# microsoft/hyperspace

Hardware: NVIDIA H100
Metric: createIndex rows/sec (higher is better)
Workload: dtype int64

## Files before the change

hyperspace_b200/csrc/api.cu:

```cuda
#include <dirent.h>
#include <fcntl.h>
#include <sys/stat.h>
#include <unistd.h>

#include <algorithm>
#include <atomic>
#include <chrono>
#include <exception>
#include <map>
#include <mutex>
#include <thread>

#include "device_utils.cuh"
#include "engine.h"

using namespace hs;

#define HS_STR2(x) #x
#define HS_STR(x) HS_STR2(x)

namespace {

void set_err(char* err, size_t errlen, const char* msg) {
  if (err && errlen) {
// ... 262 lines not shown
    return HS_EINVAL;
  }
  hs_ctx* ctx = new hs_ctx();
  ctx->device = device_id;
  int rc = guarded(nullptr, err, errlen, [&] {
    HS_CUDA(cudaSetDevice(device_id));
    cudaDeviceProp prop;
    HS_CUDA(cudaGetDeviceProperties(&prop, device_id));
    ctx->sm_count = prop.multiProcessorCount;
    if (prop.major != 9 || prop.minor != 0)
      fail(HS_ENODEVICE, "device %d is sm_%d%d; this library is built for sm_90a only", device_id, prop.major, prop.minor);
    if (cuda_stream) {
      ctx->stream = (cudaStream_t)cuda_stream;
      ctx->own_stream = false;
    } else {
      HS_CUDA(cudaStreamCreateWithFlags(&ctx->stream, cudaStreamNonBlocking));
      ctx->own_stream = true;
    }
    HS_CUDA(cudaStreamCreateWithFlags(&ctx->h2d_stream, cudaStreamNonBlocking));
    HS_CUDA(cudaStreamCreateWithFlags(&ctx->d2h_stream, cudaStreamNonBlocking));
  });
  if (rc != HS_OK) {
    delete ctx;
    return rc == HS_ECUDA ? HS_ENODEVICE : rc;
  }
  *out = ctx;
  return HS_OK;
}

void hs_shutdown(hs_ctx* ctx) {
  if (!ctx) return;
  cudaSetDevice(ctx->device);
  xfer_release(ctx);
  if (ctx->decode_cache && ctx->decode_cache_free) ctx->decode_cache_free(ctx->decode_cache);
  ctx->decode_cache = nullptr;
  comm_destroy(ctx);
  if (ctx->own_stream) cudaStreamDestroy(ctx->stream);
  if (ctx->h2d_stream) {
    cudaStreamSynchronize(ctx->h2d_stream);
    cudaStreamDestroy(ctx->h2d_stream);
  }
  if (ctx->d2h_stream) {
    cudaStreamSynchronize(ctx->d2h_stream);
    cudaStreamDestroy(ctx->d2h_stream);
  }
  delete ctx;
}

void hs_trim(hs_ctx* ctx) {
  if (!ctx) return;
  cudaSetDevice(ctx->device);
  cudaStreamSynchronize(ctx->stream);
  ctx->pool.trim();
}

void hs_profile_enable(hs_ctx* ctx, int on) {
  if (!ctx) return;
  cudaSetDevice(ctx->device);
  cudaStreamSynchronize(ctx->stream);
  for (auto& k : ctx->kevents) {
    ctx->event_pool.push_back(k.a);
    ctx->event_pool.push_back(k.b);
  }
  ctx->kevents.clear();
  ctx->profile = on != 0;
}

int hs_profile_report(hs_ctx* ctx, char* out, size_t outlen) {
  if (!ctx || !out || !outlen) return HS_EINVAL;
  cudaSetDevice(ctx->device);
  cudaStreamSynchronize(ctx->stream);
  std::map<std::string, std::pair<int, double>> acc;
  for (auto& k : ctx->kevents) {
    float ms = 0;
    if (cudaEventElapsedTime(&ms, k.a, k.b) != cudaSuccess) {
      cudaGetLastError();
      continue;
    }
    auto& e = acc[k.name];
    e.first++;
    e.second += ms;
  }
  std::string s = "{";
  bool first = true;
  for (auto& kv : acc) {
    char buf[256];
    snprintf(buf, sizeof buf, "%s\"%s\": {\"launches\": %d, \"ms\": %.6f}", first ? "" : ", ", kv.first.c_str(), kv.second.first,
             kv.second.second);
    s += buf;
    first = false;
  }
  s += "}";
  if (s.size() + 1 > outlen) return HS_ENOMEM;
  memcpy(out, s.c_str(), s.size() + 1);
  for (auto& k : ctx->kevents) {
    ctx->event_pool.push_back(k.a);
    ctx->event_pool.push_back(k.b);
  }
  ctx->kevents.clear();
  return HS_OK;
}

void* hs_host_alloc(hs_ctx* ctx, size_t bytes) {
  if (!ctx) return nullptr;
  try {
    cudaSetDevice(ctx->device);
    return ctx->pool.get(bytes, true);
  } catch (...) {
    return nullptr;
  }
}

void hs_host_free(hs_ctx* ctx, void* p) {
  if (ctx && p) ctx->pool.put(p);
}


int hs_stage_sources(hs_ctx* ctx, const hs_source_file* files, int32_t n_files, hs_staged** out, char* err, size_t errlen) {
  if (!ctx || !out || n_files < 0 || (n_files > 0 && !files)) return HS_EINVAL;
  *out = nullptr;
  std::unique_ptr<hs_staged> sg(new hs_staged());
  sg->ctx = ctx;
  int rc = guarded(ctx, err, errlen, [&] {
    const int launches_before = ctx->launches;
    std::vector<uint64_t> sizes(n_files), off(n_files);
    uint64_t total = 0;
    for (int f = 0; f < n_files; f++) {
      const hs_source_file& sf = files[f];
      if (sf.data && sf.on_device) fail(HS_EINVAL, "source file %d is already on the device", f);
      if (sf.data) {
        sizes[f] = sf.size;
      } else {
        if (!sf.path) fail(HS_EINVAL, "source file %d has neither data nor path", f);
        struct stat st;
        if (stat(sf.path, &st) != 0) fail(HS_EIO, "cannot stat %s", sf.path);
        sizes[f] = (uint64_t)st.st_size;
      }
      if (sizes[f] < 12) fail(HS_EFORMAT, "source file %d: too small to be a Parquet file", f);
      off[f] = total;
      total += round_up(sizes[f], 16) + 16;
    }
    sg->d_images.alloc(ctx, std::max<uint64_t>(total, 16));
    HS_CUDA(cudaEventCreate(&sg->begin));
    HS_CUDA(cudaEventRecord(sg->begin, ctx->h2d_stream));
    sg->files.resize(n_files);
    sg->names.resize(n_files);
    sg->metas.resize(n_files);
    std::vector<uint8_t*> pinned(n_files, nullptr);
    std::vector<size_t> disk;
    for (int f = 0; f < n_files; f++)
      if (!files[f].data) {
        sg->staging.emplace_back(ctx, sizes[f], true);
        pinned[f] = sg->staging.back().get();
        disk.push_back((size_t)f);
      }
    std::vector<std::atomic<int>> read_done(n_files);
    for (auto& d : read_done) d.store(0);
    std::exception_ptr read_error;
    std::thread reader;
    if (!disk.empty())
      reader = std::thread([&] {
        try {
          parallel_files(disk.size(), [&](size_t j) {
            const size_t f = disk[j];
            read_file_into(files[f].path, pinned[f], sizes[f]);
            read_done[f].store(1, std::memory_order_release);
          });
        } catch (...) {
          read_error = std::current_exception();
        }
        for (size_t f : disk)
          if (!read_done[f].load()) read_done[f].store(-1, std::memory_order_release);
      });
    struct Joiner {
      std::thread& t;
      ~Joiner() {
        if (t.joinable()) t.join();
      }
    } joiner{reader};
    for (int f = 0; f < n_files; f++) {
      const hs_source_file& sf = files[f];
      sg->names[f] = sf.path ? sf.path : ("<memory file " + std::to_string(f) + ">");
      const uint8_t* host = (const uint8_t*)sf.data;
      if (!host) {
        int st;
        while ((st = read_done[f].load(std::memory_order_acquire)) == 0) std::this_thread::yield();
        if (st < 0) {
          if (reader.joinable()) reader.join();
          if (read_error) std::rethrow_exception(read_error);
          fail(HS_EIO, "cannot read %s", sf.path);
        }
        host = pinned[f];
      }
      sg->metas[f] = std::make_shared<hs::pq::FileMeta>(hs::pq::parse_footer(host, sizes[f], sg->names[f].c_str()));
      HS_CUDA(cudaMemcpyAsync(sg->d_images.get() + off[f], host, sizes[f], cudaMemcpyHostToDevice, ctx->h2d_stream));
      hs_source_file& o = sg->files[f];
      o.path = nullptr;
      o.data = sg->d_images.get() + off[f];
      o.size = sizes[f];
      o.file_id = sf.file_id;
      o.on_device = 1;
      o.reserved = 0;
      sg->bytes += sizes[f];
    }
    HS_CUDA(cudaEventCreate(&sg->ready));
    HS_CUDA(cudaEventRecord(sg->ready, ctx->h2d_stream));
    for (int f = 0; f < n_files; f++) ctx->staged[sg->files[f].data] = hs_ctx::StagedImage{sg->metas[f], sg->ready};
    ctx->launches = launches_before;
  });
  if (rc == HS_OK) *out = sg.release();
  return rc;
}

int32_t hs_staged_num_files(const hs_staged* s) { return s ? (int32_t)s->files.size() : 0; }

int hs_staged_file(const hs_staged* s, int32_t i, hs_source_file* out) {
  if (!s || !out || i < 0 || i >= (int32_t)s->files.size()) return HS_EINVAL;
  *out = s->files[i];
  out->path = s->names[i].c_str();
  return HS_OK;
}

static void timeline(hs_ctx* ctx, const char* what, cudaEvent_t a, cudaEvent_t b) {
  static const bool on = getenv("HS_TIMELINE") != nullptr;
  if (!on || !a || !b) return;
  static cudaEvent_t base = nullptr;
  if (!base) base = a;
  float t0 = 0, t1 = 0;
  if (cudaEventElapsedTime(&t0, base, a) != cudaSuccess || cudaEventElapsedTime(&t1, base, b) != cudaSuccess) {
    cudaGetLastError();
    return;
  }
  fprintf(stderr, "[hs timeline] %-8s %10.2f -> %10.2f  (%8.2f ms)\n", what, t0, t1, t1 - t0);
}

int hs_staged_wait(hs_staged* s, float* ms_copy) {
  if (!s) return HS_EINVAL;
  cudaSetDevice(s->ctx->device);
  if (cudaEventSynchronize(s->ready) != cudaSuccess) return HS_ECUDA;
  if (ms_copy && cudaEventElapsedTime(ms_copy, s->begin, s->ready) != cudaSuccess) *ms_copy = 0;
  timeline(s->ctx, "H2D", s->begin, s->ready);
  return HS_OK;
}

void hs_staged_free(hs_staged* s) {
  if (!s) return;
  hs_ctx* ctx = s->ctx;
  cudaSetDevice(ctx->device);
  if (s->ready) {
    cudaEventSynchronize(s->ready);
    cudaEventDestroy(s->ready);
  }
  if (s->begin && !getenv("HS_TIMELINE")) cudaEventDestroy(s->begin);
  for (const hs_source_file& f : s->files) ctx->staged.erase(f.data);
  cudaStreamSynchronize(ctx->stream);
  delete s;
}


int hs_create_index_async(hs_ctx* ctx, const hs_index_spec* spec, hs_pending** out, char* err, size_t errlen) {
  if (!ctx || !spec || !out) return HS_EINVAL;
  *out = nullptr;
  std::unique_ptr<hs_pending> pd(new hs_pending());
  pd->ctx = ctx;
  pd->res.reset(new hs_index_result());
  hs_stats& st = pd->st;
  memset(&st, 0, sizeof st);
  hs_index_result* res = pd->res.get();
  int rc = guarded(ctx, err, errlen, [&] {
    if (spec->n_indexed < 1) fail(HS_EINVAL, "at least one indexed column is required");
    if (spec->n_files < 0 || (spec->n_files > 0 && !spec->files)) fail(HS_EINVAL, "bad source file list");
    if (spec->output == HS_OUT_FILES && !spec->out_dir) fail(HS_EINVAL, "HS_OUT_FILES needs out_dir");
    HS_CUDA(cudaEventCreate(&pd->t_begin));
    HS_CUDA(cudaEventCreate(&pd->t_compute_end));
    HS_CUDA(cudaEventRecord(pd->t_begin, ctx->stream));
    std::vector<std::string> cols = names_of(spec->indexed_columns, spec->n_indexed, spec->included_columns, spec->n_included);
    for (size_t i = 0; i < cols.size(); i++)
      for (size_t j = i + 1; j < cols.size(); j++)
        if (cols[i] == cols[j]) fail(HS_EINVAL, "duplicate column '%s' in index config", cols[i].c_str());
    EncodedFiles enc;
    {
      Table table;
      const bool no_carry = getenv("HS_NO_CARRY") != nullptr;
      CarryOptions carry;
      if ((ctx->world == 1 || p2p_exchange_supported(ctx, spec->num_buckets)) && !spec->disable_dictionary &&
          spec->n_deleted_file_ids == 0 && !no_carry && fused_partition_supported(spec->num_buckets)) {
        carry.first_col = spec->n_indexed;
        carry.num_segments = spec->num_buckets;
      }
      if (fused_partition_supported(spec->num_buckets) && spec->n_deleted_file_ids == 0 && !getenv("HS_NO_ZEROCOPY")) {
        carry.zc_tile_rows = fused_tile_rows(p2p_exchange_supported(ctx, spec->num_buckets));
        carry.zc_first_col = spec->n_indexed;
        carry.zc_key = spec->n_indexed == 1;
      }
      SourceSet src;
      open_sources(ctx, spec->files, spec->n_files, &src, &st);
      decode_sources(ctx, src, cols, nullptr, &table, &st, &carry);
      const bool has_strings = table.has_strings;
      if (has_strings && ctx->world > 1)
        fail(HS_EUNSUPPORTED, "string / binary columns are not exchanged between GPUs yet: build this index on one GPU");
      if (spec->lineage) fill_lineage(ctx, table, spec->files, spec->n_files);
      if (spec->n_deleted_file_ids > 0) drop_deleted_rows(ctx, table, spec->deleted_file_ids, spec->n_deleted_file_ids);
      IndexedRows rows;
      if (p2p_exchange_supported(ctx, spec->num_buckets)) {
        exchange_partition_p2p(ctx, table, spec->n_indexed, spec->num_buckets, &rows, &st);
        sort_partitioned_rows(ctx, spec->n_indexed, spec->num_buckets, &rows, &st, true);
      } else {
        if (ctx->world > 1) exchange_rows(ctx, table, spec->n_indexed, spec->num_buckets, &st);
        index_rows(ctx, table, spec->n_indexed, spec->num_buckets, &rows, &st, true);
      }
      if (!has_strings) src.release_images();

      EncodeRequest req;
      req.table = &rows.part;
      req.d_perm = rows.sorted.perm();
      req.d_sorted_keys = rows.sorted.keys();
      req.plan = &rows.plan;
      req.seg_offsets = rows.bucket_offsets;
      req.rows_per_page = spec->rows_per_page;
      req.rows_per_row_group = spec->rows_per_row_group;
      req.use_dictionary = spec->disable_dictionary == 0;
      if (spec->compression != HS_CODEC_UNCOMPRESSED && spec->compression != HS_CODEC_SNAPPY)
        fail(HS_EUNSUPPORTED, "compression codec %d; the GPU path writes UNCOMPRESSED and SNAPPY pages", spec->compression);
      req.codec = spec->compression == HS_CODEC_SNAPPY ? pq::SNAPPY : pq::UNCOMPRESSED;
      const std::string uuid = spec->job_uuid ? spec->job_uuid : make_uuid();
      req.seg_names.resize(spec->num_buckets);
      for (int b = 0; b < spec->num_buckets; b++) {
        char nm[160];
        snprintf(nm, sizeof nm, "part-%05d-%s_%05d.c000%s.parquet", b, uuid.c_str(), b, req.codec == pq::SNAPPY ? ".snappy" : "");
        req.seg_names[b] = nm;
      }
      req.probe = rows.probe.get();
      encode_segments(ctx, req, &enc, &st);
      if (settle_sort(ctx, &rows, &st)) {
        req.probe = nullptr;
        req.d_perm = rows.sorted.perm();
        req.d_sorted_keys = rows.sorted.keys();
        enc = EncodedFiles();
        encode_segments(ctx, req, &enc, &st);
      }
      st.rows_out = rows.part.nrows;
    }
    HS_CUDA(cudaEventRecord(pd->t_compute_end, ctx->stream));
    res->ctx = ctx;
    res->output = spec->output;
    res->files = enc.files;
    pd->save_mode = spec->save_mode;
    if (spec->out_dir) pd->out_dir = spec->out_dir;
    st.gpu_launches = ctx->launches;
    if (spec->output == HS_OUT_DEVICE) {
      res->d_arena = std::move(enc.arena);
      return;
    }
    pd->d_arena = std::move(enc.arena);
    res->h_arena.alloc(ctx, std::max<uint64_t>(enc.arena_bytes, 16), true);
    HS_CUDA(cudaEventCreate(&pd->t_d2h_begin));
    HS_CUDA(cudaEventCreate(&pd->t_d2h_end));
    HS_CUDA(cudaStreamWaitEvent(ctx->d2h_stream, pd->t_compute_end, 0));
    HS_CUDA(cudaEventRecord(pd->t_d2h_begin, ctx->d2h_stream));
    if (enc.arena_bytes)
      HS_CUDA(cudaMemcpyAsync(res->h_arena.get(), pd->d_arena.get(), enc.arena_bytes, cudaMemcpyDeviceToHost, ctx->d2h_stream));
    HS_CUDA(cudaEventRecord(pd->t_d2h_end, ctx->d2h_stream));
    pd->has_d2h = true;
  });
  if (rc == HS_OK) *out = pd.release();
  return rc;
}

int hs_pending_wait(hs_pending* p, hs_index_result** out, hs_stats* stats, char* err, size_t errlen) {
  if (!p || !out) return HS_EINVAL;
  *out = nullptr;
  std::unique_ptr<hs_pending> pd(p);
  hs_ctx* ctx = pd->ctx;
  const int launches = ctx->launches;
  int rc = guarded(ctx, err, errlen, [&] {
    hs_stats& st = pd->st;
    float ms = 0;
    if (pd->has_d2h) {
      HS_CUDA(cudaEventSynchronize(pd->t_d2h_end));
      HS_CUDA(cudaEventElapsedTime(&ms, pd->t_d2h_begin, pd->t_d2h_end));
      st.ms_d2h += ms;
      HS_CUDA(cudaEventElapsedTime(&ms, pd->t_begin, pd->t_d2h_end));
      st.ms_total = ms;
      timeline(ctx, "build", pd->t_begin, pd->t_compute_end);
      timeline(ctx, "D2H", pd->t_d2h_begin, pd->t_d2h_end);
      pd->d_arena.release();
    } else {
      HS_CUDA(cudaEventSynchronize(pd->t_compute_end));
      HS_CUDA(cudaEventElapsedTime(&ms, pd->t_begin, pd->t_compute_end));
      st.ms_total = ms;
    }
    if (pd->res->output == HS_OUT_FILES) {
      const auto w0 = std::chrono::steady_clock::now();
      write_result_files(pd->res.get(), pd->out_dir, pd->save_mode);
      st.ms_write += std::chrono::duration<float, std::milli>(std::chrono::steady_clock::now() - w0).count();
    }
  });
  ctx->launches = launches;
  if (stats) *stats = pd->st;
  if (rc == HS_OK) *out = pd->res.release();
  return rc;
}

void hs_pending_cancel(hs_pending* p) {
  if (!p) return;
  cudaSetDevice(p->ctx->device);
  if (p->has_d2h) cudaEventSynchronize(p->t_d2h_end);
  delete p;
}

int hs_create_index(hs_ctx* ctx, const hs_index_spec* spec, hs_index_result** out, hs_stats* stats, char* err,
                    size_t errlen) {
  if (!ctx || !spec || !out) return HS_EINVAL;
  *out = nullptr;
  if (stats) memset(stats, 0, sizeof *stats);
  hs_pending* pd = nullptr;
  int rc = hs_create_index_async(ctx, spec, &pd, err, errlen);
  if (rc != HS_OK) return rc;
  const int launches = ctx->launches;
  rc = hs_pending_wait(pd, out, stats, err, errlen);
  if (stats) stats->gpu_launches = launches;
  return rc;
}

int32_t hs_result_num_files(const hs_index_result* r) { return r ? (int32_t)r->files.size() : 0; }

int hs_result_file(const hs_index_result* r, int32_t i, int32_t* bucket, const char** name, const void** data,
                   uint64_t* size, int64_t* rows) {
  if (!r || i < 0 || i >= (int32_t)r->files.size()) return HS_EINVAL;
  const OutFile& f = r->files[i];
  if (bucket) *bucket = f.bucket;
  if (name) *name = f.name.c_str();
  if (data) {
    if (r->output == HS_OUT_DEVICE) *data = r->d_arena.get() + f.offset;
    else if (r->output == HS_OUT_HOST) *data = r->h_arena.get() + f.offset;
    else *data = nullptr;
  }
  if (size) *size = f.size;
  if (rows) *rows = f.rows;
  return HS_OK;
}

void hs_result_free(hs_index_result* r) {
  if (!r) return;
  if (r->ctx) {
    cudaSetDevice(r->ctx->device);
    cudaStreamSynchronize(r->ctx->stream);
  }
  delete r;
}


static void batch_from_gather(hs_ctx* ctx, const Table& t, const std::vector<int>& col_idx, const uint32_t* d_idx,
                              int64_t n_out, hs_batch* b) {
  std::vector<Buf<uint8_t>> d_data, d_valid;
  std::vector<Buf<uint64_t>> d_offsets(col_idx.size());
  std::vector<uint64_t> str_bytes(col_idx.size(), 0);
  for (size_t k = 0; k < col_idx.size(); k++) {
    const int ci = col_idx[k];
    const DevColumn& c = t.cols[ci];
    if (c.type == HS_TYPE_STRING) {
      const uint8_t* valid = c.has_nulls ? c.valid.get() : nullptr;
      Buf<uint32_t> lens(ctx, (size_t)std::max<int64_t>(1, n_out));
      d_offsets[k].alloc(ctx, (size_t)n_out + 1);
      launch_string_lengths(ctx, (const uint64_t*)c.data.get(), valid, d_idx, n_out, lens.get());
      exclusive_scan_u32_u64(ctx, lens.get(), n_out, d_offsets[k].get());
      copy_d2h(ctx, &str_bytes[k], d_offsets[k].get() + n_out, 8);
      sync_stream(ctx);
      d_data.emplace_back(ctx, std::max<uint64_t>(1, str_bytes[k]));
      launch_copy_strings(ctx, (const uint64_t*)c.data.get(), valid, d_idx, n_out, d_offsets[k].get(), d_data.back().get());
      d_valid.emplace_back();
      if (c.has_nulls) {
        d_valid.back().alloc(ctx, (size_t)std::max<int64_t>(1, n_out));
        launch_gather_plain(ctx, c.valid.get(), d_idx, n_out, 1, d_valid.back().get());
      }
      continue;
    }
    d_data.emplace_back(ctx, (size_t)std::max<int64_t>(1, n_out) * c.width);
    launch_gather_plain(ctx, c.data.get(), d_idx, n_out, c.width, d_data.back().get());
    d_valid.emplace_back();
    if (c.has_nulls) {
      d_valid.back().alloc(ctx, (size_t)std::max<int64_t>(1, n_out));
      launch_gather_plain(ctx, c.valid.get(), d_idx, n_out, 1, d_valid.back().get());
    }
  }
  for (size_t i = 0; i < col_idx.size(); i++) {
    const DevColumn& c = t.cols[col_idx[i]];
    hs_batch::Col bc;
    bc.name = c.name;
    bc.type = c.type;
    bc.has_valid = c.has_nulls;
    const bool is_str = c.type == HS_TYPE_STRING;
    const size_t data_bytes = is_str ? (size_t)str_bytes[i] : (size_t)n_out * c.width;
    bc.total_bytes = is_str ? str_bytes[i] : 0;
    if (b->on_device) {
      bc.data = std::move(d_data[i]);
      if (is_str) bc.offsets = std::move(d_offsets[i]);
      if (c.has_nulls) bc.valid = std::move(d_valid[i]);
    } else {
      bc.data.alloc(ctx, std::max<size_t>(1, data_bytes), true);
      if (data_bytes) copy_d2h_engine(ctx, bc.data.get(), d_data[i].get(), data_bytes);
      if (is_str) {
        bc.offsets.alloc(ctx, (size_t)n_out + 1, true);
        copy_d2h_engine(ctx, bc.offsets.get(), d_offsets[i].get(), 8 * ((size_t)n_out + 1));
      }
      if (c.has_nulls) {
        bc.valid.alloc(ctx, (size_t)std::max<int64_t>(1, n_out), true);
        if (n_out) copy_d2h_engine(ctx, bc.valid.get(), d_valid[i].get(), (size_t)n_out);
      }
    }
    b->cols.push_back(std::move(bc));
  }
  sync_stream(ctx);
  b->nrows = n_out;
}

__global__ void k_widen_i32(const int32_t* __restrict__ in, int64_t n, int64_t* __restrict__ out) {
  const int64_t stride = (int64_t)gridDim.x * blockDim.x;
  for (int64_t i = (int64_t)blockIdx.x * blockDim.x + threadIdx.x; i < n; i += stride) out[i] = in[i];
}

static const int64_t* widened_key(hs_ctx* ctx, const DevColumn& c, const void* data, int64_t n, Buf<int64_t>* hold) {
  if (c.type == HS_TYPE_INT64) return (const int64_t*)data;
  if (c.type != HS_TYPE_INT32) fail(HS_EUNSUPPORTED, "key column '%s' must be int32 or int64 on the read side", c.name.c_str());
  hold->alloc(ctx, std::max<int64_t>(1, n));
  if (n) {
    k_widen_i32<<<(int)std::min<int64_t>(ceil_div(n, 256), ctx->sm_count * 16), 256, 0, ctx->stream>>>((const int32_t*)data, n,
                                                                                                      hold->get());
    HS_LAUNCH_CHECK(ctx);
  }
  return hold->get();
}

__global__ void k_ranges_to_indices(const int64_t* __restrict__ bounds, const uint64_t* __restrict__ seg_offsets,
                                    const uint64_t* __restrict__ out_offsets, int nseg, uint32_t* __restrict__ out_idx) {
  const int s = blockIdx.x;
  if (s >= nseg) return;
  const int64_t first = bounds[2 * s], last = bounds[2 * s + 1];
  const uint64_t base = seg_offsets[s], o = out_offsets[s];
  for (int64_t i = first + threadIdx.x; i < last; i += blockDim.x) out_idx[o + (i - first)] = (uint32_t)(base + i);
}

}


template <typename F>
static int spark_compare(F a, F b) {
  const bool na = a != a, nb = b != b;
  if (na || nb) return na == nb ? 0 : (na ? 1 : -1);
  return a < b ? -1 : (a > b ? 1 : 0);
}

static int compare_encoded(int col_type, uint64_t e, int lit_type, int64_t lit_i, double lit_f) {
  const bool lit_long = lit_type == HS_TYPE_INT64;
  switch (col_type) {
    case HS_TYPE_INT32:
    case HS_TYPE_INT64: {
      const int64_t v = col_type == HS_TYPE_INT32 ? (int64_t)(int32_t)((uint32_t)e ^ 0x80000000u) : (int64_t)(e ^ 0x8000000000000000ull);
      if (lit_long) return v < lit_i ? -1 : (v > lit_i ? 1 : 0);
      return spark_compare((double)v, lit_f);
    }
    case HS_TYPE_FLOAT: {
      const uint32_t u = (uint32_t)e, bits = (u & 0x80000000u) ? (u & 0x7fffffffu) : ~u;
      float f;
      memcpy(&f, &bits, 4);
      return lit_long ? spark_compare(f, (float)lit_i) : spark_compare((double)f, lit_f);
    }
    default: {
      const uint64_t bits = (e & 0x8000000000000000ull) ? (e & 0x7fffffffffffffffull) : ~e;
      double d;
      memcpy(&d, &bits, 8);
      return spark_compare(d, lit_long ? (double)lit_i : lit_f);
    }
  }
}

static void encoded_domain(int col_type, uint64_t* lo, uint64_t* hi) {
  switch (col_type) {
    case HS_TYPE_INT32: *lo = 0, *hi = 0xffffffffull; return;
    case HS_TYPE_INT64: *lo = 0, *hi = ~0ull; return;
    case HS_TYPE_FLOAT: *lo = 0x007fffffull, *hi = 0xffffffffull; return;
    default: *lo = 0x000fffffffffffffull, *hi = ~0ull; return;
  }
}

struct ResolvedPredicate {
  int col = -1;
  PredRange r{};
  const uint8_t* lo_host = nullptr;
  const uint8_t* hi_host = nullptr;
  uint32_t lo_len = 0, hi_len = 0;
};

static PredRange resolve_predicate(hs_ctx* ctx, const hs_predicate& p, const DevColumn& c, std::vector<Buf<uint8_t>>* holder,
                                   ResolvedPredicate* rp) {
  const bool str_col = c.type == HS_TYPE_STRING;
  int lit = p.literal_type;
  if (lit < 0) {
    if (!str_col && c.type != HS_TYPE_INT32 && c.type != HS_TYPE_INT64) fail(HS_EUNSUPPORTED, "filter scan: key column must be int32 / int64 / string");
    lit = str_col ? HS_TYPE_STRING : HS_TYPE_INT64;
  }
  if (c.type == HS_TYPE_BOOL) fail(HS_EUNSUPPORTED, "filter scan: predicates on the boolean column '%s' are not handled", c.name.c_str());
  if (c.type < HS_TYPE_INT32 || c.type > HS_TYPE_STRING) fail(HS_EUNSUPPORTED, "filter scan: column '%s' has an unhandled type", c.name.c_str());
  if (str_col != (lit == HS_TYPE_STRING))
    fail(HS_EUNSUPPORTED, "filter scan: a %s literal cannot be compared with the %s column '%s'", lit == HS_TYPE_STRING ? "string" : "numeric",
         str_col ? "string" : "numeric", c.name.c_str());
  PredRange r{};
  r.type = c.type;
  r.has_lo = p.has_lo != 0;
  r.has_hi = p.has_hi != 0;
  if (str_col) {
    if ((p.has_lo && p.lo_len && !p.lo_bytes) || (p.has_hi && p.hi_len && !p.hi_bytes))
      fail(HS_EINVAL, "filter scan: string column '%s' needs lo_bytes / hi_bytes", c.name.c_str());
    if (p.lo_len > kMaxStringLen || p.hi_len > kMaxStringLen) fail(HS_EUNSUPPORTED, "string bound longer than 65535 bytes");
    const uint32_t ll = p.has_lo ? p.lo_len : 0, hl = p.has_hi ? p.hi_len : 0;
    holder->emplace_back(ctx, (size_t)ll + hl + 16);
    uint8_t* d = holder->back().get();
    if (ll) copy_h2d(ctx, d, p.lo_bytes, ll);
    if (hl) copy_h2d(ctx, d + ll, p.hi_bytes, hl);
    r.lo = string_ref(d, ll);
    r.hi = string_ref(d + ll, hl);
    r.lo_strict = r.has_lo && p.lo_strict;
    r.hi_strict = r.has_hi && p.hi_strict;
    rp->lo_host = (const uint8_t*)p.lo_bytes, rp->lo_len = ll;
    rp->hi_host = (const uint8_t*)p.hi_bytes, rp->hi_len = hl;
    return r;
  }
  uint64_t emin, emax;
  encoded_domain(c.type, &emin, &emax);
  auto cmp = [&](uint64_t e, bool hi_side) {
    return compare_encoded(c.type, e, lit, hi_side ? p.hi_i : p.lo_i, hi_side ? p.hi_f : p.lo_f);
  };
  bool empty = false;
  if (r.has_lo) {
    const int t = p.lo_strict ? 1 : 0;
    if (cmp(emax, false) < t) {
// ... 778 lines not shown
```

hyperspace_b200/csrc/device_utils.cuh:

```cuda
#pragma once
#include <cuda_runtime.h>

#include <cstdint>

#ifndef HS_HD
#ifdef __CUDACC__
#define HS_HD __host__ __device__ __forceinline__
#else
#define HS_HD inline
#endif
#endif

namespace hs {

HS_HD uint32_t rotl32(uint32_t x, int r) { return (x << r) | (x >> (32 - r)); }
HS_HD uint32_t mm3_mix_k1(uint32_t k1) {
  k1 *= 0xcc9e2d51u;
  k1 = rotl32(k1, 15);
  k1 *= 0x1b873593u;
  return k1;
}
HS_HD uint32_t mm3_mix_h1(uint32_t h1, uint32_t k1) {
  h1 ^= k1;
  h1 = rotl32(h1, 13);
  return h1 * 5u + 0xe6546b64u;
}
HS_HD uint32_t mm3_fmix(uint32_t h1, uint32_t len) {
  h1 ^= len;
  h1 ^= h1 >> 16;
  h1 *= 0x85ebca6bu;
  h1 ^= h1 >> 13;
  h1 *= 0xc2b2ae35u;
  h1 ^= h1 >> 16;
  return h1;
}
HS_HD uint32_t mm3_hash_int(uint32_t v, uint32_t seed) { return mm3_fmix(mm3_mix_h1(seed, mm3_mix_k1(v)), 4); }
HS_HD uint32_t mm3_hash_long(uint64_t v, uint32_t seed) {
  uint32_t h1 = mm3_mix_h1(seed, mm3_mix_k1((uint32_t)v));
  h1 = mm3_mix_h1(h1, mm3_mix_k1((uint32_t)(v >> 32)));
  return mm3_fmix(h1, 8);
}
HS_HD int32_t spark_pmod(uint32_t h, int32_t n) {
  int32_t r = (int32_t)h % n;
  return r < 0 ? r + n : r;
}

constexpr uint32_t kMaxStringLen = 0xffffu;
HS_HD uint64_t string_ref(const void* p, uint32_t len) { return ((uint64_t)(uintptr_t)p & 0xffffffffffffull) | ((uint64_t)len << 48); }
HS_HD const uint8_t* ref_ptr(uint64_t ref) { return (const uint8_t*)(uintptr_t)(ref & 0xffffffffffffull); }
HS_HD uint32_t ref_len(uint64_t ref) { return (uint32_t)(ref >> 48); }

HS_HD uint32_t mm3_hash_bytes(const uint8_t* p, uint32_t len, uint32_t seed) {
  uint32_t h1 = seed;
  const uint32_t aligned = len & ~3u;
  for (uint32_t i = 0; i < aligned; i += 4) {
    const uint32_t w = (uint32_t)p[i] | ((uint32_t)p[i + 1] << 8) | ((uint32_t)p[i + 2] << 16) | ((uint32_t)p[i + 3] << 24);
    h1 = mm3_mix_h1(h1, mm3_mix_k1(w));
  }
  for (uint32_t i = aligned; i < len; i++) h1 = mm3_mix_h1(h1, mm3_mix_k1((uint32_t)(int32_t)(int8_t)p[i]));
  return mm3_fmix(h1, len);
}

HS_HD int string_compare(uint64_t ra, uint64_t rb) {
  const uint8_t *a = ref_ptr(ra), *b = ref_ptr(rb);
  const uint32_t la = ref_len(ra), lb = ref_len(rb), n = la < lb ? la : lb;
  for (uint32_t i = 0; i < n; i++)
    if (a[i] != b[i]) return a[i] < b[i] ? -1 : 1;
  return la == lb ? 0 : (la < lb ? -1 : 1);
}

HS_HD uint64_t string_chunk(uint64_t ref, uint32_t chunk) {
  const uint8_t* p = ref_ptr(ref);
  const uint32_t len = ref_len(ref), begin = chunk * 8;
  uint64_t v = 0;
  for (uint32_t i = 0; i < 8; i++) v = (v << 8) | (begin + i < len ? (uint64_t)p[begin + i] : 0ull);
  return v;
}

HS_HD uint32_t mm3_hash_value(int type, uint64_t raw, uint32_t seed) {
  switch (type) {
    case 0: return mm3_hash_int((uint32_t)raw, seed);
    case 1: return mm3_hash_long(raw, seed);
    case 2: {
      uint32_t b = (uint32_t)raw;
      if ((b & 0x7fffffffu) == 0) b = 0;
      else if ((b & 0x7fffffffu) > 0x7f800000u) b = 0x7fc00000u;
      return mm3_hash_int(b, seed);
    }
    case 3: {
      uint64_t b = raw;
      if ((b & 0x7fffffffffffffffull) == 0) b = 0;
      else if ((b & 0x7fffffffffffffffull) > 0x7ff0000000000000ull) b = 0x7ff8000000000000ull;
      return mm3_hash_long(b, seed);
    }
    case 4: return mm3_hash_int((raw & 0xff) ? 1u : 0u, seed);
    case 5: return mm3_hash_bytes(ref_ptr(raw), ref_len(raw), seed);
  }
  return seed;
}

HS_HD uint64_t sort_encode(int type, uint64_t raw) {
  switch (type) {
    case 0: return (uint64_t)((uint32_t)raw ^ 0x80000000u);
    case 1: return raw ^ 0x8000000000000000ull;
    case 2: {
      uint32_t b = (uint32_t)raw;
      if ((b & 0x7fffffffu) == 0) b = 0;
      else if ((b & 0x7fffffffu) > 0x7f800000u) b = 0x7fc00000u;
      return (uint64_t)((b & 0x80000000u) ? ~b : (b | 0x80000000u));
    }
    case 3: {
      uint64_t b = raw;
      if ((b & 0x7fffffffffffffffull) == 0) b = 0;
      else if ((b & 0x7fffffffffffffffull) > 0x7ff0000000000000ull) b = 0x7ff8000000000000ull;
      return (b & 0x8000000000000000ull) ? ~b : (b | 0x8000000000000000ull);
    }
    case 4: return (raw & 0xff) ? 1 : 0;
  }
  return raw;
}

HS_HD uint32_t dict_hash_u64(uint64_t v) { return (uint32_t)((v * 0x9E3779B97F4A7C15ull) >> 32); }

HS_HD int type_width(int type) {
  switch (type) {
    case 0: case 2: return 4;
    case 1: case 3: return 8;
    case 4: return 1;
    case 5: return 8;
  }
  return 0;
}

#ifdef __CUDACC__

__device__ __forceinline__ uint64_t load_le64_unaligned(const uint8_t* p) {
  uintptr_t a = (uintptr_t)p;
  const uint64_t* w = (const uint64_t*)(a & ~(uintptr_t)7);
  unsigned s = (unsigned)(a & 7) * 8;
  uint64_t lo = __ldg(w);
  if (s == 0) return lo;
  uint64_t hi = __ldg(w + 1);
  return (lo >> s) | (hi << (64 - s));
}
__device__ __forceinline__ uint32_t load_le32_unaligned(const uint8_t* p) {
  uintptr_t a = (uintptr_t)p;
  const uint32_t* w = (const uint32_t*)(a & ~(uintptr_t)3);
  unsigned s = (unsigned)(a & 3) * 8;
  uint32_t lo = __ldg(w);
  if (s == 0) return lo;
  uint32_t hi = __ldg(w + 1);
  return __funnelshift_r(lo, hi, s);
}

__device__ __forceinline__ uint32_t extract_bits(const uint8_t* base, uint64_t idx, uint32_t bw) {
  uint64_t bit = idx * bw;
  const uint8_t* p = base + (bit >> 3);
  uintptr_t a = (uintptr_t)p;
  const uint32_t* w = (const uint32_t*)(a & ~(uintptr_t)3);
  unsigned s = (unsigned)(a & 3) * 8 + (unsigned)(bit & 7);
  uint64_t v = __ldg(w);
  if (s + bw > 32) v |= (uint64_t)__ldg(w + 1) << 32;
  return (uint32_t)((v >> s) & ((bw >= 32) ? 0xffffffffull : ((1ull << bw) - 1)));
}

template <int W>
__device__ __forceinline__ void warp_store_unaligned(uint8_t* dst, uint64_t v, bool active) {
  static_assert(W == 4 || W == 8, "W");
  const unsigned lane = threadIdx.x & 31;
  unsigned long long d = active ? (unsigned long long)(uintptr_t)dst : 0ull;
  unsigned long long d_prev = __shfl_up_sync(0xffffffffu, d, 1);
  uint64_t v_prev = __shfl_up_sync(0xffffffffu, (unsigned long long)v, 1);
  unsigned long long d_next = __shfl_down_sync(0xffffffffu, d, 1);
  if (!active) return;
  const unsigned a = (unsigned)(d & (W - 1));
  if (a == 0) {
    if (W == 8) *(uint64_t*)dst = v;
    else *(uint32_t*)dst = (uint32_t)v;
    return;
  }
  const bool has_prev = lane > 0 && d_prev != 0 && d_prev + W == d;
  const bool has_next = lane < 31 && d_next != 0 && d + W == d_next;
  uint8_t* word = dst - a;
  const unsigned s = a * 8;
  if (has_prev) {
    if (W == 8) *(uint64_t*)word = (v_prev >> (64 - s)) | (v << s);
    else *(uint32_t*)word = (uint32_t)(((uint32_t)v_prev >> (32 - s)) | ((uint32_t)v << s));
  } else {
    for (unsigned i = 0; i < W - a; i++) dst[i] = (uint8_t)(v >> (8 * i));
  }
  if (!has_next) {
    for (unsigned i = W - a; i < W; i++) dst[i] = (uint8_t)(v >> (8 * i));
  }
}

__device__ __forceinline__ unsigned match_any_bits(unsigned amask, unsigned v, int nbits) {
  unsigned peers = amask;
  for (int b = 0; b < nbits; b++) {
    const bool bit = (v >> b) & 1u;
    const unsigned m = __ballot_sync(amask, bit);
    peers &= bit ? m : ~m;
  }
  return peers;
}
template <int NBITS>
__device__ __forceinline__ unsigned match_any_bits(unsigned amask, unsigned v) {
  unsigned peers = amask;
#pragma unroll
  for (int b = 0; b < NBITS; b++) {
    const bool bit = (v & (1u << b)) != 0;
    const unsigned m = __ballot_sync(amask, bit);
    peers &= m ^ (bit ? 0u : ~0u);
  }
  return peers;
}

template <int NBITS>
__device__ __forceinline__ unsigned match_any_full(unsigned v) {
  unsigned peers = 0xffffffffu;
#pragma unroll
  for (int b = 0; b < NBITS; b++) {
    unsigned m, x;
    asm volatile(
        "{\n\t"
        ".reg .pred p;\n\t"
        ".reg .b32 t;\n\t"
        "and.b32 t, %2, %3;\n\t"
        "setp.ne.u32 p, t, 0;\n\t"
        "vote.sync.ballot.b32 %0, p, 0xffffffff;\n\t"
        "selp.b32 %1, 0, 0xffffffff, p;\n\t"
        "}"
        : "=r"(m), "=r"(x)
        : "r"(v), "r"(1u << b));
    peers &= m ^ x;
  }
  return peers;
}

__device__ __forceinline__ uint32_t block_exclusive_scan(uint32_t x, uint32_t* warp_sums, uint32_t* total) {
  const unsigned lane = threadIdx.x & 31, warp = threadIdx.x >> 5, nwarps = (blockDim.x + 31) >> 5;
  uint32_t incl = x;
#pragma unroll
  for (int o = 1; o < 32; o <<= 1) {
    uint32_t y = __shfl_up_sync(0xffffffffu, incl, o);
    if (lane >= (unsigned)o) incl += y;
  }
  __syncthreads();
  if (lane == 31) warp_sums[warp] = incl;
  __syncthreads();
  if (warp == 0) {
    uint32_t w = lane < nwarps ? warp_sums[lane] : 0;
    uint32_t wi = w;
#pragma unroll
    for (int o = 1; o < 32; o <<= 1) {
      uint32_t y = __shfl_up_sync(0xffffffffu, wi, o);
      if (lane >= (unsigned)o) wi += y;
    }
    warp_sums[lane] = wi - w;
    if (lane == 31) warp_sums[32] = wi;
  }
  __syncthreads();
  uint32_t res = warp_sums[warp] + incl - x;
  if (total) *total = warp_sums[32];
  return res;
}

#endif

}
```

hyperspace_b200/csrc/engine.cu:

```cuda
#include <fcntl.h>
#include <sys/stat.h>
#include <unistd.h>

#include <algorithm>
#include <array>
#include <map>
#include <random>

#include "device_utils.cuh"
#include "engine.h"

namespace hs {

std::string make_uuid() {
  std::random_device rd;
  std::mt19937_64 gen(((uint64_t)rd() << 32) ^ rd());
  uint64_t a = gen(), b = gen();
  char buf[40];
  snprintf(buf, sizeof buf, "%08x-%04x-4%03x-%04x-%012llx", (unsigned)(a >> 32), (unsigned)((a >> 16) & 0xffff),
           (unsigned)(a & 0xfff), (unsigned)(0x8000 | ((b >> 48) & 0x3fff)), (unsigned long long)(b & 0xffffffffffffull));
  return buf;
}

namespace {
// ... 436 lines not shown
    sync_stream(ctx);
    check_walk();
    std::vector<SnappyBlob> blobs;
    std::map<const uint8_t*, uint64_t> dict_off;
    uint64_t cursor = 0;
    for (PageDesc& pg : h_pages) {
      if (pg.codec == pq::UNCOMPRESSED) continue;
      if (pg.dict) {
        auto it = dict_off.find(pg.dict);
        if (it == dict_off.end()) {
          it = dict_off.emplace(pg.dict, cursor).first;
          blobs.push_back(SnappyBlob{pg.dict, cursor, (uint32_t)pg.dict_size, (uint32_t)pg.dict_uncompressed_size, 0u, 1u, 0u, 0u});
          cursor += round_up((size_t)pg.dict_uncompressed_size, 16) + 16;
        }
        pg.dict = (const uint8_t*)(uintptr_t)(it->second + 1);
        pg.dict_size = -1;
      }
      if (pg.is_compressed || pg.size != pg.uncompressed_size) {
        const uint32_t prefix = pg.page_type == pq::DATA_PAGE_V2 ? (uint32_t)(pg.rep_bytes + std::max(0, pg.def_bytes)) : 0u;
        if (prefix > (uint32_t)pg.size || prefix > (uint32_t)pg.uncompressed_size)
          fail(HS_EFORMAT, "compressed page has level bytes beyond its size");
        blobs.push_back(SnappyBlob{pg.data, cursor, (uint32_t)pg.size, (uint32_t)pg.uncompressed_size, prefix,
                                   (uint32_t)(pg.is_compressed ? 1 : 0), 0u, 0u});
        pg.data = (const uint8_t*)(uintptr_t)(cursor + 1);
        pg.size = -pg.uncompressed_size;
        cursor += round_up((size_t)pg.uncompressed_size, 16) + 16;
      }
    }
    d_scratch.alloc(ctx, std::max<uint64_t>(cursor, 16) + 16);
    for (PageDesc& pg : h_pages) {
      if (pg.codec == pq::UNCOMPRESSED) continue;
      if (pg.dict_size == -1) {
        pg.dict = d_scratch.get() + ((uintptr_t)pg.dict - 1);
        pg.dict_size = pg.dict_uncompressed_size;
      }
      if (pg.size < 0) {
        pg.data = d_scratch.get() + ((uintptr_t)pg.data - 1);
        pg.size = pg.uncompressed_size;
      }
    }
    uint64_t total_blocks = 0;
    bool any_verbatim = false;
    for (SnappyBlob& b : blobs) {
      any_verbatim = any_verbatim || b.prefix != 0 || !b.compressed;
      b.first_block = (uint32_t)total_blocks;
      total_blocks += snappy_blocks_of(b.dst_len, b.prefix);
    }
    if (total_blocks >= 0xffffffffull) fail(HS_EUNSUPPORTED, "more than 256 TB of compressed pages in one call");
    Buf<SnappyBlob> d_blobs(ctx, std::max<size_t>(1, blobs.size()));
    Buf<uint32_t> d_block_in(ctx, (size_t)total_blocks + 1), d_sequential(ctx, std::max<size_t>(1, blobs.size()));
    copy_h2d(ctx, d_blobs.get(), blobs.data(), sizeof(SnappyBlob) * blobs.size());
    copy_h2d(ctx, d_pages.get(), h_pages.data(), sizeof(PageDesc) * (size_t)n_pages);
    launch_snappy_decompress(ctx, d_blobs.get(), (int64_t)blobs.size(), (int64_t)total_blocks, any_verbatim, d_block_in.get(),
                             d_sequential.get(),
                             d_scratch.get(), d_flags.get());
    sync_stream(ctx);
  }
  Buf<uint64_t> d_string_dicts;
  bool any_string = false;
  for (int c = 0; c < ncols; c++) any_string = any_string || out->cols[c].type == HS_TYPE_STRING;
  out->has_strings = any_string;
  if (any_string && n_pages > 0) {
    std::vector<PageDesc> h_pages((size_t)n_pages);
    copy_d2h(ctx, h_pages.data(), d_pages.get(), sizeof(PageDesc) * (size_t)n_pages);
    sync_stream(ctx);
    check_walk();
    std::map<const uint8_t*, size_t> job_of;
    std::vector<StringDictJob> jobs;
    std::vector<size_t> job_off;
    size_t total = 0;
    for (PageDesc& pg : h_pages) {
      if (pg.phys_type != pq::BYTE_ARRAY || !pg.dict || pg.encoding == pq::ENC_PLAIN) continue;
      auto it = job_of.find(pg.dict);
      if (it == job_of.end()) {
        it = job_of.emplace(pg.dict, jobs.size()).first;
        jobs.push_back(StringDictJob{pg.dict, nullptr, pg.dict_size, pg.dict_count});
        job_off.push_back(total);
        total += (size_t)std::max(0, pg.dict_count);
      }
    }
    if (!jobs.empty()) {
      d_string_dicts.alloc(ctx, std::max<size_t>(1, total));
      for (size_t j = 0; j < jobs.size(); j++) jobs[j].refs = d_string_dicts.get() + job_off[j];
      for (PageDesc& pg : h_pages) {
        if (pg.phys_type != pq::BYTE_ARRAY || !pg.dict || pg.encoding == pq::ENC_PLAIN) continue;
        const StringDictJob& job = jobs[job_of[pg.dict]];
        pg.dict = (const uint8_t*)job.refs;
        pg.dict_size = job.count * 8;
      }
      Buf<StringDictJob> d_jobs(ctx, jobs.size());
      copy_h2d(ctx, d_jobs.get(), jobs.data(), sizeof(StringDictJob) * jobs.size());
      launch_build_string_dicts(ctx, d_jobs.get(), (int64_t)jobs.size(), d_flags.get());
      copy_h2d(ctx, d_pages.get(), h_pages.data(), sizeof(PageDesc) * (size_t)n_pages);
      if (sizeof(PageDesc) * (size_t)n_pages > (16u << 20)) sync_stream(ctx);
    }
  }
  const bool want_zc = carry && carry->zc_tile_rows > 0 && !file_windows && n_pages > 0 && nrows > 0;
  std::vector<uint32_t> local_cls(ncols, 0u);
  constexpr uint32_t kAgreeCap = 8192;
  constexpr int kMaxSpec = 6;
  std::vector<int> spec;
  if (want_carry)
    for (int c = carry->first_col; c < ncols && (int)spec.size() < kMaxSpec; c++) spec.push_back(c);
  const int nspec = (int)spec.size();
  std::vector<uint32_t> spec_state(4 * (size_t)std::max(1, nspec), 0u), spec_count(std::max(1, nspec), 0u);
  std::vector<uint64_t> spec_vals((size_t)std::max(1, nspec) * kAgreeCap);
  if ((want_carry || want_zc) && n_pages > 0) {
    Buf<uint32_t> d_class(ctx, ncols);
    fill_bytes(ctx, d_class.get(), 0, 4 * (size_t)ncols);
    launch_classify_pages(ctx, d_pages.get(), n_pages, d_class.get(), want_zc ? carry->zc_tile_rows : 0);
    copy_d2h(ctx, local_cls.data(), d_class.get(), 4 * (size_t)ncols);
    Buf<uint32_t> d_states(ctx, 4 * (size_t)std::max(1, nspec)), d_cnt(ctx, std::max(1, nspec));
    Buf<unsigned long long> d_vals(ctx, (size_t)std::max(1, nspec) * kAgreeCap);
    std::vector<Buf<unsigned long long>> sets(nspec);
    if (nspec) {
      fill_bytes(ctx, d_states.get(), 0, 16 * (size_t)nspec);
      fill_bytes(ctx, d_cnt.get(), 0, 4 * (size_t)nspec);
      for (int i = 0; i < nspec; i++) {
        const DevColumn& dc = out->cols[spec[i]];
        if ((dc.width != 4 && dc.width != 8) || dc.type == HS_TYPE_STRING) continue;
        sets[i].alloc(ctx, kDictCapacity);
        fill_bytes(ctx, sets[i].get(), 0xFF, sizeof(unsigned long long) * kDictCapacity);
        launch_dict_build_from_pages(ctx, d_pages.get(), n_pages, spec[i], dc.width, sets[i].get(), kDictCapacity, kMaxDictEntries,
                                     d_states.get() + 4 * i);
        launch_dict_collect(ctx, sets[i].get(), kDictCapacity, d_vals.get() + (size_t)i * kAgreeCap, d_cnt.get() + i, kAgreeCap);
      }
      copy_d2h(ctx, spec_state.data(), d_states.get(), 16 * (size_t)nspec);
      copy_d2h(ctx, spec_count.data(), d_cnt.get(), 4 * (size_t)nspec);
      copy_d2h(ctx, spec_vals.data(), d_vals.get(), 8 * (size_t)nspec * kAgreeCap);
    }
    sync_stream(ctx);
  } else {
    sync_stream(ctx);
  }
  check_walk();
  if (want_carry) {
    const int W = ctx->world;
    const size_t per_cand = 5 + kAgreeCap, words = (size_t)ncols + 1 + (size_t)nspec * per_cand;
    std::vector<uint64_t> mine(words, 0ull), all(words * W);
    for (int c = 0; c < ncols; c++) mine[c] = local_cls[c] & (PAGECLASS_NOT_DICT | PAGECLASS_MAYBE_NULLS);
    mine[ncols] = (uint64_t)nrows;
    for (int i = 0; i < nspec; i++) {
      const DevColumn& dc = out->cols[spec[i]];
      uint64_t* m = &mine[(size_t)ncols + 1 + (size_t)i * per_cand];
      m[0] = (uint64_t)(int64_t)dc.type;
      m[1] = dc.type == HS_TYPE_STRING ? 0ull : (uint64_t)dc.width;
      m[2] = spec_state[4 * i];
      m[3] = (spec_state[4 * i + 1] || spec_count[i] > kAgreeCap) ? 1 : 0;
      m[4] = spec_state[4 * i + 2];
      const uint32_t nv = std::min<uint32_t>(spec_count[i], kAgreeCap);
      for (uint32_t j = 0; j < nv; j++) m[5 + j] = spec_vals[(size_t)i * kAgreeCap + j];
      std::sort(m + 5, m + 5 + nv);
      m[2] = nv;
    }
    comm_allgather_host(ctx, mine.data(), 8 * words, all.data());
    DecodeCache* cache = static_cast<DecodeCache*>(ctx->decode_cache);
    const bool hit = cache && cache->num_segments == carry->num_segments && cache->first_col == carry->first_col &&
                     cache->message.size() == all.size() && memcmp(cache->message.data(), all.data(), 8 * all.size()) == 0;
    std::vector<uint32_t> cls(ncols, 0u);
    int64_t total_rows = 0;
    if (hit) {
      total_rows = cache->total_rows;
      for (DecodeCache::Column& cc : cache->carried) {
        DevColumn& dc = out->cols[cc.col];
        dc.carried = true;
        dc.dict_values = cc.values;
        dc.dict_bw = cc.bw;
        dc.codes.alloc(ctx, (size_t)std::max<int64_t>(1, nrows) + 16);
        h_cols[cc.col] = ColumnOut{dc.codes.get(), nullptr, dc.width, dc.type, cc.table.get(), cc.mask, cc.empty_index, 1, 0};
      }
    } else {
      for (int r = 0; r < W; r++) {
        const uint64_t* a = &all[(size_t)r * words];
        for (int c = 0; c < ncols; c++) cls[c] |= (uint32_t)a[c];
        total_rows += (int64_t)a[ncols];
      }
      if (!cache) {
        cache = new DecodeCache();
        ctx->decode_cache = cache;
        ctx->decode_cache_free = free_decode_cache;
      }
      cache->carried.clear();
      cache->message = all;
      cache->num_segments = carry->num_segments;
      cache->first_col = carry->first_col;
      cache->total_rows = total_rows;
    }
    out->global_rows = total_rows;
    int ncarried = 0;
    for (int i = 0; !hit && i < nspec && ncarried < kMaxCarried && total_rows > 0; i++) {
      const int c = spec[i];
      DevColumn& dc = out->cols[c];
      if (cls[c] != 0) continue;
      int type = -1, width = 0;
      bool overflow = false, has_empty = false;
      std::vector<uint64_t> values;
      for (int r = 0; r < W; r++) {
        const uint64_t* m = &all[(size_t)r * words + (size_t)ncols + 1 + (size_t)i * per_cand];
        if ((int64_t)m[0] >= 0) type = (int)(int64_t)m[0];
        width = std::max(width, (int)m[1]);
        overflow = overflow || m[3] != 0;
        has_empty = has_empty || m[4] != 0;
        values.insert(values.end(), m + 5, m + 5 + m[2]);
      }
      if (overflow || type < 0 || (width != 4 && width != 8)) continue;
      if (has_empty) values.push_back(~0ull);
      sort_dictionary(values, type);
      values.erase(std::unique(values.begin(), values.end()), values.end());
      const uint32_t bw = bits_for((uint32_t)values.size());
      if (!dictionary_pays_off((uint32_t)values.size(), bw, width, total_rows, carry->num_segments)) continue;
      cache->carried.emplace_back();
      DecodeCache::Column& cc = cache->carried.back();
      cc.col = c;
      cc.bw = bw;
      upload_lookup_table(ctx, values, &cc.table, &cc.mask, &cc.empty_index);
      cc.values = values;
      dc.carried = true;
      dc.dict_values = std::move(values);
      dc.dict_bw = bw;
      dc.codes.alloc(ctx, (size_t)std::max<int64_t>(1, nrows) + 16);
      h_cols[c] = ColumnOut{dc.codes.get(), nullptr, dc.width, dc.type, cc.table.get(), cc.mask, cc.empty_index, 1, 0};
      ncarried++;
    }
  }
  Buf<ZcTile*> d_tile_src;
  if (want_zc) {
    std::vector<ZcTile*> h_tile_src(ncols, nullptr);
    const int64_t T = carry->zc_tile_rows;
    bool any = false;
    for (int c = 0; c < ncols; c++) {
      DevColumn& dc = out->cols[c];
      const bool candidate = c >= carry->zc_first_col || (c == 0 && carry->zc_key && (dc.type == HS_TYPE_INT32 || dc.type == HS_TYPE_INT64));
      if (!candidate || dc.carried || (dc.width != 4 && dc.width != 8)) continue;
      if (local_cls[c] & (PAGECLASS_NOT_IN_PLACE | PAGECLASS_MAYBE_NULLS)) continue;
      dc.zero_copy = true;
      dc.zc_tiles.alloc(ctx, (size_t)ceil_div(nrows, T));
      h_tile_src[c] = dc.zc_tiles.get();
      h_cols[c] = ColumnOut{nullptr, nullptr, dc.width, dc.type, nullptr, 0u, 0u, 0, 1};
      any = true;
    }
    if (any) {
      d_tile_src.alloc(ctx, ncols);
      copy_h2d(ctx, d_tile_src.get(), h_tile_src.data(), sizeof(ZcTile*) * ncols);
      launch_fill_zc_tiles(ctx, d_pages.get(), n_pages, d_tile_src.get(), (int)T, nrows);
    }
  }
  alloc_destinations();
  copy_h2d(ctx, d_cols.get(), h_cols.data(), sizeof(ColumnOut) * ncols);
  Buf<int64_t> d_window;
  if (file_windows) {
    std::vector<int64_t> w(2 * (size_t)n_files);
    for (int f = 0; f < n_files; f++) {
      w[2 * f] = out->file_row_begin[f] + (*file_windows)[f].first;
      w[2 * f + 1] = out->file_row_begin[f] + (*file_windows)[f].second;
    }
    d_window.alloc(ctx, w.size());
    copy_h2d(ctx, d_window.get(), w.data(), 8 * w.size());
    sync_stream(ctx);
  }
  launch_decode_pages(ctx, d_pages.get(), n_pages, d_cols.get(), d_flags.get() + 1, file_windows ? d_window.get() : nullptr,
                      d_flags.get());
  std::vector<uint32_t> flags(1 + ncols);
  copy_d2h(ctx, flags.data(), d_flags.get(), sizeof(uint32_t) * (1 + ncols));
  t_dec.stop();
  sync_stream(ctx);
  if (flags[0]) {
    const uint32_t code = flags[0] >> 24, detail = flags[0] & 0xffffffu;
    const int ecode = (code == DERR_COMPRESSED || code == DERR_UNSUPPORTED_ENCODING || code == DERR_UNSUPPORTED_TYPE || code == DERR_STRING_TOO_LONG)
                          ? HS_EUNSUPPORTED
                          : HS_EFORMAT;
    fail(ecode, "Parquet decode failed: %s (detail %u)", decode_error_text(code), detail);
  }
  for (int c = 0; c < ncols; c++) out->cols[c].has_nulls = (flags[1 + c] & 1u) != 0;
  if (!file_windows && ctx->world == 1) {
    std::vector<int> cand;
    Buf<uint32_t> d_states(ctx, 4 * (size_t)std::max(1, ncols));
    fill_bytes(ctx, d_states.get(), 0, 16 * (size_t)std::max(1, ncols));
    for (int c = 0; c < ncols; c++) {
      DevColumn& dc = out->cols[c];
      if (dc.carried || dc.zero_copy || dc.type == HS_TYPE_STRING || (flags[1 + c] & 2u) || (dc.width != 4 && dc.width != 8)) continue;
      dc.dict_keys.alloc(ctx, kDictCapacity);
      fill_bytes(ctx, dc.dict_keys.get(), 0xFF, sizeof(unsigned long long) * kDictCapacity);
      launch_dict_build_from_pages(ctx, d_pages.get(), n_pages, c, dc.width, dc.dict_keys.get(), kDictCapacity, kMaxDictEntries,
                                   d_states.get() + 4 * c);
      cand.push_back(c);
    }
    if (!cand.empty()) {
      std::vector<uint32_t> h_states(4 * (size_t)ncols);
      copy_d2h(ctx, h_states.data(), d_states.get(), 16 * (size_t)ncols);
      sync_stream(ctx);
      for (int c : cand) {
        DevColumn& dc = out->cols[c];
        memcpy(dc.dict_state, &h_states[4 * c], 16);
        dc.dict_ready = dc.dict_state[1] == 0;
        if (!dc.dict_ready) dc.dict_keys.release();
      }
    }
  }
  stats->ms_plan += t_plan.ms();
  stats->ms_decode += t_dec.ms();
}


void index_rows(hs_ctx* ctx, Table& table, int nkeys, int num_buckets, IndexedRows* out, hs_stats* stats, bool defer_settle) {
  const int64_t nrows = table.nrows;
  const int ncols = (int)table.cols.size();
  if (num_buckets < 1 || num_buckets > kMaxBuckets)
    fail(HS_EUNSUPPORTED, "numBuckets = %d; the GPU path handles 1..%d buckets", num_buckets, kMaxBuckets);
  if (nkeys < 1 || nkeys > ncols) fail(HS_EINVAL, "bad number of indexed columns");
  if (nrows >= (1ll << 32)) fail(HS_EUNSUPPORTED, "more than 2^32-1 rows per GPU per call");
  StageTimer t_hash(ctx), t_part(ctx);

  t_hash.start();
  std::vector<KeyColumn> h_keys(nkeys);
  for (int k = 0; k < nkeys; k++) {
    DevColumn& c = table.cols[k];
    h_keys[k] = KeyColumn{c.data.get(), c.has_nulls ? c.valid.get() : nullptr, c.type, c.width, c.zero_copy ? c.zc_tiles.get() : nullptr};
  }
  Buf<KeyColumn> d_keys(ctx, nkeys);
  copy_h2d(ctx, d_keys.get(), h_keys.data(), sizeof(KeyColumn) * nkeys);
  const bool fused = fused_partition_supported(num_buckets);
  const int64_t ntiles = ceil_div(nrows, fused ? fused_tile_rows(false) : kPartTile);
  Buf<uint16_t> bucket;
  Buf<uint32_t> tile_hist(ctx, std::max<int64_t>(1, ntiles) * num_buckets);
  Buf<unsigned long long> ghist(ctx, num_buckets);
  out->d_bucket_offsets.alloc(ctx, num_buckets + 1);
  fill_bytes(ctx, ghist.get(), 0, sizeof(unsigned long long) * num_buckets);
  Buf<unsigned long long> d_key_bits(ctx, 2);
  if (fused) {
    const unsigned long long init[2] = {0ull, ~0ull};
    copy_h2d(ctx, d_key_bits.get(), init, sizeof init);
    static const bool rehash = getenv("HS_PART_REHASH") != nullptr;
    if (!rehash) bucket.alloc(ctx, std::max<int64_t>(1, nrows));
    launch_tile_hist(ctx, d_keys.get(), nkeys, nrows, num_buckets, 0, tile_hist.get(), ghist.get(), d_key_bits.get(),
                     single_key_type_of(h_keys.data(), nkeys), rehash ? nullptr : bucket.get());
    copy_d2h(ctx, out->key_or_and, d_key_bits.get(), sizeof out->key_or_and);
    out->have_key_bits = true;
  } else {
    bucket.alloc(ctx, std::max<int64_t>(1, nrows));
    launch_bucket_hist(ctx, d_keys.get(), nkeys, nrows, num_buckets, bucket.get(), tile_hist.get(), ghist.get());
  }
  launch_tile_offsets(ctx, tile_hist.get(), ntiles, num_buckets, ghist.get(),
                      (unsigned long long*)out->d_bucket_offsets.get());
  out->bucket_offsets.assign(num_buckets + 1, 0);
  copy_d2h(ctx, out->bucket_offsets.data(), out->d_bucket_offsets.get(), sizeof(uint64_t) * (num_buckets + 1));
  t_hash.stop();

  t_part.start();
  out->part.nrows = nrows;
  out->part.cols.clear();
  out->part.cols.resize(ncols);
  std::vector<PartColumn> h_pc;
  CodePackRound pack;
  memset(&pack, 0, sizeof pack);
  for (int c = 0; c < ncols; c++) {
    DevColumn& src = table.cols[c];
    DevColumn& dst = out->part.cols[c];
    dst.name = src.name;
    dst.type = src.type;
    dst.width = src.width;
    dst.schema = src.schema;
    dst.has_nulls = src.has_nulls;
    dst.dict_keys = std::move(src.dict_keys);
    memcpy(dst.dict_state, src.dict_state, sizeof dst.dict_state);
    dst.dict_ready = src.dict_ready;
    if (src.carried) {
      if (!fused || c < nkeys || pack.n >= kMaxCarried) fail(HS_EINVAL, "column '%s' cannot be late-materialised here", src.name.c_str());
      dst.carried = true;
      dst.dict_values = std::move(src.dict_values);
      dst.dict_bw = src.dict_bw;
      dst.carry_slot = pack.n;
      pack.src[pack.n++] = src.codes.get();
      continue;
    }
    dst.data.alloc(ctx, (size_t)nrows * src.width + 16);
    h_pc.push_back(PartColumn{src.data.get(), dst.data.get(), src.width, 0, src.zero_copy ? src.zc_tiles.get() : nullptr});
    if (src.has_nulls) {
      dst.valid.alloc(ctx, (size_t)nrows + 16);
      h_pc.push_back(PartColumn{src.valid.get(), dst.valid.get(), 1, 0});
    }
  }
  Buf<uint32_t> dest;
  Buf<PartColumn> d_pc(ctx, h_pc.size());
  if (fused) {
    copy_h2d(ctx, d_pc.get(), h_pc.data(), sizeof(PartColumn) * h_pc.size());
    if (pack.n > 0) {
      out->part.rec.alloc(ctx, (size_t)nrows * 8 + 16);
      pack.out = out->part.rec.get();
    }
    launch_partition_rows(ctx, d_keys.get(), nkeys, nrows, num_buckets, 0, tile_hist.get(), d_pc.get(), (int)h_pc.size(),
                          nullptr, 1, single_key_type_of(h_keys.data(), nkeys), &pack, bucket ? bucket.get() : nullptr);
  } else {
    dest.alloc(ctx, std::max<int64_t>(1, nrows));
    launch_partition_dest(ctx, bucket.get(), nrows, num_buckets, tile_hist.get(), dest.get());
    for (const PartColumn& pc : h_pc) launch_scatter_column(ctx, pc.in, pc.out, dest.get(), nrows, pc.width);
  }
  t_part.stop();
  if (defer_settle) launch_dictionary_probes(ctx, out->part, true, &out->probe);
  sync_stream(ctx);
  for (int c = 0; c < ncols; c++) {
    table.cols[c].data.release();
    table.cols[c].valid.release();
    table.cols[c].codes.release();
    table.cols[c].zc_tiles.release();
  }

  stats->ms_hash += t_hash.ms();
  stats->ms_partition += t_part.ms();
  sort_partitioned_rows(ctx, nkeys, num_buckets, out, stats, defer_settle);
}

void sort_partitioned_rows(hs_ctx* ctx, int nkeys, int num_buckets, IndexedRows* out, hs_stats* stats, bool defer_settle) {
  auto t_sort = std::make_unique<StageTimer>(ctx);
  if (defer_settle && !out->probe) {
    launch_dictionary_probes(ctx, out->part, true, &out->probe);
    if (out->probe) sync_stream(ctx);
  }
  t_sort->start();
  build_sort_plan(ctx, out->bucket_offsets.data(), num_buckets, &out->plan);
  std::vector<KeyColumn> keys(nkeys);
  for (int k = 0; k < nkeys; k++) {
    const DevColumn& c = out->part.cols[k];
    keys[k] = KeyColumn{c.data.get(), c.has_nulls ? c.valid.get() : nullptr, c.type, c.width};
  }
  sort_rows(ctx, &out->plan, keys.data(), nkeys, out->have_key_bits ? out->key_or_and : nullptr, defer_settle, &out->sorted);
  t_sort->stop();
  if (out->sorted.queued) {
    out->pending_timers.push_back(IndexedRows::DeferredTimer{std::move(t_sort), &hs_stats::ms_sort});
    return;
  }
  sync_stream(ctx);
  stats->ms_sort += t_sort->ms();
  for (auto& d : out->pending_timers) stats->*(d.field) += d.t->ms();
  out->pending_timers.clear();
}

bool settle_sort(hs_ctx* ctx, IndexedRows* out, hs_stats* stats) {
  StageTimer t(ctx);
  t.start();
  const bool again = settle_sorted_rows(ctx, &out->plan, &out->sorted);
  t.stop();
  if (again) {
    sync_stream(ctx);
    stats->ms_sort += t.ms();
  }
  for (auto& d : out->pending_timers) stats->*(d.field) += d.t->ms();
  out->pending_timers.clear();
  return again;
}

void launch_dictionary_probes(hs_ctx* ctx, const Table& part, bool use_dictionary, std::unique_ptr<DictProbe>* out) {
  out->reset();
  const int ncols = (int)part.cols.size();
  if (!use_dictionary || part.nrows == 0) return;
  auto pr = std::make_unique<DictProbe>();
  pr->mini = std::min<int64_t>(part.nrows, 1 << 14);
  pr->d_states.alloc(ctx, 4 * (size_t)ncols);
  pr->h_states.assign(4 * (size_t)ncols, 0u);
  pr->keys.resize(ncols);
  fill_bytes(ctx, pr->d_states.get(), 0, 16 * (size_t)ncols);
  bool any = false;
  for (int c = 0; c < ncols; c++) {
    const DevColumn& dc = part.cols[c];
    if (dc.has_nulls || dc.carried || dc.type == HS_TYPE_STRING || (dc.dict_ready && dc.dict_keys)) continue;
    if (dc.width != 4 && dc.width != 8) continue;
    pr->keys[c].alloc(ctx, kDictCapacity);
    fill_bytes(ctx, pr->keys[c].get(), 0xFF, sizeof(unsigned long long) * kDictCapacity);
    launch_dict_build(ctx, dc.data.get(), dc.width, 0, pr->mini, pr->keys[c].get(), kDictCapacity, kMaxDictEntries,
                      pr->d_states.get() + 4 * c);
    copy_d2h(ctx, &pr->h_states[4 * (size_t)c], pr->d_states.get() + 4 * c, 16);
    any = true;
  }
  if (!any) return;
  pr->queued_at = ctx->sync_count;
  *out = std::move(pr);
}


void encode_segments(hs_ctx* ctx, const EncodeRequest& req, EncodedFiles* out, hs_stats* stats) {
  const Table& table = *req.table;
  const int ncols = (int)table.cols.size();
  const int nseg = (int)req.seg_offsets.size() - 1;
  int64_t P = req.rows_per_page > 0 ? req.rows_per_page : 131072;
  P = (int64_t)round_up((size_t)P, kSortTile);
  StageTimer t_plan(ctx), t_enc(ctx);
  t_plan.start();
  for (int c = 0; c < ncols; c++) {
    const DevColumn& dc = table.cols[c];
    if (dc.width != 4 && dc.width != 8)
      fail(HS_EUNSUPPORTED, "column '%s': %d-byte values cannot be written by the GPU encoder yet", dc.name.c_str(), dc.width);
  }
  std::vector<pq::SchemaColumn> schema(ncols);
  for (int c = 0; c < ncols; c++) {
    schema[c] = table.cols[c].schema;
    schema[c].repetition = pq::OPTIONAL;
    schema[c].num_children = 0;
    switch (table.cols[c].type) {
      case HS_TYPE_INT32: schema[c].type = pq::INT32; break;
      case HS_TYPE_INT64: schema[c].type = pq::INT64; break;
      case HS_TYPE_FLOAT: schema[c].type = pq::FLOAT; break;
      case HS_TYPE_DOUBLE: schema[c].type = pq::DOUBLE; break;
      case HS_TYPE_STRING: schema[c].type = pq::BYTE_ARRAY; break;
    }
  }
  const std::string schema_json = pq::spark_schema_json(schema);

  const int64_t ntiles = req.plan->ntiles;
  std::vector<std::vector<uint32_t>> tile_valid(ncols), tile_bytes(ncols);
  std::vector<std::vector<uint64_t>> tile_val_off(ncols), tile_def_off(ncols);
  {
    std::vector<Buf<uint32_t>> d_counts(ncols), d_bytes(ncols);
    bool any = false;
    for (int c = 0; c < ncols; c++) {
      if (table.cols[c].type == HS_TYPE_STRING) {
        any = true;
        d_counts[c].alloc(ctx, std::max<int64_t>(1, ntiles));
        d_bytes[c].alloc(ctx, std::max<int64_t>(1, ntiles));
        launch_tile_string_sizes(ctx, req.plan->tiles.get(), ntiles, req.d_perm, (const uint64_t*)table.cols[c].data.get(),
                                 table.cols[c].has_nulls ? table.cols[c].valid.get() : nullptr, d_bytes[c].get(), d_counts[c].get());
        tile_valid[c].resize(ntiles);
        tile_bytes[c].resize(ntiles);
        tile_val_off[c].assign(ntiles, 0);
        tile_def_off[c].assign(ntiles, 0);
        if (ntiles) {
          copy_d2h(ctx, tile_valid[c].data(), d_counts[c].get(), sizeof(uint32_t) * ntiles);
          copy_d2h(ctx, tile_bytes[c].data(), d_bytes[c].get(), sizeof(uint32_t) * ntiles);
        }
        continue;
      }
      if (!table.cols[c].has_nulls) continue;
      any = true;
      d_counts[c].alloc(ctx, std::max<int64_t>(1, ntiles));
      launch_tile_valid_counts(ctx, req.plan->tiles.get(), ntiles, req.d_perm, table.cols[c].valid.get(), d_counts[c].get());
      tile_valid[c].resize(ntiles);
      tile_val_off[c].assign(ntiles, 0);
      tile_def_off[c].assign(ntiles, 0);
      if (ntiles)
        copy_d2h(ctx, tile_valid[c].data(), d_counts[c].get(), sizeof(uint32_t) * ntiles);
    }
    if (any) sync_stream(ctx);
  }
  const std::vector<uint32_t>& seg_tile_begin = req.plan->h_seg_tile_begin;

  struct ColDict {
    bool use = false;
    uint32_t bw = 0, ndict = 0, empty_index = 0, mask = 0;
    Buf<unsigned long long> keys;
    const unsigned long long* keys_ptr = nullptr;
    Buf<uint8_t> entries;
    size_t skel_off = 0, skel_len = 0;
    std::vector<uint64_t> values;
  };
  std::vector<ColDict> dicts(ncols);
  const int64_t total_rows = table.nrows;
  std::vector<int> carried_cols(kMaxCarried, -1);
  for (int c = 0; c < ncols; c++) {
    const DevColumn& dc = table.cols[c];
    if (!dc.carried) continue;
    if (dc.carry_slot < 0 || dc.carry_slot >= kMaxCarried || !table.rec) fail(HS_EINVAL, "column '%s': code record missing", dc.name.c_str());
    ColDict& cd = dicts[c];
    cd.values = dc.dict_values;
    cd.ndict = (uint32_t)cd.values.size();
    cd.bw = dc.dict_bw;
    cd.use = true;
    carried_cols[dc.carry_slot] = c;
  }
  if (req.use_dictionary && total_rows > 0) {
    DictProbe* early = req.probe;
    if (early && ((int)early->keys.size() != ncols || early->mini != std::min<int64_t>(total_rows, 1 << 14))) early = nullptr;
    if (early && !early->delivered(ctx)) sync_stream(ctx);
    Buf<uint32_t> own_states;
    if (early) own_states = std::move(early->d_states);
    else own_states.alloc(ctx, 4 * (size_t)ncols);
    Buf<uint32_t>& d_states = own_states;
    std::vector<uint32_t> h_states(4 * (size_t)ncols, 0u);
    if (early) h_states = early->h_states;
    else fill_bytes(ctx, d_states.get(), 0, 16 * (size_t)ncols);
    const int64_t mini = std::min<int64_t>(total_rows, 1 << 14);
    bool any_sampled = false;
    for (int c = 0; c < ncols; c++) {
      const DevColumn& dc = table.cols[c];
      if (dc.has_nulls || dc.carried || dc.type == HS_TYPE_STRING) continue;
      ColDict& cd = dicts[c];
      if (dc.dict_ready && dc.dict_keys) {
        cd.keys_ptr = dc.dict_keys.get();
        memcpy(&h_states[4 * (size_t)c], dc.dict_state, 16);
        continue;
      }
      if (early && early->keys[c]) {
        cd.keys = std::move(early->keys[c]);
        cd.keys_ptr = cd.keys.get();
        continue;
      }
      cd.keys.alloc(ctx, kDictCapacity);
      cd.keys_ptr = cd.keys.get();
      fill_bytes(ctx, cd.keys.get(), 0xFF, sizeof(unsigned long long) * kDictCapacity);
      launch_dict_build(ctx, dc.data.get(), dc.width, 0, mini, cd.keys.get(), kDictCapacity, kMaxDictEntries, d_states.get() + 4 * c);
      copy_d2h(ctx, &h_states[4 * (size_t)c], d_states.get() + 4 * c, 16);
      any_sampled = true;
    }
    if (any_sampled) sync_stream(ctx);
    for (int c = 0; c < ncols; c++) {
      const DevColumn& dc = table.cols[c];
      if (dc.has_nulls || dc.carried || dc.type == HS_TYPE_STRING) continue;
      ColDict& cd = dicts[c];
      uint32_t* st = &h_states[4 * (size_t)c];
      const bool ready = dc.dict_ready && dc.dict_keys;
      if (!ready) {
        uint32_t* d_state = d_states.get() + 4 * c;
        if (total_rows > (1 << 20) && st[0] + st[2] > 0.95 * mini) {
          cd.keys.release();
          continue;
        }
        const int64_t sample = std::min<int64_t>(total_rows, 1 << 18);
        if (sample > mini) {
          launch_dict_build(ctx, dc.data.get(), dc.width, mini, sample, cd.keys.get(), kDictCapacity, kMaxDictEntries, d_state);
          copy_d2h(ctx, st, d_state, 16);
          sync_stream(ctx);
        }
        if (!st[1] && sample < total_rows) {
          launch_dict_build(ctx, dc.data.get(), dc.width, sample, total_rows, cd.keys.get(), kDictCapacity, kMaxDictEntries, d_state);
          copy_d2h(ctx, st, d_state, 16);
          sync_stream(ctx);
        }
      }
      if (st[1]) {
        cd.keys.release();
        continue;
      }
      cd.values = sorted_dictionary(ctx, cd.keys_ptr, st, dc.type);
      cd.ndict = (uint32_t)cd.values.size();
      cd.bw = bits_for(cd.ndict);
      if (!dictionary_pays_off(cd.ndict, cd.bw, dc.width, total_rows, nseg)) {
        cd.keys.release();
        continue;
      }
      upload_lookup_table(ctx, cd.values, &cd.entries, &cd.mask, &cd.empty_index);
      cd.use = true;
    }
  }

  const bool stats_on_key = req.d_sorted_keys != nullptr && !table.cols[0].has_nulls &&
                            (table.cols[0].type == HS_TYPE_INT32 || table.cols[0].type == HS_TYPE_INT64);
  std::vector<StatPatch> stat_patches;
  std::vector<uint8_t> skeleton;
  std::vector<ByteCopy> copies;
  struct PagePlan {
    uint64_t hdr_off;
    uint32_t hdr_len;
    uint32_t body_len;
  };
  struct FilePlan {
    int seg = 0;
    int64_t rows = 0;
    std::vector<pq::OutRowGroup> rgs;
    std::vector<std::pair<size_t, size_t>> chunk_pages;
  };
  const bool compress = req.codec == pq::SNAPPY;
  std::vector<PagePlan> page_plans;
  std::vector<FilePlan> file_plans;
  auto header_len_at = [&](size_t skel_pos) -> uint32_t {
    thrift::Reader r(skeleton.data() + skel_pos, skeleton.data() + skeleton.size());
    r.skip(thrift::T_STRUCT);
    if (r.bad) fail(HS_EINVAL, "internal: page header does not parse");
    return (uint32_t)(r.p - (skeleton.data() + skel_pos));
  };
  std::vector<uint32_t> seg_page_begin(nseg + 1, 0);
  std::vector<std::vector<uint64_t>> page_value_offset(ncols);
  uint64_t cursor = 0;
  uint32_t page_counter = 0;
  auto emit = [&](uint64_t dst, size_t skel_begin) {
    copies.push_back(ByteCopy{dst, (uint32_t)skel_begin, (uint32_t)(skeleton.size() - skel_begin)});
  };
  for (int c = 0; c < ncols; c++) {
    ColDict& cd = dicts[c];
    if (!cd.use) continue;
    const int W = table.cols[c].width;
    cd.skel_off = skeleton.size();
    pq::write_dict_page_header(skeleton, (int32_t)(cd.ndict * W), (int32_t)cd.ndict);
    for (uint64_t v : cd.values) {
      const uint8_t* vp = (const uint8_t*)&v;
      skeleton.insert(skeleton.end(), vp, vp + W);
    }
    cd.skel_len = skeleton.size() - cd.skel_off;
  }
  out->files.clear();
  for (int s = 0; s < nseg; s++) {
    seg_page_begin[s] = page_counter;
    const int64_t n = (int64_t)(req.seg_offsets[s + 1] - req.seg_offsets[s]);
    if (n == 0) continue;
    int64_t RG = !req.seg_rows_per_row_group.empty() ? req.seg_rows_per_row_group[s]
                                                     : (req.rows_per_row_group > 0 ? req.rows_per_row_group : 4194304);
    RG = std::max<int64_t>(P, RG / P * P);
    const uint64_t file_off = round_up(cursor, 64);
    cursor = file_off;
    {
      size_t b = skeleton.size();
      skeleton.insert(skeleton.end(), {'P', 'A', 'R', '1'});
      emit(cursor, b);
      cursor += 4;
    }
    const int64_t npages = ceil_div(n, P);
    for (int c = 0; c < ncols; c++) page_value_offset[c].resize(page_counter + npages);
    std::vector<pq::OutRowGroup> rgs;
    for (int64_t r0 = 0; r0 < n; r0 += RG) {
      const int64_t r1 = std::min(n, r0 + RG);
      pq::OutRowGroup g;
      g.num_rows = r1 - r0;
      g.file_offset = (int64_t)(cursor - file_off);
      const uint64_t rg_begin = cursor;
      for (int c = 0; c < ncols; c++) {
        const int W = table.cols[c].width;
        pq::OutChunk ch;
        ch.type = schema[c].type;
        ch.num_values = r1 - r0;
        ch.data_page_offset = (int64_t)(cursor - file_off);
        ch.null_count = 0;
        ch.value_width = W;
        ch.has_minmax = stats_on_key && c == 0;
        const uint64_t chunk_begin = cursor;
        const size_t chunk_first_page = page_plans.size();
        if (dicts[c].use) {
          ch.has_dictionary = true;
          ch.dictionary_page_offset = (int64_t)(cursor - file_off);
          copies.push_back(ByteCopy{cursor, (uint32_t)dicts[c].skel_off, (uint32_t)dicts[c].skel_len});
          if (compress) {
            const uint32_t hl = header_len_at(dicts[c].skel_off);
            page_plans.push_back(PagePlan{cursor, hl, (uint32_t)(dicts[c].skel_len - hl)});
          }
          cursor += dicts[c].skel_len;
          ch.data_page_offset = (int64_t)(cursor - file_off);
        }
        for (int64_t p0 = r0; p0 < r1; p0 += P) {
          const int64_t np = std::min(P, r1 - p0);
          const size_t b = skeleton.size();
          const uint64_t page_begin = cursor;
          if (dicts[c].use) {
            pq::write_dict_data_page_prefix(skeleton, np, dicts[c].bw);
            emit(cursor, b);
            cursor += skeleton.size() - b;
            page_value_offset[c][page_counter + (p0 / P)] = cursor;
            cursor += (uint64_t)((np + 7) / 8) * dicts[c].bw;
          } else if (table.cols[c].type == HS_TYPE_STRING) {
            const int64_t t0 = seg_tile_begin[s] + p0 / kSortTile, t1 = seg_tile_begin[s] + ceil_div(p0 + np, (int64_t)kSortTile);
            int64_t non_null = 0;
            uint64_t value_bytes = 0;
            for (int64_t t = t0; t < t1; t++) {
              non_null += tile_valid[c][t];
              value_bytes += tile_bytes[c][t];
            }
            if (value_bytes + (uint64_t)np / 8 + 64 >= (1ull << 31)) fail(HS_EUNSUPPORTED, "column '%s': a page of strings exceeds 2 GiB", table.cols[c].name.c_str());
            pq::write_nullable_page_prefix_bytes(skeleton, np, value_bytes);
            emit(cursor, b);
            cursor += skeleton.size() - b;
            const uint64_t def_bits = cursor;
            cursor += (uint64_t)((np + 7) / 8);
            page_value_offset[c][page_counter + (p0 / P)] = cursor;
            uint64_t voff = cursor;
            for (int64_t t = t0; t < t1; t++) {
              tile_def_off[c][t] = def_bits + (uint64_t)(t - t0) * (kSortTile / 8);
              tile_val_off[c][t] = voff;
              voff += tile_bytes[c][t];
            }
            cursor += value_bytes;
            ch.null_count += np - non_null;
          } else if (!table.cols[c].has_nulls) {
            pq::write_plain_page_prefix(skeleton, cursor, np, W);
            emit(cursor, b);
            cursor += skeleton.size() - b;
            page_value_offset[c][page_counter + (p0 / P)] = cursor;
            cursor += (uint64_t)np * W;
          } else {
            const int64_t t0 = seg_tile_begin[s] + p0 / kSortTile, t1 = seg_tile_begin[s] + ceil_div(p0 + np, (int64_t)kSortTile);
            int64_t non_null = 0;
            for (int64_t t = t0; t < t1; t++) non_null += tile_valid[c][t];
            pq::write_nullable_page_prefix(skeleton, np, non_null, W);
            emit(cursor, b);
            cursor += skeleton.size() - b;
            const uint64_t def_bits = cursor;
            cursor += (uint64_t)((np + 7) / 8);
            page_value_offset[c][page_counter + (p0 / P)] = cursor;
            uint64_t voff = cursor;
            for (int64_t t = t0; t < t1; t++) {
              tile_def_off[c][t] = def_bits + (uint64_t)(t - t0) * (kSortTile / 8);
              tile_val_off[c][t] = voff;
              voff += (uint64_t)tile_valid[c][t] * W;
            }
            cursor += (uint64_t)non_null * W;
            ch.null_count += np - non_null;
          }
          if (compress) {
            const uint32_t hl = header_len_at(b);
            page_plans.push_back(PagePlan{page_begin, hl, (uint32_t)(cursor - page_begin - hl)});
          }
        }
        ch.total_size = (int64_t)(cursor - chunk_begin);
        g.chunks.push_back(ch);
        if (compress) {
          if (file_plans.empty() || file_plans.back().seg != s) {
            file_plans.emplace_back();
            file_plans.back().seg = s;
            file_plans.back().rows = n;
          }
          file_plans.back().chunk_pages.emplace_back(chunk_first_page, page_plans.size() - chunk_first_page);
        }
      }
      g.total_byte_size = (int64_t)(cursor - rg_begin);
      rgs.push_back(std::move(g));
    }
    {
      const size_t b = skeleton.size();
      std::vector<pq::StatSlot> slots;
      std::vector<uint8_t> footer = pq::write_footer(schema, rgs, n, schema_json, &slots);
      for (const pq::StatSlot& sl : slots) {
        StatPatch sp;
        int64_t row0 = 0;
        for (int g = 0; g < sl.row_group; g++) row0 += rgs[g].num_rows;
        sp.first_pos = req.seg_offsets[s] + (uint64_t)row0;
        sp.last_pos = sp.first_pos + (uint64_t)rgs[sl.row_group].num_rows - 1;
        for (int j = 0; j < 2; j++) {
          sp.min_off[j] = cursor + sl.min_off[j];
          sp.max_off[j] = cursor + sl.max_off[j];
        }
        sp.width = sl.width;
        sp.pad = 0;
        stat_patches.push_back(sp);
      }
      if (compress) file_plans.back().rgs = rgs;
      skeleton.insert(skeleton.end(), footer.begin(), footer.end());
      uint32_t flen = (uint32_t)footer.size();
      const uint8_t* lp = (const uint8_t*)&flen;
      skeleton.insert(skeleton.end(), lp, lp + 4);
      skeleton.insert(skeleton.end(), {'P', 'A', 'R', '1'});
      emit(cursor, b);
      cursor += skeleton.size() - b;
    }
    OutFile of;
    of.bucket = req.seg_ids.empty() ? s : req.seg_ids[s];
    of.name = req.seg_names[s];
    of.offset = file_off;
    of.size = cursor - file_off;
    of.rows = n;
    out->files.push_back(std::move(of));
    page_counter += (uint32_t)npages;
  }
  seg_page_begin[nseg] = page_counter;
  if (skeleton.size() >= (1ull << 32)) fail(HS_EUNSUPPORTED, "index metadata exceeds 4 GiB");
  out->arena_bytes = cursor;
  out->arena.alloc(ctx, std::max<uint64_t>(cursor, 16) + 64);

  Buf<uint8_t> d_skel(ctx, std::max<size_t>(1, skeleton.size()));
  Buf<ByteCopy> d_copies(ctx, std::max<size_t>(1, copies.size()));
  Buf<uint32_t> d_page_begin(ctx, seg_page_begin.size());
  Buf<uint64_t> d_pvo(ctx, std::max<size_t>(1, (size_t)ncols * page_counter));
  if (!skeleton.empty())
    copy_h2d(ctx, d_skel.get(), skeleton.data(), skeleton.size());
  if (!copies.empty())
    copy_h2d(ctx, d_copies.get(), copies.data(), copies.size() * sizeof(ByteCopy));
  copy_h2d(ctx, d_page_begin.get(), seg_page_begin.data(), seg_page_begin.size() * 4);
  for (int c = 0; c < ncols; c++)
    if (page_counter)
      copy_h2d(ctx, d_pvo.get() + (size_t)c * page_counter, page_value_offset[c].data(), (size_t)page_counter * 8);
  t_plan.stop();

  t_enc.start();
  launch_scatter_bytes(ctx, d_copies.get(), (int64_t)copies.size(), d_skel.get(), out->arena.get());
  for (int c = 0; c < ncols; c++) {
    const DevColumn& dc = table.cols[c];
    GatherColumn gc;
    gc.src = dc.data.get();
    gc.sorted_keys = nullptr;
    gc.key_type = dc.type;
    gc.width = dc.width;
    gc.page_value_offset = d_pvo.get() + (size_t)c * page_counter;
    if (dicts[c].use) continue;
    if (dc.type == HS_TYPE_STRING) {
      Buf<uint64_t> d_voff(ctx, std::max<int64_t>(1, ntiles)), d_doff(ctx, std::max<int64_t>(1, ntiles));
      if (ntiles) {
        copy_h2d(ctx, d_voff.get(), tile_val_off[c].data(), 8 * ntiles);
        copy_h2d(ctx, d_doff.get(), tile_def_off[c].data(), 8 * ntiles);
      }
      launch_gather_encode_strings(ctx, req.plan->tiles.get(), ntiles, req.d_perm, (const uint64_t*)dc.data.get(),
                                   dc.has_nulls ? dc.valid.get() : nullptr, d_voff.get(), d_doff.get(), out->arena.get());
      continue;
    }
    if (dc.has_nulls) {
      Buf<uint64_t> d_voff(ctx, std::max<int64_t>(1, ntiles)), d_doff(ctx, std::max<int64_t>(1, ntiles));
      if (ntiles) {
        copy_h2d(ctx, d_voff.get(), tile_val_off[c].data(), 8 * ntiles);
        copy_h2d(ctx, d_doff.get(), tile_def_off[c].data(), 8 * ntiles);
      }
      launch_gather_encode_nullable(ctx, req.plan->tiles.get(), ntiles, req.d_perm, dc.data.get(), dc.valid.get(), dc.width,
                                    d_voff.get(), d_doff.get(), out->arena.get());
      continue;
    }
    if (c == 0 && req.d_sorted_keys && (dc.type == HS_TYPE_INT32 || dc.type == HS_TYPE_INT64)) gc.sorted_keys = req.d_sorted_keys;
    launch_gather_encode(ctx, req.plan->tiles.get(), req.plan->ntiles, req.plan->seg_start.get(), req.d_perm, gc,
                         d_page_begin.get(), P, out->arena.get());
  }
  if (!stat_patches.empty()) {
    Buf<StatPatch> d_sp(ctx, stat_patches.size());
    copy_h2d(ctx, d_sp.get(), stat_patches.data(), sizeof(StatPatch) * stat_patches.size());
    launch_patch_key_stats(ctx, d_sp.get(), (int64_t)stat_patches.size(), req.d_sorted_keys, table.cols[0].type, out->arena.get());
  }
  {
    std::vector<int> dcols;
    for (int c = 0; c < ncols; c++)
      if (dicts[c].use && !table.cols[c].carried) dcols.push_back(c);
    if (carried_cols[0] >= 0) {
      DictPackArgs pa;
      memset(&pa, 0, sizeof pa);
      for (int slot = 0; slot < kMaxCarried && carried_cols[slot] >= 0; slot++) {
        const int c = carried_cols[slot];
        pa.page_value_offset[slot] = d_pvo.get() + (size_t)c * page_counter;
        pa.bw[slot] = dicts[c].bw;
        pa.ncols = slot + 1;
      }
      launch_dict_pack(ctx, req.plan->tiles.get(), ntiles, req.plan->seg_start.get(), req.d_perm, pa, 4,
                       (const uint16_t*)table.rec.get(), d_page_begin.get(), P, out->arena.get());
    }
    for (size_t b0 = 0; b0 < dcols.size(); b0 += 8) {
      DictMapArgs ma;
      DictPackArgs pa;
      memset(&ma, 0, sizeof ma);
      memset(&pa, 0, sizeof pa);
      const int nd = (int)std::min<size_t>(8, dcols.size() - b0);
      ma.ncols = pa.ncols = nd;
      for (int j = 0; j < nd; j++) {
        const int c = dcols[b0 + j];
        ma.src[j] = table.cols[c].data.get();
        ma.width[j] = table.cols[c].width;
        ma.entries[j] = dicts[c].entries.get();
        ma.mask[j] = dicts[c].mask;
        ma.empty_index[j] = dicts[c].empty_index;
        pa.page_value_offset[j] = d_pvo.get() + (size_t)c * page_counter;
        pa.bw[j] = dicts[c].bw;
      }
      Buf<uint16_t> rec(ctx, (size_t)std::max<int64_t>(1, table.nrows) * (nd <= 4 ? 4 : 8));
      launch_dict_encode_all(ctx, req.plan->tiles.get(), ntiles, req.plan->seg_start.get(), req.d_perm, ma, pa, table.nrows,
                             kDictCapacity, rec.get(), d_page_begin.get(), P, out->arena.get());
    }
  }
  if (compress && !page_plans.empty()) {
    std::vector<SnappyFragment> frags;
    std::vector<size_t> page_first_frag(page_plans.size() + 1, 0);
    uint64_t slot_cursor = 0;
    for (size_t i = 0; i < page_plans.size(); i++) {
      page_first_frag[i] = frags.size();
      const PagePlan& pp = page_plans[i];
      for (uint32_t o = 0; o < pp.body_len; o += kSnappyFragment) {
        const uint32_t len = std::min<uint32_t>(kSnappyFragment, pp.body_len - o);
        frags.push_back(SnappyFragment{pp.hdr_off + pp.hdr_len + o, slot_cursor, len, 0});
        slot_cursor += round_up(snappy_max_compressed(len), 16);
      }
    }
    page_first_frag[page_plans.size()] = frags.size();
    Buf<uint8_t> d_slots(ctx, std::max<uint64_t>(slot_cursor, 16));
    Buf<SnappyFragment> d_frags(ctx, std::max<size_t>(1, frags.size()));
    Buf<uint32_t> d_flen(ctx, std::max<size_t>(1, frags.size()));
    std::vector<uint32_t> flen(frags.size());
    copy_h2d(ctx, d_frags.get(), frags.data(), sizeof(SnappyFragment) * frags.size());
    launch_snappy_compress(ctx, d_frags.get(), (int64_t)frags.size(), out->arena.get(), d_slots.get(), d_flen.get());
    copy_d2h(ctx, flen.data(), d_flen.get(), 4 * frags.size());
    sync_stream(ctx);
    std::vector<uint8_t> skel2;
    std::vector<ByteCopy> copies2;
    std::vector<BlobCopy> blobs;
    std::vector<StatPatch> patches2;
    uint64_t cur2 = 0;
    auto emit2 = [&](size_t skel_begin) {
      copies2.push_back(ByteCopy{cur2, (uint32_t)skel_begin, (uint32_t)(skel2.size() - skel_begin)});
      cur2 += skel2.size() - skel_begin;
    };
    std::map<uint64_t, size_t> skel_at;
    for (const ByteCopy& bc : copies) skel_at[bc.dst] = bc.src;
    size_t page_i = 0;
    std::vector<OutFile> files2;
    for (size_t fi = 0; fi < file_plans.size(); fi++) {
      FilePlan& fp = file_plans[fi];
      const uint64_t file_off = round_up(cur2, 64);
      cur2 = file_off;
      {
        const size_t b0 = skel2.size();
        skel2.insert(skel2.end(), {'P', 'A', 'R', '1'});
        emit2(b0);
      }
      size_t chunk_i = 0;
      for (pq::OutRowGroup& g : fp.rgs) {
        g.file_offset = (int64_t)(cur2 - file_off);
        int64_t rg_comp = 0, rg_uncomp = 0;
        for (pq::OutChunk& ch : g.chunks) {
          const auto range = fp.chunk_pages[chunk_i++];
          const uint64_t chunk_begin = cur2;
          int64_t uncomp = 0;
          bool first_data = true;
          for (size_t pi = range.first; pi < range.first + range.second; pi++, page_i++) {
            const PagePlan& pp = page_plans[pi];
            auto it = skel_at.find(pp.hdr_off);
            if (it == skel_at.end()) fail(HS_EINVAL, "internal: page header not found in the layout");
            thrift::Reader r(skeleton.data() + it->second, skeleton.data() + it->second + pp.hdr_len);
            int32_t ptype = -1, nvals = 0, enc = 0;
            int16_t fid = 0;
            for (;;) {
              const uint8_t t = r.field(fid);
              if (r.bad || t == thrift::T_STOP) break;
              if (fid == 1) ptype = (int32_t)r.zigzag();
              else if (fid == 5 || fid == 7) {
                int16_t f2 = 0;
                for (;;) {
                  const uint8_t t2 = r.field(f2);
                  if (r.bad || t2 == thrift::T_STOP) break;
                  if (f2 == 1) nvals = (int32_t)r.zigzag();
                  else if (f2 == 2) enc = (int32_t)r.zigzag();
                  else r.skip(t2);
                }
              } else r.skip(t);
            }
            uint8_t pre[5];
            int pl = 0;
            for (uint32_t v = pp.body_len;; v >>= 7) {
              if (v >= 0x80) pre[pl++] = (uint8_t)(v | 0x80);
              else {
                pre[pl++] = (uint8_t)v;
                break;
              }
            }
            uint64_t comp = (uint64_t)pl;
            for (size_t f = page_first_frag[pi]; f < page_first_frag[pi + 1]; f++) comp += flen[f];
            if (comp >= (1ull << 31)) fail(HS_EUNSUPPORTED, "a compressed page exceeds 2 GiB");
            const size_t b0 = skel2.size();
            if (ptype == pq::DICTIONARY_PAGE) {
              ch.dictionary_page_offset = (int64_t)(cur2 - file_off);
              pq::write_dict_page_header(skel2, (int32_t)pp.body_len, nvals, (int32_t)comp);
            } else {
              if (first_data) ch.data_page_offset = (int64_t)(cur2 - file_off);
              first_data = false;
              pq::write_data_page_header(skel2, (int32_t)pp.body_len, nvals, enc, (int32_t)comp);
            }
            uncomp += (int64_t)(skel2.size() - b0) + pp.body_len;
            skel2.insert(skel2.end(), pre, pre + pl);
            emit2(b0);
            for (size_t f = page_first_frag[pi]; f < page_first_frag[pi + 1]; f++) {
              blobs.push_back(BlobCopy{frags[f].dst_off, cur2, flen[f], 0});
              cur2 += flen[f];
            }
          }
          ch.total_size = (int64_t)(cur2 - chunk_begin);
          ch.total_uncompressed = uncomp;
          ch.codec = pq::SNAPPY;
          rg_comp += ch.total_size;
          rg_uncomp += uncomp;
        }
        g.total_byte_size = rg_uncomp;
        g.total_compressed = rg_comp;
      }
      {
        const size_t b0 = skel2.size();
        std::vector<pq::StatSlot> slots;
        std::vector<uint8_t> footer = pq::write_footer(schema, fp.rgs, fp.rows, schema_json, &slots);
        for (const pq::StatSlot& sl : slots) {
          StatPatch sp;
          int64_t row0 = 0;
          for (int g = 0; g < sl.row_group; g++) row0 += fp.rgs[g].num_rows;
          sp.first_pos = req.seg_offsets[fp.seg] + (uint64_t)row0;
          sp.last_pos = sp.first_pos + (uint64_t)fp.rgs[sl.row_group].num_rows - 1;
          for (int j = 0; j < 2; j++) {
            sp.min_off[j] = cur2 + sl.min_off[j];
            sp.max_off[j] = cur2 + sl.max_off[j];
          }
          sp.width = sl.width;
          sp.pad = 0;
          patches2.push_back(sp);
        }
        skel2.insert(skel2.end(), footer.begin(), footer.end());
        const uint32_t flen32 = (uint32_t)footer.size();
        const uint8_t* lp = (const uint8_t*)&flen32;
        skel2.insert(skel2.end(), lp, lp + 4);
        skel2.insert(skel2.end(), {'P', 'A', 'R', '1'});
        emit2(b0);
      }
      OutFile of = out->files[fi];
      of.offset = file_off;
      of.size = cur2 - file_off;
      files2.push_back(std::move(of));
    }
    if (skel2.size() >= (1ull << 32)) fail(HS_EUNSUPPORTED, "index metadata exceeds 4 GiB");
    Buf<uint8_t> arena2(ctx, std::max<uint64_t>(cur2, 16) + 64);
    Buf<uint8_t> d_skel2(ctx, std::max<size_t>(1, skel2.size()));
    Buf<ByteCopy> d_copies2(ctx, std::max<size_t>(1, copies2.size()));
    Buf<BlobCopy> d_blobs(ctx, std::max<size_t>(1, blobs.size()));
    copy_h2d(ctx, d_skel2.get(), skel2.data(), skel2.size());
    copy_h2d(ctx, d_copies2.get(), copies2.data(), copies2.size() * sizeof(ByteCopy));
    copy_h2d(ctx, d_blobs.get(), blobs.data(), blobs.size() * sizeof(BlobCopy));
    launch_scatter_bytes(ctx, d_copies2.get(), (int64_t)copies2.size(), d_skel2.get(), arena2.get());
    launch_copy_blobs(ctx, d_blobs.get(), (int64_t)blobs.size(), d_slots.get(), arena2.get());
    if (!patches2.empty()) {
      Buf<StatPatch> d_sp(ctx, patches2.size());
      copy_h2d(ctx, d_sp.get(), patches2.data(), sizeof(StatPatch) * patches2.size());
      launch_patch_key_stats(ctx, d_sp.get(), (int64_t)patches2.size(), req.d_sorted_keys, table.cols[0].type, arena2.get());
    }
    sync_stream(ctx);
    out->arena = std::move(arena2);
    out->arena_bytes = cur2;
    out->files = std::move(files2);
    cursor = cur2;
  }
  t_enc.stop();
  sync_stream(ctx);
  stats->ms_plan += t_plan.ms();
  stats->ms_encode += t_enc.ms();
  stats->bytes_out += (int64_t)cursor;
  stats->files_out += (int32_t)out->files.size();
}

}
```

hyperspace_b200/csrc/engine.h:

```cpp
#pragma once
#include <memory>
#include <string>
#include <vector>

#include "hs_common.h"
#include "kernels.h"
#include "parquet_meta.h"

namespace hs {

struct DevColumn {
  std::string name;
  int32_t type = -1;
  int32_t width = 0;
  pq::SchemaColumn schema;
  Buf<uint8_t> data;
  Buf<uint8_t> valid;
  bool has_nulls = false;
  Buf<unsigned long long> dict_keys;
  uint32_t dict_state[4] = {0, 0, 0, 0};
  bool dict_ready = false;
  bool zero_copy = false;
  Buf<ZcTile> zc_tiles;
  bool carried = false;
  Buf<uint16_t> codes;
  std::vector<uint64_t> dict_values;
  uint32_t dict_bw = 0;
  int carry_slot = -1;
};

constexpr int kMaxCarried = 4;

struct Table {
  int64_t nrows = 0;
  std::vector<DevColumn> cols;
  std::vector<int64_t> file_row_begin;
  int64_t global_rows = -1;
  bool has_strings = false;
  Buf<uint8_t> rec;
};

struct CarryOptions {
  int first_col = -1;
  int num_segments = 1;
  int zc_tile_rows = 0;
  int zc_first_col = 0;
  bool zc_key = false;
};

struct DictProbe {
  int64_t mini = 0;
  Buf<uint32_t> d_states;
  std::vector<uint32_t> h_states;
  std::vector<Buf<unsigned long long>> keys;
  uint64_t queued_at = 0;
  bool delivered(const hs_ctx* ctx) const { return ctx->sync_count > queued_at; }
};

struct IndexedRows {
  Table part;
  std::vector<uint64_t> bucket_offsets;
  Buf<uint64_t> d_bucket_offsets;
  SortPlan plan;
  SortedRows sorted;
  bool have_key_bits = false;
  unsigned long long key_or_and[2] = {0, ~0ull};
  struct DeferredTimer {
    std::unique_ptr<StageTimer> t;
    float hs_stats::*field;
  };
  std::vector<DeferredTimer> pending_timers;
  std::unique_ptr<DictProbe> probe;
};

struct OutFile {
  int32_t bucket = 0;
  std::string name;
  uint64_t offset = 0;
  uint64_t size = 0;
  int64_t rows = 0;
};

struct StageTimes;

struct LoadOptions {
  const int64_t* d_row_window = nullptr;
  bool allow_missing_lineage = true;
};
void load_sources(hs_ctx* ctx, const hs_source_file* files, int n_files, const std::vector<std::string>& columns,
                  Table* out, hs_stats* stats, const CarryOptions* carry = nullptr);
struct SourceSet {
  struct Impl;
  Impl* impl;
  int n_files = 0;
  SourceSet();
  ~SourceSet();
  void release_images();
  SourceSet(const SourceSet&) = delete;
  SourceSet& operator=(const SourceSet&) = delete;
};
void open_sources(hs_ctx* ctx, const hs_source_file* files, int n_files, SourceSet* set, hs_stats* stats);
void decode_sources(hs_ctx* ctx, SourceSet& set, const std::vector<std::string>& columns,
                    const std::vector<std::pair<int64_t, int64_t>>* file_windows, Table* out, hs_stats* stats,
                    const CarryOptions* carry = nullptr);

void index_rows(hs_ctx* ctx, Table& table, int nkeys, int num_buckets, IndexedRows* out, hs_stats* stats, bool defer_settle = false);

struct EncodeRequest {
  const Table* table = nullptr;
  const uint32_t* d_perm = nullptr;
  const uint64_t* d_sorted_keys = nullptr;
  const SortPlan* plan = nullptr;
  std::vector<uint64_t> seg_offsets;
  std::vector<std::string> seg_names;
  std::vector<int32_t> seg_ids;
  int64_t rows_per_page = 0;
  int64_t rows_per_row_group = 0;
  std::vector<int64_t> seg_rows_per_row_group;
  bool use_dictionary = true;
  int codec = 0;
  DictProbe* probe = nullptr;
};
struct EncodedFiles {
  Buf<uint8_t> arena;
  uint64_t arena_bytes = 0;
  std::vector<OutFile> files;
};
void encode_segments(hs_ctx* ctx, const EncodeRequest& req, EncodedFiles* out, hs_stats* stats);

void exchange_rows(hs_ctx* ctx, Table& table, int nkeys, int num_buckets, hs_stats* stats);
void comm_destroy(hs_ctx* ctx);
void comm_allgather_host(hs_ctx* ctx, const void* in, size_t bytes, void* out);
bool p2p_exchange_supported(hs_ctx* ctx, int num_buckets);
void exchange_partition_p2p(hs_ctx* ctx, Table& table, int nkeys, int num_buckets, IndexedRows* out, hs_stats* stats);
void sort_partitioned_rows(hs_ctx* ctx, int nkeys, int num_buckets, IndexedRows* out, hs_stats* stats, bool defer_settle = false);
bool settle_sort(hs_ctx* ctx, IndexedRows* out, hs_stats* stats);
void launch_dictionary_probes(hs_ctx* ctx, const Table& part, bool use_dictionary, std::unique_ptr<DictProbe>* out);

std::string make_uuid();

}

struct hs_index_result {
  hs_ctx* ctx = nullptr;
  int output = HS_OUT_FILES;
  hs::Buf<uint8_t> d_arena;
  hs::Buf<uint8_t> h_arena;
  std::vector<hs::OutFile> files;
};

struct hs_staged {
  hs_ctx* ctx = nullptr;
  hs::Buf<uint8_t> d_images;
  std::vector<hs_source_file> files;
  std::vector<std::string> names;
  std::vector<std::shared_ptr<hs::pq::FileMeta>> metas;
  std::vector<hs::Buf<uint8_t>> staging;
  cudaEvent_t begin = nullptr, ready = nullptr;
  uint64_t bytes = 0;
};

struct hs_pending {
  hs_ctx* ctx = nullptr;
  std::unique_ptr<hs_index_result> res;
  hs_stats st;
  hs::Buf<uint8_t> d_arena;
  cudaEvent_t t_begin = nullptr, t_compute_end = nullptr, t_d2h_begin = nullptr, t_d2h_end = nullptr;
  bool has_d2h = false;
  std::string out_dir;
  int save_mode = 0;
  ~hs_pending() {
    if (getenv("HS_TIMELINE")) return;
    for (cudaEvent_t e : {t_begin, t_compute_end, t_d2h_begin, t_d2h_end})
      if (e) cudaEventDestroy(e);
  }
};

struct hs_batch {
  hs_ctx* ctx = nullptr;
  int64_t nrows = 0;
  bool on_device = false;
  struct Col {
    std::string name;
    int32_t type;
    hs::Buf<uint8_t> data;
    hs::Buf<uint8_t> valid;
    bool has_valid = false;
    hs::Buf<uint64_t> offsets;
    uint64_t total_bytes = 0;
  };
  std::vector<Col> cols;
};
```

hyperspace_b200/csrc/gather_encode.cu:

```cuda
#include "device_utils.cuh"
#include "kernels.h"

namespace hs {

namespace {

constexpr int kThreads = 256;

__device__ __forceinline__ uint64_t sort_decode_int(int type, uint64_t e) {
  return type == 1 ? (e ^ 0x8000000000000000ull) : (uint64_t)((uint32_t)e ^ 0x80000000u);
}

template <int W>
__global__ void __launch_bounds__(kThreads) k_gather_encode(const SortTile* __restrict__ tiles,
                                                             const uint64_t* __restrict__ seg_start,
                                                             const uint32_t* __restrict__ perm, GatherColumn col,
                                                             const uint32_t* __restrict__ bucket_page_begin,
                                                             int64_t rows_per_page, uint8_t* __restrict__ arena) {
  const SortTile t = tiles[blockIdx.x];
  const uint64_t lr0 = t.start - seg_start[t.seg];
  const uint64_t page = lr0 / (uint64_t)rows_per_page;
  uint8_t* const base = arena + col.page_value_offset[bucket_page_begin[t.seg] + page] + (lr0 - page * (uint64_t)rows_per_page) * W;
  const bool aligned = ((uintptr_t)base & (W - 1)) == 0;
  if (aligned && t.count == kSortTile) {
    constexpr int kPer = kSortTile / kThreads;
    uint64_t v[kPer];
    if (col.sorted_keys) {
#pragma unroll
      for (int it = 0; it < kPer; it++) v[it] = sort_decode_int(col.key_type, col.sorted_keys[t.start + it * kThreads + threadIdx.x]);
    } else {
      uint32_t r[kPer];
#pragma unroll
      for (int it = 0; it < kPer; it++) r[it] = perm[t.start + it * kThreads + threadIdx.x];
#pragma unroll
      for (int it = 0; it < kPer; it++) v[it] = W == 8 ? ((const uint64_t*)col.src)[r[it]] : ((const uint32_t*)col.src)[r[it]];
    }
#pragma unroll
    for (int it = 0; it < kPer; it++) {
      const uint32_t i = it * kThreads + threadIdx.x;
      if (W == 8) reinterpret_cast<uint64_t*>(base)[i] = v[it];
      else reinterpret_cast<uint32_t*>(base)[i] = (uint32_t)v[it];
    }
    return;
  }
  const uint32_t iters = (t.count + kThreads - 1) / kThreads;
  for (uint32_t it = 0; it < iters; it++) {
    const uint32_t i = it * kThreads + threadIdx.x;
    const bool active = i < t.count;
    uint64_t v = 0;
    if (active) {
      const uint64_t p = t.start + i;
      if (col.sorted_keys) {
        v = sort_decode_int(col.key_type, col.sorted_keys[p]);
      } else {
        const uint32_t src_row = perm[p];
        v = W == 8 ? ((const uint64_t*)col.src)[src_row] : ((const uint32_t*)col.src)[src_row];
      }
    }
    if (aligned) {
      if (active) {
        if (W == 8) reinterpret_cast<uint64_t*>(base)[i] = v;
        else reinterpret_cast<uint32_t*>(base)[i] = (uint32_t)v;
      }
    } else {
      warp_store_unaligned<W>(base + (size_t)i * W, v, active);
    }
  }
}

__global__ void __launch_bounds__(kThreads) k_tile_valid_counts(const SortTile* __restrict__ tiles,
                                                                 const uint32_t* __restrict__ perm,
                                                                 const uint8_t* __restrict__ valid,
                                                                 uint32_t* __restrict__ counts) {
  __shared__ uint32_t s_total;
  if (threadIdx.x == 0) s_total = 0;
  __syncthreads();
  const SortTile t = tiles[blockIdx.x];
  uint32_t local = 0;
  for (uint32_t i = threadIdx.x; i < t.count; i += kThreads) local += valid[perm[t.start + i]] ? 1u : 0u;
  for (int o = 16; o > 0; o >>= 1) local += __shfl_xor_sync(0xffffffffu, local, o);
  if ((threadIdx.x & 31) == 0 && local) atomicAdd(&s_total, local);
  __syncthreads();
  if (threadIdx.x == 0) counts[blockIdx.x] = s_total;
}

template <int W>
__global__ void __launch_bounds__(kThreads) k_gather_encode_nullable(const SortTile* __restrict__ tiles,
                                                                      const uint32_t* __restrict__ perm,
                                                                      const void* __restrict__ src,
                                                                      const uint8_t* __restrict__ valid,
                                                                      const uint64_t* __restrict__ tile_value_offset,
                                                                      const uint64_t* __restrict__ tile_def_offset,
                                                                      uint8_t* __restrict__ arena) {
  __shared__ uint64_t s_vals[kSortTile];
  __shared__ uint32_t warp_sums[40];
  const SortTile t = tiles[blockIdx.x];
  uint8_t* const def_out = arena + tile_def_offset[blockIdx.x];
  uint32_t base = 0;
  const uint32_t iters = (t.count + kThreads - 1) / kThreads;
  for (uint32_t it = 0; it < iters; it++) {
    const uint32_t i = it * kThreads + threadIdx.x;
    const bool active = i < t.count;
    uint32_t flag = 0;
    uint64_t v = 0;
    if (active) {
      const uint32_t row = perm[t.start + i];
      flag = valid[row] ? 1u : 0u;
      if (flag) v = W == 8 ? ((const uint64_t*)src)[row] : ((const uint32_t*)src)[row];
    }
    const unsigned bits = __ballot_sync(0xffffffffu, flag != 0);
    if ((threadIdx.x & 31) == 0) {
      const uint32_t first = it * kThreads + (threadIdx.x & ~31u);
      if (first < t.count) {
        const uint32_t nbytes = min(4u, (t.count - first + 7) / 8);
        for (uint32_t b = 0; b < nbytes; b++) def_out[first / 8 + b] = (uint8_t)(bits >> (8 * b));
      }
    }
    uint32_t total = 0;
    const uint32_t pos = block_exclusive_scan(flag, warp_sums, &total);
    if (flag) s_vals[base + pos] = v;
    base += total;
  }
  __syncthreads();
  uint8_t* const val_out = arena + tile_value_offset[blockIdx.x];
  const uint32_t viters = (base + kThreads - 1) / kThreads;
  for (uint32_t it = 0; it < viters; it++) {
    const uint32_t j = it * kThreads + threadIdx.x;
    const bool active = j < base;
    warp_store_unaligned<W>(val_out + (size_t)j * W, active ? s_vals[j] : 0, active);
  }
}

__global__ void __launch_bounds__(kThreads) k_tile_string_sizes(const SortTile* __restrict__ tiles, const uint32_t* __restrict__ perm,
                                                                 const uint64_t* __restrict__ refs,
                                                                 const uint8_t* __restrict__ valid,
                                                                 uint32_t* __restrict__ bytes, uint32_t* __restrict__ counts) {
  __shared__ uint32_t s_bytes, s_count;
  if (threadIdx.x == 0) s_bytes = s_count = 0;
  __syncthreads();
  const SortTile t = tiles[blockIdx.x];
  uint32_t b = 0, c = 0;
  for (uint32_t i = threadIdx.x; i < t.count; i += kThreads) {
    const uint32_t row = perm[t.start + i];
    if (!valid || valid[row]) {
      b += 4u + ref_len(refs[row]);
      c++;
    }
  }
  for (int o = 16; o > 0; o >>= 1) {
    b += __shfl_xor_sync(0xffffffffu, b, o);
    c += __shfl_xor_sync(0xffffffffu, c, o);
  }
  if ((threadIdx.x & 31) == 0 && c) {
    atomicAdd(&s_bytes, b);
    atomicAdd(&s_count, c);
  }
  __syncthreads();
  if (threadIdx.x == 0) {
    bytes[blockIdx.x] = s_bytes;
    counts[blockIdx.x] = s_count;
  }
}

__global__ void __launch_bounds__(kThreads) k_gather_encode_strings(const SortTile* __restrict__ tiles,
                                                                     const uint32_t* __restrict__ perm,
                                                                     const uint64_t* __restrict__ refs,
                                                                     const uint8_t* __restrict__ valid,
                                                                     const uint64_t* __restrict__ tile_value_offset,
                                                                     const uint64_t* __restrict__ tile_def_offset,
                                                                     uint8_t* __restrict__ arena) {
  __shared__ uint32_t warp_sums[40];
  const SortTile t = tiles[blockIdx.x];
  uint8_t* const def_out = arena + tile_def_offset[blockIdx.x];
  uint8_t* const val_out = arena + tile_value_offset[blockIdx.x];
  uint32_t base = 0;
  const uint32_t iters = (t.count + kThreads - 1) / kThreads;
  for (uint32_t it = 0; it < iters; it++) {
    const uint32_t i = it * kThreads + threadIdx.x;
    const bool active = i < t.count;
    uint32_t flag = 0;
    uint64_t r = 0;
    if (active) {
      const uint32_t row = perm[t.start + i];
      flag = (!valid || valid[row]) ? 1u : 0u;
      if (flag) r = refs[row];
    }
    const unsigned bits = __ballot_sync(0xffffffffu, flag != 0);
    if ((threadIdx.x & 31) == 0) {
      const uint32_t first = it * kThreads + (threadIdx.x & ~31u);
      if (first < t.count) {
        const uint32_t nbytes = min(4u, (t.count - first + 7) / 8);
        for (uint32_t b = 0; b < nbytes; b++) def_out[first / 8 + b] = (uint8_t)(bits >> (8 * b));
      }
    }
    const uint32_t len = ref_len(r), size = flag ? 4u + len : 0u;
    uint32_t total = 0;
    const uint32_t pos = block_exclusive_scan(size, warp_sums, &total);
    if (flag) {
      uint8_t* o = val_out + base + pos;
      o[0] = (uint8_t)len;
      o[1] = (uint8_t)(len >> 8);
      o[2] = (uint8_t)(len >> 16);
      o[3] = (uint8_t)(len >> 24);
      const uint8_t* src = ref_ptr(r);
      for (uint32_t b = 0; b < len; b++) o[4 + b] = src[b];
    }
    base += total;
  }
}

template <typename T>
__global__ void k_gather_plain(const T* __restrict__ src, const uint32_t* __restrict__ perm, int64_t n,
                               T* __restrict__ out) {
  const int64_t stride = (int64_t)gridDim.x * blockDim.x;
  for (int64_t i = (int64_t)blockIdx.x * blockDim.x + threadIdx.x; i < n; i += stride) out[i] = src[perm[i]];
}

__global__ void k_scatter_bytes(const ByteCopy* __restrict__ copies, int64_t n, const uint8_t* __restrict__ skeleton,
                                uint8_t* __restrict__ arena) {
  const int64_t warp = ((int64_t)blockIdx.x * blockDim.x + threadIdx.x) >> 5;
  const int lane = threadIdx.x & 31;
  if (warp >= n) return;
  const ByteCopy c = copies[warp];
  for (uint32_t i = lane; i < c.len; i += 32) arena[c.dst + i] = skeleton[c.src + i];
}

__global__ void __launch_bounds__(256) k_copy_blobs(const BlobCopy* __restrict__ blobs, const uint8_t* __restrict__ src_base,
                                                     uint8_t* __restrict__ dst_base) {
  const BlobCopy b = blobs[blockIdx.x];
  const uint8_t* src = src_base + b.src;
  uint8_t* dst = dst_base + b.dst;
  const uint32_t head = min(b.len, (uint32_t)((4 - ((uintptr_t)dst & 3)) & 3));
  for (uint32_t i = threadIdx.x; i < head; i += 256) dst[i] = src[i];
  const uint32_t nwords = (b.len - head) / 4;
  uint32_t* d32 = reinterpret_cast<uint32_t*>(dst + head);
  const uint8_t* s0 = src + head;
  for (uint32_t w = threadIdx.x; w < nwords; w += 256) d32[w] = load_le32_unaligned(s0 + 4 * (size_t)w);
  for (uint32_t i = head + 4 * nwords + threadIdx.x; i < b.len; i += 256) dst[i] = src[i];
}

__global__ void k_patch_key_stats(const StatPatch* __restrict__ patches, int64_t n, const uint64_t* __restrict__ sorted_keys,
                                  int key_type, uint8_t* __restrict__ arena) {
  const int64_t i = (int64_t)blockIdx.x * blockDim.x + threadIdx.x;
  if (i >= n) return;
  const StatPatch p = patches[i];
  const uint64_t vmin = sort_decode_int(key_type, sorted_keys[p.first_pos]);
  const uint64_t vmax = sort_decode_int(key_type, sorted_keys[p.last_pos]);
  for (int b = 0; b < p.width; b++) {
    const uint8_t lo = (uint8_t)(vmin >> (8 * b)), hi = (uint8_t)(vmax >> (8 * b));
    arena[p.min_off[0] + b] = lo;
    arena[p.min_off[1] + b] = lo;
    arena[p.max_off[0] + b] = hi;
    arena[p.max_off[1] + b] = hi;
  }
}

__device__ __forceinline__ uint64_t splitmix64(uint64_t seed, uint64_t i) {
  uint64_t z = seed + (i + 1) * 0x9E3779B97F4A7C15ull;
  z = (z ^ (z >> 30)) * 0xBF58476D1CE4E5B9ull;
  z = (z ^ (z >> 27)) * 0x94D049BB133111EBull;
  return z ^ (z >> 31);
}

__global__ void k_synth_column(int col, int64_t first_row, int64_t n, void* __restrict__ out) {
  const int64_t stride = (int64_t)gridDim.x * blockDim.x;
  for (int64_t j = (int64_t)blockIdx.x * blockDim.x + threadIdx.x; j < n; j += stride) {
    const uint64_t i = (uint64_t)(first_row + j);
    switch (col) {
      case 0: ((uint64_t*)out)[j] = splitmix64(42, i); break;
      case 1: ((int64_t*)out)[j] = (int64_t)(splitmix64(43, i) % 1000ull); break;
      case 2: ((double*)out)[j] = (double)i * 1e-3; break;
      case 3: ((int32_t*)out)[j] = (int32_t)(i % 100ull); break;
      case 4: ((float*)out)[j] = (float)(i % 4096ull) * 0.25f; break;
    }
  }
}

inline int grid_for(hs_ctx* ctx, int64_t n, int threads, int per_sm) {
  int64_t want = ceil_div(n, threads);
  int64_t cap = (int64_t)ctx->sm_count * per_sm;
  return (int)std::max<int64_t>(1, std::min(want, cap));
}

}

void launch_gather_encode(hs_ctx* ctx, const SortTile* tiles, int64_t ntiles, const uint64_t* seg_start,
                          const uint32_t* perm, const GatherColumn& col, const uint32_t* bucket_page_begin,
                          int64_t rows_per_page, uint8_t* arena) {
  KernelScope _ks(ctx, "k_gather_encode");
  if (ntiles == 0) return;
  if (col.width == 8)
    k_gather_encode<8><<<(unsigned)ntiles, kThreads, 0, ctx->stream>>>(tiles, seg_start, perm, col, bucket_page_begin,
                                                                        rows_per_page, arena);
  else if (col.width == 4)
    k_gather_encode<4><<<(unsigned)ntiles, kThreads, 0, ctx->stream>>>(tiles, seg_start, perm, col, bucket_page_begin,
                                                                        rows_per_page, arena);
  else
    fail(HS_EUNSUPPORTED, "gather_encode: column width %d", col.width);
  HS_LAUNCH_CHECK(ctx);
}

void launch_tile_valid_counts(hs_ctx* ctx, const SortTile* tiles, int64_t ntiles, const uint32_t* perm,
                              const uint8_t* valid, uint32_t* counts) {
  KernelScope _ks(ctx, "k_tile_valid_counts");
  if (ntiles == 0) return;
  k_tile_valid_counts<<<(unsigned)ntiles, kThreads, 0, ctx->stream>>>(tiles, perm, valid, counts);
  HS_LAUNCH_CHECK(ctx);
}

void launch_gather_encode_nullable(hs_ctx* ctx, const SortTile* tiles, int64_t ntiles, const uint32_t* perm,
                                   const void* src, const uint8_t* valid, int width, const uint64_t* tile_value_offset,
                                   const uint64_t* tile_def_offset, uint8_t* arena) {
  KernelScope _ks(ctx, "k_gather_encode_nullable");
  if (ntiles == 0) return;
  if (width == 8)
    k_gather_encode_nullable<8><<<(unsigned)ntiles, kThreads, 0, ctx->stream>>>(tiles, perm, src, valid, tile_value_offset,
                                                                                 tile_def_offset, arena);
  else if (width == 4)
    k_gather_encode_nullable<4><<<(unsigned)ntiles, kThreads, 0, ctx->stream>>>(tiles, perm, src, valid, tile_value_offset,
                                                                                 tile_def_offset, arena);
  else
    fail(HS_EUNSUPPORTED, "gather_encode_nullable: column width %d", width);
  HS_LAUNCH_CHECK(ctx);
}

void launch_tile_string_sizes(hs_ctx* ctx, const SortTile* tiles, int64_t ntiles, const uint32_t* perm, const uint64_t* refs,
                              const uint8_t* valid, uint32_t* bytes, uint32_t* counts) {
  KernelScope _ks(ctx, "k_tile_string_sizes");
  if (ntiles == 0) return;
  k_tile_string_sizes<<<(unsigned)ntiles, kThreads, 0, ctx->stream>>>(tiles, perm, refs, valid, bytes, counts);
  HS_LAUNCH_CHECK(ctx);
}

void launch_gather_encode_strings(hs_ctx* ctx, const SortTile* tiles, int64_t ntiles, const uint32_t* perm, const uint64_t* refs,
                                  const uint8_t* valid, const uint64_t* tile_value_offset, const uint64_t* tile_def_offset,
                                  uint8_t* arena) {
  KernelScope _ks(ctx, "k_gather_encode_strings");
  if (ntiles == 0) return;
  k_gather_encode_strings<<<(unsigned)ntiles, kThreads, 0, ctx->stream>>>(tiles, perm, refs, valid, tile_value_offset,
                                                                          tile_def_offset, arena);
  HS_LAUNCH_CHECK(ctx);
}

void launch_copy_blobs(hs_ctx* ctx, const BlobCopy* blobs, int64_t n, const uint8_t* src_base, uint8_t* dst_base) {
  KernelScope _ks(ctx, "k_copy_blobs");
  if (n == 0) return;
  k_copy_blobs<<<(unsigned)n, 256, 0, ctx->stream>>>(blobs, src_base, dst_base);
  HS_LAUNCH_CHECK(ctx);
}

void launch_gather_plain(hs_ctx* ctx, const void* src, const uint32_t* perm, int64_t n, int width, void* out) {
  KernelScope _ks(ctx, "k_gather_plain");
  if (n == 0) return;
  const int grid = grid_for(ctx, n, 256, 16);
  switch (width) {
    case 8: k_gather_plain<uint64_t><<<grid, 256, 0, ctx->stream>>>((const uint64_t*)src, perm, n, (uint64_t*)out); break;
    case 4: k_gather_plain<uint32_t><<<grid, 256, 0, ctx->stream>>>((const uint32_t*)src, perm, n, (uint32_t*)out); break;
    case 1: k_gather_plain<uint8_t><<<grid, 256, 0, ctx->stream>>>((const uint8_t*)src, perm, n, (uint8_t*)out); break;
    default: fail(HS_EINVAL, "gather: unsupported width %d", width);
  }
  HS_LAUNCH_CHECK(ctx);
}

void launch_scatter_bytes(hs_ctx* ctx, const ByteCopy* copies, int64_t n, const uint8_t* skeleton, uint8_t* arena) {
  if (n == 0) return;
  const int64_t threads = n * 32;
  k_scatter_bytes<<<(unsigned)ceil_div(threads, 256), 256, 0, ctx->stream>>>(copies, n, skeleton, arena);
  HS_LAUNCH_CHECK(ctx);
}

void launch_patch_key_stats(hs_ctx* ctx, const StatPatch* patches, int64_t n, const uint64_t* sorted_keys, int key_type,
                            uint8_t* arena) {
  if (n == 0) return;
  k_patch_key_stats<<<(unsigned)ceil_div(n, 128), 128, 0, ctx->stream>>>(patches, n, sorted_keys, key_type, arena);
  HS_LAUNCH_CHECK(ctx);
}

void launch_synth_column(hs_ctx* ctx, int col, int64_t first_row, int64_t n, void* out) {
  KernelScope _ks(ctx, "k_synth_column");
  if (n == 0) return;
  k_synth_column<<<grid_for(ctx, n, 256, 16), 256, 0, ctx->stream>>>(col, first_row, n, out);
  HS_LAUNCH_CHECK(ctx);
}

}
```

hyperspace_b200/csrc/kernels.h:

```cpp
#pragma once
#include "hs_common.h"

namespace hs {

struct ChunkDesc {
  const uint8_t* data;
  uint64_t size;
  int64_t num_values;
  int64_t row_base;
  int32_t col;
  int32_t phys_type;
  int32_t max_def;
  int32_t file_index;
  int32_t codec;
  int32_t pad;
};

struct PageDesc {
  const uint8_t* data;
  const uint8_t* dict;
  int64_t first_row;
  int32_t dict_count;
  int32_t size;
  int32_t num_values;
  int32_t encoding;
  int32_t page_type;
  int32_t def_bytes;
  int32_t rep_bytes;
  int32_t col, phys_type, max_def;
  int32_t file_index;
  int32_t uncompressed_size;
  int32_t dict_size, dict_uncompressed_size;
  int32_t is_compressed;
  int32_t codec;
  int32_t chunk;
};

struct ColumnOut {
  void* data;
  uint8_t* valid;
  int32_t width;
  int32_t type;
  const void* carry_entries;
  uint32_t carry_mask;
  uint32_t carry_empty_index;
  int32_t carry;
  int32_t skip;
};

enum : uint32_t { PAGECLASS_NOT_DICT = 1u, PAGECLASS_MAYBE_NULLS = 2u, PAGECLASS_NOT_IN_PLACE = 4u };
void launch_classify_pages(hs_ctx* ctx, const PageDesc* pages, int64_t n_pages, uint32_t* col_flags, int zc_tile_rows);
struct ZcTile {
  const uint8_t* p0;
  const uint8_t* p1;
  int64_t split;
};
void launch_fill_zc_tiles(hs_ctx* ctx, const PageDesc* pages, int64_t n_pages, ZcTile* const* tile_src, int zc_tile_rows,
                          int64_t nrows);

enum DecodeError : uint32_t {
  DERR_NONE = 0, DERR_BAD_HEADER = 1, DERR_UNSUPPORTED_ENCODING = 2, DERR_VALUE_COUNT = 3, DERR_COMPRESSED = 4,
  DERR_OVERRUN = 5, DERR_DICT_INDEX = 6, DERR_UNSUPPORTED_TYPE = 7, DERR_SNAPPY = 8, DERR_STRING_TOO_LONG = 9
};
struct StringDictJob {
  const uint8_t* page;
  uint64_t* refs;
  int32_t size, count;
};
void launch_build_string_dicts(hs_ctx* ctx, const StringDictJob* jobs, int64_t n, uint32_t* d_error);

struct SnappyBlob {
  const uint8_t* src;
  uint64_t dst_off;
  uint32_t src_len;
  uint32_t dst_len;
  uint32_t prefix;
  uint32_t compressed;
  uint32_t first_block;
  uint32_t pad;
};
__host__ __device__ inline uint32_t snappy_blocks_of(uint32_t dst_len, uint32_t prefix) {
  const uint32_t body = dst_len - prefix;
  return body == 0 ? 1u : (body + 65535u) / 65536u;
}
void launch_snappy_decompress(hs_ctx* ctx, const SnappyBlob* blobs, int64_t n, int64_t total_blocks, bool any_verbatim,
                              uint32_t* block_in, uint32_t* sequential, uint8_t* scratch, uint32_t* d_error);

struct SnappyFragment {
  uint64_t src_off, dst_off;
  uint32_t len, pad;
};
constexpr uint32_t kSnappyFragment = 65536;
inline uint64_t snappy_max_compressed(uint64_t len) { return 32 + len + len / 6; }
void launch_snappy_compress(hs_ctx* ctx, const SnappyFragment* frags, int64_t n, const uint8_t* raw, uint8_t* scratch,
                            uint32_t* out_len);

void launch_walk_pages(hs_ctx* ctx, const ChunkDesc* chunks, int n_chunks, int32_t* page_counts,
                       const int64_t* page_offsets, PageDesc* pages, uint32_t* d_error, int mode);
void launch_decode_pages(hs_ctx* ctx, const PageDesc* pages, int64_t n_pages, const ColumnOut* cols,
                         uint32_t* col_has_nulls, const int64_t* row_window, uint32_t* d_error);

struct KeyColumn {
  const void* data;
  const uint8_t* valid;
  int32_t type;
  int32_t width;
  const ZcTile* tiles = nullptr;
};

constexpr int kPartTile = 4096;
constexpr int kMaxBuckets = 4096;

void launch_bucket_hist(hs_ctx* ctx, const KeyColumn* d_keys, int nkeys, int64_t nrows, int num_buckets,
                        uint16_t* bucket, uint32_t* tile_hist, unsigned long long* global_hist);
void launch_owner_hist(hs_ctx* ctx, const KeyColumn* d_keys, int nkeys, int64_t nrows, int num_buckets, int world,
                       uint16_t* owner, uint32_t* tile_hist, unsigned long long* global_hist);
void launch_tile_offsets(hs_ctx* ctx, uint32_t* tile_hist, int64_t ntiles, int num_buckets,
                         const unsigned long long* global_hist, unsigned long long* bucket_offsets ,
                         const unsigned long long* explicit_base = nullptr);
void launch_partition_dest(hs_ctx* ctx, const uint16_t* bucket, int64_t nrows, int num_buckets,
                           const uint32_t* tile_offsets, uint32_t* dest);
void launch_scatter_column(hs_ctx* ctx, const void* in, void* out, const uint32_t* dest, int64_t nrows, int width);
constexpr int kFusedTileLocal = 4096;
constexpr int kFusedTilePeer = 8192;
int fused_tile_rows(bool peer_tiles);
constexpr int kFusedMaxBins = 1024;
struct PartColumn {
  const void* in;
  void* out;
  int32_t width;
  int32_t pad;
  const ZcTile* tiles = nullptr;
};
bool fused_partition_supported(int nbins);
void launch_tile_hist(hs_ctx* ctx, const KeyColumn* d_keys, int nkeys, int64_t nrows, int num_buckets, int owner_mod,
                      uint32_t* tile_hist, unsigned long long* global_hist,
                      unsigned long long* key_or_and = nullptr, int single_key_type = -1, uint16_t* bin_ids = nullptr,
                      bool peer_tiles = false);
inline int single_key_type_of(const KeyColumn* h_keys, int nkeys) {
  return nkeys == 1 && h_keys[0].valid == nullptr && (h_keys[0].type == 0 || h_keys[0].type == 1) ? h_keys[0].type : -1;
}
struct CodePackRound {
  const uint16_t* src[4];
  void* out;
  int32_t n;
  int32_t pad;
};
void launch_partition_rows(hs_ctx* ctx, const KeyColumn* d_keys, int nkeys, int64_t nrows, int num_buckets, int owner_mod,
                           const uint32_t* tile_dst, const PartColumn* d_cols, int ncols, void* const* d_peer_out = nullptr,
                           int out_world = 1, int single_key_type = -1, const CodePackRound* pack = nullptr,
                           const uint16_t* bin_ids = nullptr);
void launch_encode_keys(hs_ctx* ctx, const void* in, int type, const uint32_t* src, int64_t nrows, uint64_t* out,
                        unsigned long long* or_and);
void launch_iota_u32(hs_ctx* ctx, uint32_t* out, int64_t n);
void launch_string_piece_keys(hs_ctx* ctx, const uint64_t* refs, const uint32_t* perm, int64_t nrows, int piece, uint64_t* out,
                              unsigned long long* or_and);

constexpr int kSortTile = 4096;
struct SortTile {
  uint32_t seg;
  uint32_t count;
  uint64_t start;
};
struct SortChunk;
struct SortPlan {
  int64_t n = 0;
  int64_t ntiles = 0;
  int32_t nseg = 0;
  Buf<SortTile> tiles;
  Buf<uint32_t> seg_tile_begin;
  Buf<uint64_t> seg_start;
  Buf<uint32_t> tile_hist;
  Buf<uint32_t> tile_dst;
  std::vector<uint32_t> h_seg_tile_begin;
  std::vector<uint64_t> h_seg_start;
  int64_t nchunks = 0;
  Buf<SortChunk> chunks;
  Buf<uint32_t> seg_chunk_begin;
  Buf<uint32_t> chunk_sums;
};
void build_sort_plan(hs_ctx* ctx, const uint64_t* seg_offsets, int nseg, SortPlan* plan);
struct SortedRows {
  Buf<uint64_t> keys_buf[2];
  Buf<uint32_t> perm_buf[2];
  int cur = 0;
  uint64_t* keys() const { return keys_buf[cur].get(); }
  uint32_t* perm() const { return perm_buf[cur].get(); }
  bool queued = false;
  uint64_t resort_bits = 0, queued_at = 0;
  uint32_t gave_up = 0;
};
void sort_rows(hs_ctx* ctx, SortPlan* plan, const KeyColumn* cols, int ncols, const unsigned long long* last_or_and,
               bool may_defer, SortedRows* out);
bool settle_sorted_rows(hs_ctx* ctx, SortPlan* plan, SortedRows* s);

struct GatherColumn {
  const void* src;
  const uint64_t* sorted_keys;
  int32_t key_type;
  int32_t width;
  const uint64_t* page_value_offset;
};
void launch_gather_encode(hs_ctx* ctx, const SortTile* tiles, int64_t ntiles, const uint64_t* seg_start,
                          const uint32_t* perm, const GatherColumn& col, const uint32_t* bucket_page_begin,
                          int64_t rows_per_page, uint8_t* arena);
void launch_tile_valid_counts(hs_ctx* ctx, const SortTile* tiles, int64_t ntiles, const uint32_t* perm,
                              const uint8_t* valid, uint32_t* counts);
void launch_gather_encode_nullable(hs_ctx* ctx, const SortTile* tiles, int64_t ntiles, const uint32_t* perm,
                                   const void* src, const uint8_t* valid, int width, const uint64_t* tile_value_offset,
                                   const uint64_t* tile_def_offset, uint8_t* arena);
void launch_tile_string_sizes(hs_ctx* ctx, const SortTile* tiles, int64_t ntiles, const uint32_t* perm, const uint64_t* refs,
                              const uint8_t* valid, uint32_t* bytes, uint32_t* counts);
void launch_gather_encode_strings(hs_ctx* ctx, const SortTile* tiles, int64_t ntiles, const uint32_t* perm, const uint64_t* refs,
                                  const uint8_t* valid, const uint64_t* tile_value_offset, const uint64_t* tile_def_offset,
                                  uint8_t* arena);
constexpr uint32_t kMaxDictEntries = 65536;
constexpr uint32_t kDictCapacity = 8 * kMaxDictEntries;
void launch_dict_build(hs_ctx* ctx, const void* src, int width, int64_t begin, int64_t end, unsigned long long* keys,
                       uint32_t capacity, uint32_t max_distinct, uint32_t* state);
void launch_dict_build_from_pages(hs_ctx* ctx, const PageDesc* pages, int64_t n_pages, int col, int width,
                                  unsigned long long* keys, uint32_t capacity, uint32_t max_distinct, uint32_t* state);
void launch_dict_collect(hs_ctx* ctx, const unsigned long long* keys, uint32_t capacity, unsigned long long* out,
                         uint32_t* counter, uint32_t max_out = 0xffffffffu);
struct DictMapArgs {
  const void* src[8];
  const void* entries[8];
  uint32_t mask[8];
  uint32_t empty_index[8];
  int32_t width[8];
  int32_t ncols;
};
struct DictPackArgs {
  const uint64_t* page_value_offset[8];
  uint32_t bw[8];
  int32_t ncols;
};
void launch_dict_pack(hs_ctx* ctx, const SortTile* tiles, int64_t ntiles, const uint64_t* seg_start, const uint32_t* perm,
                      const DictPackArgs& pack_args, int slots, const uint16_t* rec, const uint32_t* bucket_page_begin,
                      int64_t rows_per_page, uint8_t* arena);
void launch_dict_encode_all(hs_ctx* ctx, const SortTile* tiles, int64_t ntiles, const uint64_t* seg_start, const uint32_t* perm,
                            const DictMapArgs& map_args, const DictPackArgs& pack_args, int64_t nrows, uint32_t capacity,
                            uint16_t* rec_scratch, const uint32_t* bucket_page_begin, int64_t rows_per_page, uint8_t* arena);
void launch_gather_plain(hs_ctx* ctx, const void* src, const uint32_t* perm, int64_t n, int width, void* out);
struct StatPatch {
  uint64_t first_pos, last_pos;
  uint64_t min_off[2], max_off[2];
  int32_t width, pad;
};
void launch_patch_key_stats(hs_ctx* ctx, const StatPatch* patches, int64_t n, const uint64_t* sorted_keys, int key_type,
                            uint8_t* arena);
struct ByteCopy {
  uint64_t dst;
  uint32_t src;
  uint32_t len;
};
void launch_scatter_bytes(hs_ctx* ctx, const ByteCopy* copies, int64_t n, const uint8_t* skeleton, uint8_t* arena);
struct BlobCopy {
  uint64_t src, dst;
  uint32_t len, pad;
};
void launch_copy_blobs(hs_ctx* ctx, const BlobCopy* blobs, int64_t n, const uint8_t* src_base, uint8_t* dst_base);
void launch_synth_column(hs_ctx* ctx, int col, int64_t first_row, int64_t n, void* out);

constexpr int kMaxPredicates = 16;
constexpr int kMaxJoinKeys = 8;
struct PredRange {
  int32_t type;
  int32_t has_lo, has_hi, lo_strict, hi_strict;
  uint64_t lo, hi;
};
struct PredDesc {
  const void* data;
  const uint8_t* valid;
  PredRange r;
};
struct PredSet {
  PredDesc p[kMaxPredicates + kMaxJoinKeys];
  int n = 0;
};
void launch_range_bounds(hs_ctx* ctx, const void* keys, const PredRange& r, const uint64_t* seg_offsets, int nseg,
                         int64_t* bounds);
void launch_predicate_mask(hs_ctx* ctx, const PredSet& preds, const uint32_t* cand, int64_t n, uint32_t* mask);
void launch_join_count(hs_ctx* ctx, const int64_t* lkeys, const uint64_t* lseg, const int64_t* rkeys,
                       const uint64_t* rseg, int nseg, int64_t nl, uint32_t* counts, uint32_t* first_match, bool string_keys = false);
struct JoinKeyCols {
  const uint64_t* col[kMaxJoinKeys];
  int32_t n;
  uint32_t str_mask;
};
void launch_join_count_keys(hs_ctx* ctx, const JoinKeyCols& lkeys, const uint64_t* lseg, const JoinKeyCols& rkeys,
                            const uint64_t* rseg, int nseg, int64_t nl, uint32_t* counts, uint32_t* first_match);
void launch_join_emit(hs_ctx* ctx, const uint32_t* counts, const uint32_t* first_match, const uint64_t* out_offsets,
                      int64_t nl, uint32_t* out_li, uint32_t* out_ri);
void exclusive_scan_u32_u64(hs_ctx* ctx, const uint32_t* in, int64_t n, uint64_t* out);
void launch_string_lengths(hs_ctx* ctx, const uint64_t* refs, const uint8_t* valid, const uint32_t* idx, int64_t n,
                           uint32_t* lens);
void launch_copy_strings(hs_ctx* ctx, const uint64_t* refs, const uint8_t* valid, const uint32_t* idx, int64_t n,
                         const uint64_t* offsets, uint8_t* out);
void launch_compact_indices(hs_ctx* ctx, const uint32_t* mask, const uint64_t* offsets, int64_t n, const uint32_t* cand,
                            uint32_t* out_idx);
void launch_not_in_mask(hs_ctx* ctx, const int64_t* file_ids, int64_t n, const int64_t* deleted, int ndeleted,
                        uint32_t* mask );

}
```

hyperspace_b200/csrc/radix_sort.cu:

```cuda
#include <cmath>

#include "device_utils.cuh"
#include "kernels.h"

namespace hs {

struct SortChunk {
  uint32_t seg;
  uint32_t tile_begin, tile_end;
};

namespace {

constexpr int kThreads = 512;
constexpr int kWarps = kThreads / 32;
constexpr int kItems = kSortTile / kThreads;
constexpr int kWarpRows = kSortTile / kWarps;
constexpr int kChunkTiles = 128;
constexpr int kHistThreads = 256;

struct DigitShift {
  int shift;
  __device__ __forceinline__ uint32_t operator()(uint64_t key, uint32_t) const { return (uint32_t)(key >> shift) & 255u; }
};
// ... 5 lines not shown
struct SrcPairs {
  const uint64_t* __restrict__ keys;
  const uint32_t* __restrict__ vals;
  __device__ __forceinline__ void load(uint64_t p, uint64_t& k, uint32_t& v) const {
    k = keys[p];
    v = vals[p];
  }
};
template <int TYPE>
struct SrcRaw {
  const void* __restrict__ raw;
  __device__ __forceinline__ void load(uint64_t p, uint64_t& k, uint32_t& v) const {
    const uint64_t r = (TYPE == HS_TYPE_INT64 || TYPE == HS_TYPE_DOUBLE) ? ((const uint64_t*)raw)[p]
                                                                          : (uint64_t)((const uint32_t*)raw)[p];
    k = sort_encode(TYPE, r);
    v = (uint32_t)p;
  }
};

template <typename Src, typename Digit>
__global__ void __launch_bounds__(kHistThreads) k_sort_hist(const SortTile* __restrict__ tiles, Src src, Digit digit,
                                                         uint32_t* __restrict__ tile_hist) {
  __shared__ uint32_t s_hist[256];
  s_hist[threadIdx.x] = 0;
  __syncthreads();
  const SortTile t = tiles[blockIdx.x];
  for (uint32_t i = threadIdx.x; i < t.count; i += kHistThreads) {
    uint64_t k;
    uint32_t v;
    src.load(t.start + i, k, v);
    atomicAdd(&s_hist[digit(k, v)], 1u);
  }
  __syncthreads();
  tile_hist[(size_t)blockIdx.x * 256 + threadIdx.x] = s_hist[threadIdx.x];
}

__global__ void __launch_bounds__(256) k_seg_chunk_sums(const SortChunk* __restrict__ chunks,
                                                         const uint32_t* __restrict__ tile_hist,
                                                         uint32_t* __restrict__ chunk_sums) {
  const SortChunk c = chunks[blockIdx.x];
  uint32_t s = 0;
  for (uint32_t t = c.tile_begin; t < c.tile_end; t++) s += tile_hist[(size_t)t * 256 + threadIdx.x];
  chunk_sums[(size_t)blockIdx.x * 256 + threadIdx.x] = s;
}

__global__ void __launch_bounds__(256) k_seg_scan(const uint32_t* __restrict__ seg_chunk_begin,
                                                   const uint64_t* __restrict__ seg_start,
                                                   uint32_t* __restrict__ chunk_sums, uint32_t* __restrict__ digit_base) {
  __shared__ uint32_t warp_sums[40];
  const uint32_t seg = blockIdx.x;
  const uint32_t c0 = seg_chunk_begin[seg], c1 = seg_chunk_begin[seg + 1];
  uint32_t tot = 0;
  for (uint32_t c = c0; c < c1; c++) {
    const uint32_t v = chunk_sums[(size_t)c * 256 + threadIdx.x];
    chunk_sums[(size_t)c * 256 + threadIdx.x] = tot;
    tot += v;
  }
  const uint32_t dbase = block_exclusive_scan(tot, warp_sums, nullptr) + (uint32_t)seg_start[seg];
  if (digit_base) digit_base[(size_t)seg * 256 + threadIdx.x] = dbase;
  for (uint32_t c = c0; c < c1; c++) chunk_sums[(size_t)c * 256 + threadIdx.x] += dbase;
}

__global__ void __launch_bounds__(1024) k_seg_apply(const SortChunk* __restrict__ chunks,
                                                     const uint32_t* __restrict__ tile_hist,
                                                     uint32_t* __restrict__ tile_dst,
                                                     const uint32_t* __restrict__ chunk_sums) {
  __shared__ uint32_t s_group[4][256];
  const SortChunk c = chunks[blockIdx.x];
  const uint32_t d = threadIdx.x & 255, g = threadIdx.x >> 8;
  const uint32_t n = c.tile_end - c.tile_begin;
  const uint32_t per = (n + 3) / 4;
  const uint32_t t0 = c.tile_begin + min(g * per, n), t1 = c.tile_begin + min((g + 1) * per, n);
  uint32_t s = 0;
#pragma unroll 8
  for (uint32_t t = t0; t < t1; t++) s += tile_hist[(size_t)t * 256 + d];
  s_group[g][d] = s;
  __syncthreads();
  uint32_t run = chunk_sums[(size_t)blockIdx.x * 256 + d];
  for (uint32_t gg = 0; gg < g; gg++) run += s_group[gg][d];
#pragma unroll 8
  for (uint32_t t = t0; t < t1; t++) {
    const uint32_t v = tile_hist[(size_t)t * 256 + d];
    tile_dst[(size_t)t * 256 + d] = run;
    run += v;
  }
}

template <int W, int I, bool kGuard, typename Bin>
__device__ __forceinline__ uint32_t rank_tile(uint16_t (&cnt)[W][256], uint32_t* warp_sums, Bin bin, uint32_t count,
                                              uint32_t (&rank)[I]) {
  const uint32_t warp = threadIdx.x >> 5, lane = threadIdx.x & 31;
  const unsigned lt = (1u << lane) - 1;
  uint16_t* wcnt = cnt[warp];
#pragma unroll
  for (int j = 0; j < I; j++) {
    rank[j] = 0;
    if (!kGuard || warp * (I * 32) + j * 32 < count) {
      const uint32_t b = bin(j);
      const unsigned peers = match_any_full<8>(b);
      const uint32_t before = __popc(peers & lt);
      const uint32_t pre = wcnt[b];
      __syncwarp();
      if (before == 0) wcnt[b] = (uint16_t)(pre + __popc(peers));
      __syncwarp();
      rank[j] = pre + before;
    }
  }
  __syncthreads();
  uint32_t total = 0;
  if (threadIdx.x < 256) {
#pragma unroll
    for (int w = 0; w < W; w++) total += cnt[w][threadIdx.x];
  }
  const uint32_t start = block_exclusive_scan(total, warp_sums, nullptr);
  if (threadIdx.x < 256) {
    uint32_t run = start;
#pragma unroll
    for (int w = 0; w < W; w++) {
      const uint16_t c = cnt[w][threadIdx.x];
      cnt[w][threadIdx.x] = (uint16_t)run;
      run += c;
    }
  }
  return start;
}

struct ScatterShared {
  uint64_t keys[kSortTile];
  uint32_t vals[kSortTile];
  uint16_t cnt[kWarps][256];
  uint32_t out_adj[256];
  uint32_t warp_sums[40];
};

template <typename Src, typename Digit>
__global__ void __launch_bounds__(kThreads, 2) k_sort_scatter(const SortTile* __restrict__ tiles, Src src, Digit digit,
                                                               const uint32_t* __restrict__ tile_dst,
                                                               uint64_t* __restrict__ out_keys,
                                                               uint32_t* __restrict__ out_vals) {
  extern __shared__ __align__(16) uint8_t smem_raw[];
  ScatterShared& sm = *reinterpret_cast<ScatterShared*>(smem_raw);
  const uint32_t warp = threadIdx.x >> 5, lane = threadIdx.x & 31;
  {
    uint32_t* z = reinterpret_cast<uint32_t*>(&sm.cnt[0][0]);
#pragma unroll
    for (int i = 0; i < kWarps * 256 / 2 / kThreads; i++) z[threadIdx.x + i * kThreads] = 0;
  }
  const SortTile t = tiles[blockIdx.x];
  uint32_t dst0 = 0;
  if (threadIdx.x < 256) dst0 = tile_dst[(size_t)blockIdx.x * 256 + threadIdx.x];
  const uint32_t first = warp * kWarpRows + lane;
  const uint64_t p0 = t.start + first;
  uint64_t k[kItems];
  uint32_t v[kItems];
  uint32_t bin[kItems];
#pragma unroll
  for (int j = 0; j < kItems; j++) {
    const bool a = first + j * 32 < t.count;
    k[j] = ~0ull;
    v[j] = 0;
    if (a) src.load(p0 + j * 32, k[j], v[j]);
    bin[j] = a ? digit(k[j], v[j]) : 255u;
  }
  __syncthreads();
  uint32_t rank[kItems];
  const uint32_t start = rank_tile<kWarps, kItems, false>(sm.cnt, sm.warp_sums, [&](int j) { return bin[j]; }, 0, rank);
  if (threadIdx.x < 256) sm.out_adj[threadIdx.x] = dst0 - start;
  __syncthreads();
  const uint16_t* cnt = sm.cnt[warp];
#pragma unroll
  for (int j = 0; j < kItems; j++) {
    const uint32_t pos = cnt[bin[j]] + rank[j];
    sm.keys[pos] = k[j];
    sm.vals[pos] = v[j];
  }
  __syncthreads();
#pragma unroll
  for (int j = 0; j < kItems; j++) {
    const uint32_t i = threadIdx.x + j * kThreads;
    if (i < t.count) {
      const uint64_t key = sm.keys[i];
      const uint32_t val = sm.vals[i];
      const uint32_t dst = sm.out_adj[digit(key, val)] + i;
      out_keys[dst] = key;
      out_vals[dst] = val;
    }
  }
}

constexpr uint32_t kFixMaxRun = 64;
__global__ void __launch_bounds__(256) k_fix_runs(const SortTile* __restrict__ tiles, const uint64_t* __restrict__ seg_start,
                                                   uint64_t* __restrict__ keys, uint32_t* __restrict__ vals,
                                                   uint64_t high_mask, uint64_t low_mask, uint32_t max_run,
                                                   uint32_t* __restrict__ flag) {
  __shared__ uint64_t s_key[kSortTile + 2];
  __shared__ uint16_t s_heads[kSortTile / 2], s_len[kSortTile / 2];
  const SortTile t = tiles[blockIdx.x];
  const uint64_t segb = seg_start[t.seg], sege = seg_start[t.seg + 1];
  const unsigned lane = threadIdx.x & 31, lt = (1u << lane) - 1;
  constexpr int kPer = kSortTile / 256;
  {
    uint64_t k[kPer];
#pragma unroll
    for (int j = 0; j < kPer; j++) {
      const uint32_t i = j * 256 + threadIdx.x;
      k[j] = i < t.count ? keys[t.start + i] : 0;
    }
#pragma unroll
    for (int j = 0; j < kPer; j++) s_key[1 + j * 256 + threadIdx.x] = k[j];
  }
  __syncthreads();
  if (threadIdx.x == 0) {
    const uint64_t flip = high_mask & (~high_mask + 1);
    s_key[0] = t.start > segb ? keys[t.start - 1] : (s_key[1] ^ flip);
    s_key[t.count + 1] = t.start + t.count < sege ? keys[t.start + t.count] : (s_key[t.count] ^ flip);
  }
  __syncthreads();
  const uint32_t wid = threadIdx.x >> 5;
  uint16_t* my_heads = s_heads + wid * (kSortTile / 16);
  uint16_t* my_len = s_len + wid * (kSortTile / 16);
  uint32_t my_n = 0;
#pragma unroll 4
  for (uint32_t i0 = 0; i0 < kSortTile; i0 += 256) {
    const uint32_t i = i0 + threadIdx.x;
    bool head = false;
    if (i < t.count) {
      const uint64_t kh = s_key[1 + i] & high_mask;
      head = (s_key[i] & high_mask) != kh && (s_key[2 + i] & high_mask) == kh;
    }
    const unsigned m = __ballot_sync(0xffffffffu, head);
    if (head) my_heads[my_n + __popc(m & lt)] = (uint16_t)i;
    my_n += __popc(m);
  }
  __syncwarp();
  for (uint32_t e = lane; e < my_n; e += 32) {
    const uint32_t i = my_heads[e];
    const uint64_t* sk = s_key + 1 + i;
    const uint64_t kh = sk[0] & high_mask;
    uint32_t len = 1;
    while (i + len < t.count && len <= max_run && (sk[len] & high_mask) == kh) len++;
    const bool crosses = i + len == t.count && (sk[len] & high_mask) == kh;
    my_len[e] = crosses ? (uint16_t)0xffffu : (uint16_t)len;
  }
  __syncthreads();
  for (uint32_t e = lane; e < my_n; e += 32) {
    const uint32_t i = my_heads[e];
    const uint64_t p = t.start + i;
    uint64_t* sk = s_key + 1 + i;
    const uint64_t kh = sk[0] & high_mask;
    uint32_t len = my_len[e];
    if (len == 0xffffu) {
      len = t.count - i;
      uint64_t q = p + len;
      while (q < sege && q - p <= max_run && (keys[q] & high_mask) == kh) q++;
      const uint32_t glen = (uint32_t)(q - p);
      if (glen > max_run) {
        *flag = 1;
        continue;
      }
      for (uint32_t a = 1; a < glen; a++) {
        const uint64_t ka = keys[p + a];
        const uint32_t va = vals[p + a];
        const uint64_t la = ka & low_mask;
        uint32_t b = a;
        while (b > 0 && (keys[p + b - 1] & low_mask) > la) {
          keys[p + b] = keys[p + b - 1];
          vals[p + b] = vals[p + b - 1];
          b--;
        }
        if (b != a) {
          keys[p + b] = ka;
          vals[p + b] = va;
        }
      }
      continue;
    }
    if (len > max_run) {
      *flag = 1;
      continue;
    }
    for (uint32_t a = 1; a < len; a++) {
      const uint64_t ka = sk[a];
      const uint64_t la = ka & low_mask;
      uint32_t b = a;
      while (b > 0 && (sk[b - 1] & low_mask) > la) b--;
      if (b == a) continue;
      const uint32_t va = vals[p + a];
      for (uint32_t c = a; c > b; c--) {
        const uint64_t kc = sk[c - 1];
        sk[c] = kc;
        keys[p + c] = kc;
        vals[p + c] = vals[p + c - 1];
      }
      sk[b] = ka;
      keys[p + b] = ka;
      vals[p + b] = va;
    }
  }
}

constexpr int kLocalSortCap = 12288;
struct LocalSortItem {
  uint32_t start, count;
};
constexpr int kLocalThreads = 1024;
constexpr int kLocalWarps = kLocalThreads / 32;
constexpr int kLocalItems = kLocalSortCap / kLocalThreads;
constexpr int kLocalWarpRows = kLocalSortCap / kLocalWarps;
constexpr uint32_t kLocalMaxRun = 64;
static_assert(kLocalSortCap % kLocalThreads == 0 && kLocalSortCap <= 65536, "slot numbers are 16-bit");

struct LocalShared {
  uint64_t keys[kLocalSortCap];
  uint32_t vals[kLocalSortCap];
  uint16_t slot[kLocalSortCap];
  uint16_t cnt[kLocalWarps][256];
  uint32_t warp_sums[40];
  unsigned long long or_bits, and_bits;
  uint32_t long_run;
};

__device__ __forceinline__ void local_pass(LocalShared& sm, uint32_t count, int shift) {
  const uint32_t warp = threadIdx.x >> 5, lane = threadIdx.x & 31;
  {
    uint32_t* z = reinterpret_cast<uint32_t*>(&sm.cnt[0][0]);
#pragma unroll
    for (int i = 0; i < kLocalWarps * 256 / 2 / kLocalThreads; i++) z[threadIdx.x + i * kLocalThreads] = 0;
  }
  const uint32_t first = warp * kLocalWarpRows + lane;
  uint32_t slot_bin[kLocalItems], rank[kLocalItems];
#pragma unroll
  for (int j = 0; j < kLocalItems; j++) {
    const uint32_t pos = first + j * 32;
    const uint32_t s = pos < count ? sm.slot[pos] : pos;
    slot_bin[j] = s << 8 | (pos < count ? (uint32_t)(sm.keys[s] >> shift) & 255u : 255u);
  }
  __syncthreads();
  rank_tile<kLocalWarps, kLocalItems, true>(sm.cnt, sm.warp_sums, [&](int j) { return slot_bin[j] & 255u; }, count, rank);
  __syncthreads();
  const uint16_t* cnt = sm.cnt[warp];
#pragma unroll
  for (int j = 0; j < kLocalItems; j++)
    if (warp * kLocalWarpRows + j * 32 < count) sm.slot[cnt[slot_bin[j] & 255u] + rank[j]] = (uint16_t)(slot_bin[j] >> 8);
  __syncthreads();
}

template <typename Src>
__global__ void __launch_bounds__(kLocalThreads, 1) k_local_sort(const LocalSortItem* __restrict__ items, Src src,
                                                                 uint64_t* __restrict__ out_keys,
                                                                 uint32_t* __restrict__ out_vals) {
  extern __shared__ __align__(16) uint8_t smem_raw[];
  LocalShared& sm = *reinterpret_cast<LocalShared*>(smem_raw);
  const LocalSortItem it = items[blockIdx.x];
  const uint32_t count = it.count;
  if (threadIdx.x == 0) {
    sm.or_bits = 0;
    sm.and_bits = ~0ull;
    sm.long_run = 0;
  }
  uint64_t k_or = 0, k_and = ~0ull;
  constexpr int kHalf = kLocalItems / 2;
#pragma unroll 1
  for (int h = 0; h < 2; h++) {
    uint64_t k[kHalf];
    uint32_t v[kHalf];
#pragma unroll
    for (int j = 0; j < kHalf; j++) {
      const uint32_t i = (h * kHalf + j) * kLocalThreads + threadIdx.x;
      if (i < count) src.load((uint64_t)it.start + i, k[j], v[j]);
    }
#pragma unroll
    for (int j = 0; j < kHalf; j++) {
      const uint32_t i = (h * kHalf + j) * kLocalThreads + threadIdx.x;
      if (i < count) {
        sm.keys[i] = k[j];
        sm.vals[i] = v[j];
        sm.slot[i] = (uint16_t)i;
        k_or |= k[j];
        k_and &= k[j];
      }
    }
  }
#pragma unroll
  for (int o = 16; o > 0; o >>= 1) {
    k_or |= __shfl_xor_sync(0xffffffffu, k_or, o);
    k_and &= __shfl_xor_sync(0xffffffffu, k_and, o);
  }
  __syncthreads();
  if ((threadIdx.x & 31) == 0) {
    atomicOr(&sm.or_bits, k_or);
    atomicAnd(&sm.and_bits, k_and);
  }
  __syncthreads();
  const uint64_t varying = sm.or_bits ^ sm.and_bits;
  if (varying != 0) {
    const int top = 63 - __clzll((long long)varying);
    int pbits = 1;
    while ((1u << pbits) < 2 * count) pbits++;
    const int ndig = (min(pbits, top + 1) + 7) / 8;
    const int low = max(0, top + 1 - 8 * ndig);
    for (int d = ndig - 1; d >= 0; d--) {
      const int shift = max(0, top + 1 - 8 * (d + 1));
      if ((varying >> shift) & 0xff) local_pass(sm, count, shift);
    }
    const uint64_t high_mask = ~0ull << low;
    if (varying & ~high_mask) {
      for (uint32_t i = threadIdx.x; i < count; i += kLocalThreads) {
        const uint64_t kh = sm.keys[sm.slot[i]] & high_mask;
        if (i > 0 && (sm.keys[sm.slot[i - 1]] & high_mask) == kh) continue;
        if (i + 1 >= count || (sm.keys[sm.slot[i + 1]] & high_mask) != kh) continue;
        uint32_t len = 2;
        while (i + len < count && len <= kLocalMaxRun && (sm.keys[sm.slot[i + len]] & high_mask) == kh) len++;
        if (len > kLocalMaxRun) {
          sm.long_run = 1;
          continue;
        }
        uint16_t* s = sm.slot + i;
        for (uint32_t a = 1; a < len; a++) {
          const uint16_t sa = s[a];
          const uint64_t ka = sm.keys[sa];
          uint32_t b = a;
          while (b > 0 && sm.keys[s[b - 1]] > ka) {
            s[b] = s[b - 1];
            b--;
          }
          s[b] = sa;
        }
      }
      __syncthreads();
      if (sm.long_run) {
        for (uint32_t i = threadIdx.x; i < count; i += kLocalThreads) sm.slot[i] = (uint16_t)i;
        __syncthreads();
        for (int shift = 0; shift < 64; shift += 8)
          if ((varying >> shift) & 0xff) local_pass(sm, count, shift);
      }
    }
  }
  __syncthreads();
#pragma unroll
  for (int j = 0; j < kLocalItems; j++) {
    const uint32_t i = j * kLocalThreads + threadIdx.x;
    if (i < count) {
      const uint32_t s = sm.slot[i];
      out_keys[(uint64_t)it.start + i] = sm.keys[s];
      out_vals[(uint64_t)it.start + i] = sm.vals[s];
    }
  }
}

template <typename Src>
void launch_local_sort(hs_ctx* ctx, const std::vector<LocalSortItem>& items, Src src, uint64_t* out_keys,
                       uint32_t* out_vals) {
  if (items.empty()) return;
  Buf<LocalSortItem> d_items(ctx, items.size());
  copy_h2d(ctx, d_items.get(), items.data(), items.size() * sizeof(LocalSortItem));
  static DeviceOnce attr_once;
  bool& attr = attr_once(ctx->device);
  if (!attr) {
    HS_CUDA(cudaFuncSetAttribute(k_local_sort<Src>, cudaFuncAttributeMaxDynamicSharedMemorySize, (int)sizeof(LocalShared)));
    attr = true;
  }
  KernelScope _ks(ctx, "k_local_sort");
  k_local_sort<Src><<<(unsigned)items.size(), kLocalThreads, sizeof(LocalShared), ctx->stream>>>(d_items.get(), src,
                                                                                                 out_keys, out_vals);
  HS_LAUNCH_CHECK(ctx);
}

template <typename Src, typename Digit>
void run_hist(hs_ctx* ctx, SortPlan* plan, Src src, Digit digit, uint32_t* digit_base) {
  {
    KernelScope _ks(ctx, "k_sort_hist");
    k_sort_hist<Src, Digit><<<(unsigned)plan->ntiles, kHistThreads, 0, ctx->stream>>>(plan->tiles.get(), src, digit,
                                                                                 plan->tile_hist.get());
    HS_LAUNCH_CHECK(ctx);
  }
  KernelScope _ks(ctx, "k_seg_scan");
  k_seg_chunk_sums<<<(unsigned)plan->nchunks, 256, 0, ctx->stream>>>(plan->chunks.get(), plan->tile_hist.get(),
                                                                     plan->chunk_sums.get());
  HS_LAUNCH_CHECK(ctx);
  k_seg_scan<<<(unsigned)plan->nseg, 256, 0, ctx->stream>>>(plan->seg_chunk_begin.get(), plan->seg_start.get(),
                                                            plan->chunk_sums.get(), digit_base);
  HS_LAUNCH_CHECK(ctx);
}

template <typename Src, typename Digit>
void run_scatter(hs_ctx* ctx, SortPlan* plan, Src src, Digit digit, uint64_t* out_keys, uint32_t* out_vals) {
  {
    KernelScope _ks(ctx, "k_seg_scan");
    k_seg_apply<<<(unsigned)plan->nchunks, 1024, 0, ctx->stream>>>(plan->chunks.get(), plan->tile_hist.get(),
                                                                   plan->tile_dst.get(), plan->chunk_sums.get());
    HS_LAUNCH_CHECK(ctx);
  }
  static DeviceOnce attr_once;
  bool& attr = attr_once(ctx->device);
  if (!attr) {
    HS_CUDA(cudaFuncSetAttribute(k_sort_scatter<Src, Digit>, cudaFuncAttributeMaxDynamicSharedMemorySize,
                                 (int)sizeof(ScatterShared)));
    attr = true;
  }
  KernelScope _ks(ctx, "k_sort_scatter");
  k_sort_scatter<Src, Digit><<<(unsigned)plan->ntiles, kThreads, sizeof(ScatterShared), ctx->stream>>>(
      plan->tiles.get(), src, digit, plan->tile_dst.get(), out_keys, out_vals);
  HS_LAUNCH_CHECK(ctx);
}

template <typename Src, typename Digit>
void run_pass(hs_ctx* ctx, SortPlan* plan, Src src, Digit digit, SortedRows* s) {
  run_hist(ctx, plan, src, digit, nullptr);
  run_scatter(ctx, plan, src, digit, s->keys_buf[s->cur ^ 1].get(), s->perm_buf[s->cur ^ 1].get());
  s->cur ^= 1;
}

template <typename F>
void with_raw_source(const KeyColumn& raw, F&& f) {
  switch (raw.type) {
    case HS_TYPE_INT32: f(SrcRaw<HS_TYPE_INT32>{raw.data}); break;
    case HS_TYPE_INT64: f(SrcRaw<HS_TYPE_INT64>{raw.data}); break;
    case HS_TYPE_FLOAT: f(SrcRaw<HS_TYPE_FLOAT>{raw.data}); break;
    case HS_TYPE_DOUBLE: f(SrcRaw<HS_TYPE_DOUBLE>{raw.data}); break;
    default: fail(HS_EUNSUPPORTED, "sort: key type %d", raw.type);
  }
}

void lsd_passes(hs_ctx* ctx, SortPlan* plan, SortedRows* s, uint64_t bits, const KeyColumn* raw) {
  if (plan->ntiles == 0) return;
  bool first = raw != nullptr;
  for (int pass = 0; pass < 8; pass++) {
    if (((bits >> (pass * 8)) & 0xff) == 0) continue;
    const DigitShift digit{pass * 8};
    if (first)
      with_raw_source(*raw, [&](auto src) { run_pass(ctx, plan, src, digit, s); });
    else
      run_pass(ctx, plan, SrcPairs{s->keys(), s->perm()}, digit, s);
    first = false;
  }
  if (first) fail(HS_EINVAL, "sort: raw first-pass source given but no pass ran");
}

void local_sort_segments(hs_ctx* ctx, const SortPlan& plan, const KeyColumn& raw, SortedRows* s) {
  std::vector<LocalSortItem> items;
  for (int g = 0; g < plan.nseg; g++) {
    const uint64_t n = plan.h_seg_start[g + 1] - plan.h_seg_start[g];
    if (n) items.push_back(LocalSortItem{(uint32_t)plan.h_seg_start[g], (uint32_t)n});
  }
  with_raw_source(raw, [&](auto src) { launch_local_sort(ctx, items, src, s->keys(), s->perm()); });
}

bool msd_local_sort(hs_ctx* ctx, SortPlan* plan, const KeyColumn& raw, int shift, SortedRows* s) {
  if (plan->ntiles == 0) return false;
  const size_t nsub = (size_t)plan->nseg * 256;
  Buf<uint32_t> d_base(ctx, nsub);
  const DigitShift digit{shift};
  with_raw_source(raw, [&](auto src) { run_hist(ctx, plan, src, digit, d_base.get()); });
  std::vector<uint32_t> base(nsub + 1);
  copy_d2h(ctx, base.data(), d_base.get(), nsub * 4);
  sync_stream(ctx);
  base[nsub] = (uint32_t)plan->n;
  std::vector<LocalSortItem> items;
  for (int g = 0; g < plan->nseg; g++) {
    LocalSortItem cur{base[(size_t)g * 256], 0};
    for (size_t d = (size_t)g * 256; d < (size_t)(g + 1) * 256; d++) {
      const uint32_t sz = base[d + 1] - base[d];
      if (sz > (uint32_t)kLocalSortCap) return false;
      if (cur.count + sz > (uint32_t)kLocalSortCap) {
        items.push_back(cur);
        cur = LocalSortItem{base[d], 0};
      }
      cur.count += sz;
    }
    if (cur.count) items.push_back(cur);
  }
  uint64_t* keys_alt = s->keys_buf[s->cur ^ 1].get();
  uint32_t* perm_alt = s->perm_buf[s->cur ^ 1].get();
  with_raw_source(raw, [&](auto src) { run_scatter(ctx, plan, src, digit, keys_alt, perm_alt); });
  launch_local_sort(ctx, items, SrcPairs{keys_alt, perm_alt}, s->keys(), s->perm());
  return true;
}

}

__global__ void k_build_tiles(const uint64_t* __restrict__ seg_start, const uint32_t* __restrict__ seg_tile_begin,
                              SortTile* __restrict__ tiles) {
  const uint32_t s = blockIdx.x;
  const uint64_t b = seg_start[s], e = seg_start[s + 1];
  const uint32_t t0 = seg_tile_begin[s], nt = seg_tile_begin[s + 1] - t0;
  for (uint32_t i = threadIdx.x; i < nt; i += blockDim.x) {
    const uint64_t p = b + (uint64_t)i * kSortTile;
    tiles[t0 + i] = SortTile{s, (uint32_t)min((uint64_t)kSortTile, e - p), p};
  }
}

void build_sort_plan(hs_ctx* ctx, const uint64_t* seg_offsets, int nseg, SortPlan* plan) {
  std::vector<uint32_t> stb(nseg + 1), scb(nseg + 1);
  std::vector<uint64_t> sstart(nseg + 1);
  std::vector<SortChunk> chunks;
  uint64_t ntiles = 0;
  for (int s = 0; s < nseg; s++) {
    stb[s] = (uint32_t)ntiles;
    sstart[s] = seg_offsets[s];
    ntiles += ceil_div(seg_offsets[s + 1] - seg_offsets[s], (uint64_t)kSortTile);
    scb[s] = (uint32_t)chunks.size();
    for (uint32_t t = stb[s]; t < ntiles; t += kChunkTiles)
      chunks.push_back(SortChunk{(uint32_t)s, t, (uint32_t)std::min<uint64_t>(t + kChunkTiles, ntiles)});
  }
  stb[nseg] = (uint32_t)ntiles;
  sstart[nseg] = seg_offsets[nseg];
  scb[nseg] = (uint32_t)chunks.size();
  if (seg_offsets[nseg] >= (1ull << 32)) fail(HS_EUNSUPPORTED, "more than 2^32-1 rows per GPU per call");
  plan->n = (int64_t)seg_offsets[nseg];
  plan->ntiles = (int64_t)ntiles;
  plan->nseg = nseg;
  plan->nchunks = (int64_t)chunks.size();
  plan->tiles.alloc(ctx, std::max<size_t>(1, ntiles));
  plan->seg_tile_begin.alloc(ctx, stb.size());
  plan->seg_start.alloc(ctx, sstart.size());
  plan->tile_hist.alloc(ctx, std::max<size_t>(1, ntiles) * 256);
  plan->tile_dst.alloc(ctx, std::max<size_t>(1, ntiles) * 256);
  plan->chunks.alloc(ctx, std::max<size_t>(1, chunks.size()));
  plan->seg_chunk_begin.alloc(ctx, scb.size());
  plan->chunk_sums.alloc(ctx, std::max<size_t>(1, chunks.size()) * 256);
  copy_h2d(ctx, plan->seg_tile_begin.get(), stb.data(), stb.size() * 4);
  copy_h2d(ctx, plan->seg_start.get(), sstart.data(), sstart.size() * 8);
  if (!chunks.empty()) copy_h2d(ctx, plan->chunks.get(), chunks.data(), chunks.size() * sizeof(SortChunk));
  copy_h2d(ctx, plan->seg_chunk_begin.get(), scb.data(), scb.size() * 4);
  if (nseg > 0 && ntiles > 0) {
    k_build_tiles<<<nseg, 256, 0, ctx->stream>>>(plan->seg_start.get(), plan->seg_tile_begin.get(), plan->tiles.get());
    HS_LAUNCH_CHECK(ctx);
  }
  plan->h_seg_tile_begin = std::move(stb);
  plan->h_seg_start = std::move(sstart);
}

void sort_rows(hs_ctx* ctx, SortPlan* plan, const KeyColumn* cols, int ncols, const unsigned long long* last_or_and,
               bool may_defer, SortedRows* out) {
  const int64_t nrows = plan->n;
  for (auto& b : out->keys_buf) b.alloc(ctx, std::max<int64_t>(1, nrows));
  for (auto& b : out->perm_buf) b.alloc(ctx, std::max<int64_t>(1, nrows));
  out->cur = 0;
  out->queued = false;
  out->resort_bits = 0;
  Buf<unsigned long long> d_or_and(ctx, 2);
  unsigned long long or_and[2] = {0, 0};
  auto reduce = [&](auto launch) {
    const unsigned long long init[2] = {0ull, ~0ull};
    copy_h2d(ctx, d_or_and.get(), init, sizeof init);
    launch(d_or_and.get());
    copy_d2h(ctx, or_and, d_or_and.get(), sizeof or_and);
    sync_stream(ctx);
  };
  uint64_t max_seg = 1;
  for (int g = 0; g < plan->nseg; g++) max_seg = std::max<uint64_t>(max_seg, plan->h_seg_start[g + 1] - plan->h_seg_start[g]);
  int want_bytes = 2;
  while (want_bytes < 8 && (double)max_seg / std::pow(256.0, want_bytes) > 0.5) want_bytes++;
  const bool lsd_only = getenv("HS_LSD_SORT") != nullptr;
  for (int k = ncols - 1; k >= 0; k--) {
    const KeyColumn& kc = cols[k];
    const bool from_raw = k == ncols - 1 && kc.type >= HS_TYPE_INT32 && kc.type <= HS_TYPE_DOUBLE;
    if (k == ncols - 1 && !from_raw) launch_iota_u32(ctx, out->perm(), nrows);
    if (kc.type == HS_TYPE_STRING) {
      auto sort_piece = [&](int piece) {
        reduce([&](unsigned long long* d) {
          launch_string_piece_keys(ctx, (const uint64_t*)kc.data, out->perm(), nrows, piece, out->keys(), d);
        });
        lsd_passes(ctx, plan, out, or_and[0] ^ or_and[1], nullptr);
      };
      sort_piece(-1);
      const unsigned long long len_or = or_and[0];
      for (int piece = (int)((len_or + 7) / 8) - 1; piece >= 0; piece--) sort_piece(piece);
    } else {
      if (from_raw && last_or_and) {
        or_and[0] = last_or_and[0];
        or_and[1] = last_or_and[1];
      } else {
        reduce([&](unsigned long long* d) {
          launch_encode_keys(ctx, kc.data, kc.type, from_raw ? nullptr : out->perm(), nrows, from_raw ? nullptr : out->keys(), d);
        });
      }
      const uint64_t varying = nrows ? (or_and[0] ^ or_and[1]) : 0;
      int nbytes = 0, lowest_high_byte = 0;
      for (int b = 7, seen = 0; b >= 0; b--)
        if ((varying >> (8 * b)) & 0xff) {
          nbytes++;
          if (++seen == want_bytes) lowest_high_byte = b;
        }
      const KeyColumn* raw = from_raw ? &kc : nullptr;
      if (from_raw && varying == 0) {
        launch_iota_u32(ctx, out->perm(), nrows);
        launch_encode_keys(ctx, kc.data, kc.type, nullptr, nrows, out->keys(), d_or_and.get());
        raw = nullptr;
      }
      const bool defer = may_defer && ncols == 1 && !kc.valid;
      bool local = false;
      if (raw && !kc.valid && !lsd_only) {
        if (max_seg <= (uint64_t)kLocalSortCap) {
          local_sort_segments(ctx, *plan, kc, out);
          local = true;
        } else if (nbytes > 2 && max_seg <= (uint64_t)(0.85 * 256 * kLocalSortCap)) {
          local = msd_local_sort(ctx, plan, kc, std::max(0, 63 - __builtin_clzll(varying) - 7), out);
        }
      }
      if (local) {
        out->queued = defer;
      } else if (nbytes > want_bytes) {
        const uint64_t high_mask = ~0ull << (8 * lowest_high_byte);
        lsd_passes(ctx, plan, out, varying & high_mask, raw);
        Buf<uint32_t> d_gave_up(ctx, 1);
        fill_bytes(ctx, d_gave_up.get(), 0, 4);
        {
          KernelScope _ks(ctx, "k_fix_runs");
          k_fix_runs<<<(unsigned)plan->ntiles, 256, 0, ctx->stream>>>(plan->tiles.get(), plan->seg_start.get(), out->keys(),
                                                                      out->perm(), high_mask, ~high_mask, kFixMaxRun,
                                                                      d_gave_up.get());
          HS_LAUNCH_CHECK(ctx);
        }
        out->gave_up = 0;
        out->resort_bits = varying;
        out->queued_at = ctx->sync_count;
        out->queued = true;
        copy_d2h(ctx, &out->gave_up, d_gave_up.get(), 4);
        if (!defer) settle_sorted_rows(ctx, plan, out);
      } else {
        lsd_passes(ctx, plan, out, varying, raw);
      }
    }
    if (kc.valid && plan->ntiles)
      run_pass(ctx, plan, SrcPairs{out->keys(), out->perm()}, DigitTable{kc.valid}, out);
  }
}

bool settle_sorted_rows(hs_ctx* ctx, SortPlan* plan, SortedRows* s) {
  const uint64_t bits = s->resort_bits;
  s->queued = false;
  s->resort_bits = 0;
  if (bits == 0) return false;
  if (ctx->sync_count <= s->queued_at) sync_stream(ctx);
  if (!s->gave_up) return false;
  lsd_passes(ctx, plan, s, bits, nullptr);
  return true;
}

}
```

Baseline: 8.021 billion.

## Write sorted int key column straight into Parquet pages from local sort

Splits encoding into a layout step and a write step so the page layout can be computed before sorting. The local sort kernel then decodes the sorted int32/int64 keys and stores them directly into their final arena page positions, which avoids writing a sorted-keys buffer and a later gather-encode pass for the key column. Key statistics are now patched using the permutation and the raw column instead of the sorted-keys buffer. This adds complexity around when the layout runs relative to the sort, and it needs fallbacks for nulls, strings and dictionary columns.

```diff
diff --git a/hyperspace_b200/csrc/api.cu b/hyperspace_b200/csrc/api.cu
--- a/hyperspace_b200/csrc/api.cu
+++ b/hyperspace_b200/csrc/api.cu
@@ -588,21 +588,10 @@
       if (spec->lineage) fill_lineage(ctx, table, spec->files, spec->n_files);
       if (spec->n_deleted_file_ids > 0) drop_deleted_rows(ctx, table, spec->deleted_file_ids, spec->n_deleted_file_ids);
       IndexedRows rows;
-      if (p2p_exchange_supported(ctx, spec->num_buckets)) {
-        exchange_partition_p2p(ctx, table, spec->n_indexed, spec->num_buckets, &rows, &st);
-        sort_partitioned_rows(ctx, spec->n_indexed, spec->num_buckets, &rows, &st, true);
-      } else {
-        if (ctx->world > 1) exchange_rows(ctx, table, spec->n_indexed, spec->num_buckets, &st);
-        index_rows(ctx, table, spec->n_indexed, spec->num_buckets, &rows, &st, true);
-      }
-      if (!has_strings) src.release_images();
-
       EncodeRequest req;
       req.table = &rows.part;
-      req.d_perm = rows.sorted.perm();
-      req.d_sorted_keys = rows.sorted.keys();
+      req.key_sorted = true;
       req.plan = &rows.plan;
-      req.seg_offsets = rows.bucket_offsets;
       req.rows_per_page = spec->rows_per_page;
       req.rows_per_row_group = spec->rows_per_row_group;
       req.use_dictionary = spec->disable_dictionary == 0;
@@ -616,8 +605,30 @@
         snprintf(nm, sizeof nm, "part-%05d-%s_%05d.c000%s.parquet", b, uuid.c_str(), b, req.codec == pq::SNAPPY ? ".snappy" : "");
         req.seg_names[b] = nm;
       }
-      req.probe = rows.probe.get();
-      encode_segments(ctx, req, &enc, &st);
+      EncodeLayout lay;
+      const KeyPagesFn layout_before_sort = [&]() -> const KeyPageDest* {
+        if (layout_needs_sorted_rows(rows.part)) return nullptr;
+        req.seg_offsets = rows.bucket_offsets;
+        req.probe = rows.probe.get();
+        layout_segments(ctx, req, &lay, &enc, &st);
+        return key_page_dest(lay, req, &enc);
+      };
+      if (p2p_exchange_supported(ctx, spec->num_buckets)) {
+        exchange_partition_p2p(ctx, table, spec->n_indexed, spec->num_buckets, &rows, &st);
+        sort_partitioned_rows(ctx, spec->n_indexed, spec->num_buckets, &rows, &st, true, &layout_before_sort);
+      } else {
+        if (ctx->world > 1) exchange_rows(ctx, table, spec->n_indexed, spec->num_buckets, &st);
+        index_rows(ctx, table, spec->n_indexed, spec->num_buckets, &rows, &st, true, &layout_before_sort);
+      }
+      if (!has_strings) src.release_images();
+      req.d_perm = rows.sorted.perm();
+      if (!rows.sorted.key_pages_written) req.d_sorted_keys = rows.sorted.keys();
+      if (!lay.impl) {
+        req.seg_offsets = rows.bucket_offsets;
+        req.probe = rows.probe.get();
+        layout_segments(ctx, req, &lay, &enc, &st);
+      }
+      write_segments(ctx, req, lay, rows.sorted.key_pages_written, &enc, &st);
       if (settle_sort(ctx, &rows, &st)) {
         req.probe = nullptr;
         req.d_perm = rows.sorted.perm();
diff --git a/hyperspace_b200/csrc/device_utils.cuh b/hyperspace_b200/csrc/device_utils.cuh
--- a/hyperspace_b200/csrc/device_utils.cuh
+++ b/hyperspace_b200/csrc/device_utils.cuh
@@ -118,6 +118,9 @@
     case 4: return (raw & 0xff) ? 1 : 0;
   }
   return raw;
+}
+__device__ __forceinline__ uint64_t sort_decode_int(int type, uint64_t e) {
+  return type == 1 ? (e ^ 0x8000000000000000ull) : (uint64_t)((uint32_t)e ^ 0x80000000u);
 }
 
 HS_HD uint32_t dict_hash_u64(uint64_t v) { return (uint32_t)((v * 0x9E3779B97F4A7C15ull) >> 32); }
diff --git a/hyperspace_b200/csrc/engine.cu b/hyperspace_b200/csrc/engine.cu
--- a/hyperspace_b200/csrc/engine.cu
+++ b/hyperspace_b200/csrc/engine.cu
@@ -762,7 +762,8 @@
 }
 
 
-void index_rows(hs_ctx* ctx, Table& table, int nkeys, int num_buckets, IndexedRows* out, hs_stats* stats, bool defer_settle) {
+void index_rows(hs_ctx* ctx, Table& table, int nkeys, int num_buckets, IndexedRows* out, hs_stats* stats, bool defer_settle,
+                const KeyPagesFn* key_pages) {
   const int64_t nrows = table.nrows;
   const int ncols = (int)table.cols.size();
   if (num_buckets < 1 || num_buckets > kMaxBuckets)
@@ -867,10 +868,11 @@
 
   stats->ms_hash += t_hash.ms();
   stats->ms_partition += t_part.ms();
-  sort_partitioned_rows(ctx, nkeys, num_buckets, out, stats, defer_settle);
-}
-
-void sort_partitioned_rows(hs_ctx* ctx, int nkeys, int num_buckets, IndexedRows* out, hs_stats* stats, bool defer_settle) {
+  sort_partitioned_rows(ctx, nkeys, num_buckets, out, stats, defer_settle, key_pages);
+}
+
+void sort_partitioned_rows(hs_ctx* ctx, int nkeys, int num_buckets, IndexedRows* out, hs_stats* stats, bool defer_settle,
+                           const KeyPagesFn* key_pages) {
   auto t_sort = std::make_unique<StageTimer>(ctx);
   if (defer_settle && !out->probe) {
     launch_dictionary_probes(ctx, out->part, true, &out->probe);
@@ -883,7 +885,8 @@
     const DevColumn& c = out->part.cols[k];
     keys[k] = KeyColumn{c.data.get(), c.has_nulls ? c.valid.get() : nullptr, c.type, c.width};
   }
-  sort_rows(ctx, &out->plan, keys.data(), nkeys, out->have_key_bits ? out->key_or_and : nullptr, defer_settle, &out->sorted);
+  sort_rows(ctx, &out->plan, keys.data(), nkeys, out->have_key_bits ? out->key_or_and : nullptr, defer_settle, &out->sorted,
+            key_pages);
   t_sort->stop();
   if (out->sorted.queued) {
     out->pending_timers.push_back(IndexedRows::DeferredTimer{std::move(t_sort), &hs_stats::ms_sort});
@@ -937,20 +940,94 @@
 }
 
 
+namespace {
+
+struct ColDict {
+  bool use = false;
+  uint32_t bw = 0, ndict = 0, empty_index = 0, mask = 0;
+  Buf<unsigned long long> keys;
+  const unsigned long long* keys_ptr = nullptr;
+  Buf<uint8_t> entries;
+  size_t skel_off = 0, skel_len = 0;
+  std::vector<uint64_t> values;
+};
+struct PagePlan {
+  uint64_t hdr_off;
+  uint32_t hdr_len;
+  uint32_t body_len;
+};
+struct FilePlan {
+  int seg = 0;
+  int64_t rows = 0;
+  std::vector<pq::OutRowGroup> rgs;
+  std::vector<std::pair<size_t, size_t>> chunk_pages;
+};
+
+}
+
+struct EncodeLayout::Impl {
+  explicit Impl(hs_ctx* ctx) : t_plan(ctx) {}
+  StageTimer t_plan;
+  int64_t P = 0;
+  std::vector<pq::SchemaColumn> schema;
+  std::string schema_json;
+  std::vector<std::vector<uint64_t>> tile_val_off, tile_def_off;
+  std::vector<ColDict> dicts;
+  std::vector<int> carried_cols;
+  std::vector<StatPatch> stat_patches;
+  std::vector<uint8_t> skeleton;
+  std::vector<ByteCopy> copies;
+  bool compress = false;
+  std::vector<PagePlan> page_plans;
+  std::vector<FilePlan> file_plans;
+  uint64_t cursor = 0;
+  uint32_t page_counter = 0;
+  Buf<uint8_t> d_skel;
+  Buf<ByteCopy> d_copies;
+  Buf<uint32_t> d_page_begin;
+  Buf<uint64_t> d_pvo;
+  KeyPageDest key_dest{};
+};
+
+bool layout_needs_sorted_rows(const Table& table) {
+  for (const DevColumn& dc : table.cols)
+    if (dc.has_nulls || dc.type == HS_TYPE_STRING) return true;
+  return false;
+}
+
 void encode_segments(hs_ctx* ctx, const EncodeRequest& req, EncodedFiles* out, hs_stats* stats) {
+  EncodeLayout lay;
+  layout_segments(ctx, req, &lay, out, stats);
+  write_segments(ctx, req, lay, false, out, stats);
+}
+
+const KeyPageDest* key_page_dest(EncodeLayout& lay, const EncodeRequest& req, EncodedFiles* out) {
+  EncodeLayout::Impl& L = *lay.impl;
+  const DevColumn& dc = req.table->cols[0];
+  if (dc.has_nulls || L.dicts[0].use || (dc.type != HS_TYPE_INT32 && dc.type != HS_TYPE_INT64) || L.P > (int64_t)UINT32_MAX)
+    return nullptr;
+  L.key_dest = KeyPageDest{out->arena.get(), L.d_page_begin.get(), L.d_pvo.get(), (uint32_t)L.P, dc.width, dc.type};
+  return &L.key_dest;
+}
+
+void layout_segments(hs_ctx* ctx, const EncodeRequest& req, EncodeLayout* lay, EncodedFiles* out, hs_stats* stats) {
+  (void)stats;
+  lay->impl = std::make_shared<EncodeLayout::Impl>(ctx);
+  EncodeLayout::Impl& L = *lay->impl;
   const Table& table = *req.table;
   const int ncols = (int)table.cols.size();
   const int nseg = (int)req.seg_offsets.size() - 1;
   int64_t P = req.rows_per_page > 0 ? req.rows_per_page : 131072;
   P = (int64_t)round_up((size_t)P, kSortTile);
-  StageTimer t_plan(ctx), t_enc(ctx);
-  t_plan.start();
+  L.P = P;
+  L.t_plan.start();
   for (int c = 0; c < ncols; c++) {
     const DevColumn& dc = table.cols[c];
     if (dc.width != 4 && dc.width != 8)
       fail(HS_EUNSUPPORTED, "column '%s': %d-byte values cannot be written by the GPU encoder yet", dc.name.c_str(), dc.width);
   }
-  std::vector<pq::SchemaColumn> schema(ncols);
+  std::vector<pq::SchemaColumn>& schema = L.schema;
+  schema.resize(ncols);
   for (int c = 0; c < ncols; c++) {
     schema[c] = table.cols[c].schema;
     schema[c].repetition = pq::OPTIONAL;
@@ -963,11 +1040,15 @@
       case HS_TYPE_STRING: schema[c].type = pq::BYTE_ARRAY; break;
     }
   }
-  const std::string schema_json = pq::spark_schema_json(schema);
+  L.schema_json = pq::spark_schema_json(schema);
+  const std::string& schema_json = L.schema_json;
 
   const int64_t ntiles = req.plan->ntiles;
   std::vector<std::vector<uint32_t>> tile_valid(ncols), tile_bytes(ncols);
-  std::vector<std::vector<uint64_t>> tile_val_off(ncols), tile_def_off(ncols);
+  std::vector<std::vector<uint64_t>>& tile_val_off = L.tile_val_off;
+  std::vector<std::vector<uint64_t>>& tile_def_off = L.tile_def_off;
+  tile_val_off.resize(ncols);
+  tile_def_off.resize(ncols);
   {
     std::vector<Buf<uint32_t>> d_counts(ncols), d_bytes(ncols);
     bool any = false;
@@ -1002,18 +1083,11 @@
   }
   const std::vector<uint32_t>& seg_tile_begin = req.plan->h_seg_tile_begin;
 
-  struct ColDict {
-    bool use = false;
-    uint32_t bw = 0, ndict = 0, empty_index = 0, mask = 0;
-    Buf<unsigned long long> keys;
-    const unsigned long long* keys_ptr = nullptr;
-    Buf<uint8_t> entries;
-    size_t skel_off = 0, skel_len = 0;
-    std::vector<uint64_t> values;
-  };
-  std::vector<ColDict> dicts(ncols);
+  std::vector<ColDict>& dicts = L.dicts;
+  dicts.resize(ncols);
   const int64_t total_rows = table.nrows;
-  std::vector<int> carried_cols(kMaxCarried, -1);
+  std::vector<int>& carried_cols = L.carried_cols;
+  carried_cols.assign(kMaxCarried, -1);
   for (int c = 0; c < ncols; c++) {
     const DevColumn& dc = table.cols[c];
     if (!dc.carried) continue;
@@ -1100,25 +1174,15 @@
     }
   }
 
-  const bool stats_on_key = req.d_sorted_keys != nullptr && !table.cols[0].has_nulls &&
+  const bool stats_on_key = req.key_sorted && !table.cols[0].has_nulls &&
                             (table.cols[0].type == HS_TYPE_INT32 || table.cols[0].type == HS_TYPE_INT64);
-  std::vector<StatPatch> stat_patches;
-  std::vector<uint8_t> skeleton;
-  std::vector<ByteCopy> copies;
-  struct PagePlan {
-    uint64_t hdr_off;
-    uint32_t hdr_len;
-    uint32_t body_len;
-  };
-  struct FilePlan {
-    int seg = 0;
-    int64_t rows = 0;
-    std::vector<pq::OutRowGroup> rgs;
-    std::vector<std::pair<size_t, size_t>> chunk_pages;
-  };
-  const bool compress = req.codec == pq::SNAPPY;
-  std::vector<PagePlan> page_plans;
-  std::vector<FilePlan> file_plans;
+  std::vector<StatPatch>& stat_patches = L.stat_patches;
+  std::vector<uint8_t>& skeleton = L.skeleton;
+  std::vector<ByteCopy>& copies = L.copies;
+  L.compress = req.codec == pq::SNAPPY;
+  const bool compress = L.compress;
+  std::vector<PagePlan>& page_plans = L.page_plans;
+  std::vector<FilePlan>& file_plans = L.file_plans;
   auto header_len_at = [&](size_t skel_pos) -> uint32_t {
     thrift::Reader r(skeleton.data() + skel_pos, skeleton.data() + skeleton.size());
     r.skip(thrift::T_STRUCT);
@@ -1127,8 +1191,8 @@
   };
   std::vector<uint32_t> seg_page_begin(nseg + 1, 0);
   std::vector<std::vector<uint64_t>> page_value_offset(ncols);
-  uint64_t cursor = 0;
-  uint32_t page_counter = 0;
+  uint64_t& cursor = L.cursor;
+  uint32_t& page_counter = L.page_counter;
   auto emit = [&](uint64_t dst, size_t skel_begin) {
     copies.push_back(ByteCopy{dst, (uint32_t)skel_begin, (uint32_t)(skeleton.size() - skel_begin)});
   };
@@ -1309,19 +1373,47 @@
   out->arena_bytes = cursor;
   out->arena.alloc(ctx, std::max<uint64_t>(cursor, 16) + 64);
 
-  Buf<uint8_t> d_skel(ctx, std::max<size_t>(1, skeleton.size()));
-  Buf<ByteCopy> d_copies(ctx, std::max<size_t>(1, copies.size()));
-  Buf<uint32_t> d_page_begin(ctx, seg_page_begin.size());
-  Buf<uint64_t> d_pvo(ctx, std::max<size_t>(1, (size_t)ncols * page_counter));
+  L.d_skel.alloc(ctx, std::max<size_t>(1, skeleton.size()));
+  L.d_copies.alloc(ctx, std::max<size_t>(1, copies.size()));
+  L.d_page_begin.alloc(ctx, seg_page_begin.size());
+  L.d_pvo.alloc(ctx, std::max<size_t>(1, (size_t)ncols * page_counter));
   if (!skeleton.empty())
-    copy_h2d(ctx, d_skel.get(), skeleton.data(), skeleton.size());
+    copy_h2d(ctx, L.d_skel.get(), skeleton.data(), skeleton.size());
   if (!copies.empty())
-    copy_h2d(ctx, d_copies.get(), copies.data(), copies.size() * sizeof(ByteCopy));
-  copy_h2d(ctx, d_page_begin.get(), seg_page_begin.data(), seg_page_begin.size() * 4);
+    copy_h2d(ctx, L.d_copies.get(), copies.data(), copies.size() * sizeof(ByteCopy));
+  copy_h2d(ctx, L.d_page_begin.get(), seg_page_begin.data(), seg_page_begin.size() * 4);
   for (int c = 0; c < ncols; c++)
     if (page_counter)
-      copy_h2d(ctx, d_pvo.get() + (size_t)c * page_counter, page_value_offset[c].data(), (size_t)page_counter * 8);
-  t_plan.stop();
+      copy_h2d(ctx, L.d_pvo.get() + (size_t)c * page_counter, page_value_offset[c].data(), (size_t)page_counter * 8);
+  L.t_plan.stop();
+}
+
+void write_segments(hs_ctx* ctx, const EncodeRequest& req, EncodeLayout& lay, bool key_pages_written, EncodedFiles* out,
+                    hs_stats* stats) {
+  EncodeLayout::Impl& L = *lay.impl;
+  const Table& table = *req.table;
+  const int ncols = (int)table.cols.size();
+  const int64_t ntiles = req.plan->ntiles;
+  const int64_t P = L.P;
+  const std::vector<pq::SchemaColumn>& schema = L.schema;
+  const std::string& schema_json = L.schema_json;
+  const std::vector<std::vector<uint64_t>>& tile_val_off = L.tile_val_off;
+  const std::vector<std::vector<uint64_t>>& tile_def_off = L.tile_def_off;
+  const std::vector<ColDict>& dicts = L.dicts;
+  const std::vector<int>& carried_cols = L.carried_cols;
+  const std::vector<StatPatch>& stat_patches = L.stat_patches;
+  const std::vector<uint8_t>& skeleton = L.skeleton;
+  const std::vector<ByteCopy>& copies = L.copies;
+  const bool compress = L.compress;
+  const std::vector<PagePlan>& page_plans = L.page_plans;
+  std::vector<FilePlan>& file_plans = L.file_plans;
+  uint64_t& cursor = L.cursor;
+  const uint32_t page_counter = L.page_counter;
+  const Buf<uint8_t>& d_skel = L.d_skel;
+  const Buf<ByteCopy>& d_copies = L.d_copies;
+  const Buf<uint32_t>& d_page_begin = L.d_page_begin;
+  const Buf<uint64_t>& d_pvo = L.d_pvo;
+  StageTimer t_enc(ctx);
 
   t_enc.start();
   launch_scatter_bytes(ctx, d_copies.get(), (int64_t)copies.size(), d_skel.get(), out->arena.get());
@@ -1354,6 +1446,7 @@
                                     d_voff.get(), d_doff.get(), out->arena.get());
       continue;
     }
+    if (c == 0 && key_pages_written) continue;
     if (c == 0 && req.d_sorted_keys && (dc.type == HS_TYPE_INT32 || dc.type == HS_TYPE_INT64)) gc.sorted_keys = req.d_sorted_keys;
     launch_gather_encode(ctx, req.plan->tiles.get(), req.plan->ntiles, req.plan->seg_start.get(), req.d_perm, gc,
                          d_page_begin.get(), P, out->arena.get());
@@ -1361,7 +1454,7 @@
   if (!stat_patches.empty()) {
     Buf<StatPatch> d_sp(ctx, stat_patches.size());
     copy_h2d(ctx, d_sp.get(), stat_patches.data(), sizeof(StatPatch) * stat_patches.size());
-    launch_patch_key_stats(ctx, d_sp.get(), (int64_t)stat_patches.size(), req.d_sorted_keys, table.cols[0].type, out->arena.get());
+    launch_patch_key_stats(ctx, d_sp.get(), (int64_t)stat_patches.size(), req.d_perm, table.cols[0].data.get(), out->arena.get());
   }
   {
     std::vector<int> dcols;
@@ -1557,7 +1650,7 @@
     if (!patches2.empty()) {
       Buf<StatPatch> d_sp(ctx, patches2.size());
       copy_h2d(ctx, d_sp.get(), patches2.data(), sizeof(StatPatch) * patches2.size());
-      launch_patch_key_stats(ctx, d_sp.get(), (int64_t)patches2.size(), req.d_sorted_keys, table.cols[0].type, arena2.get());
+      launch_patch_key_stats(ctx, d_sp.get(), (int64_t)patches2.size(), req.d_perm, table.cols[0].data.get(), arena2.get());
     }
     sync_stream(ctx);
     out->arena = std::move(arena2);
@@ -1567,10 +1660,11 @@
   }
   t_enc.stop();
   sync_stream(ctx);
-  stats->ms_plan += t_plan.ms();
+  stats->ms_plan += L.t_plan.ms();
   stats->ms_encode += t_enc.ms();
   stats->bytes_out += (int64_t)cursor;
   stats->files_out += (int32_t)out->files.size();
-}
-
-}
+  lay.impl.reset();
+}
+
+}
diff --git a/hyperspace_b200/csrc/engine.h b/hyperspace_b200/csrc/engine.h
--- a/hyperspace_b200/csrc/engine.h
+++ b/hyperspace_b200/csrc/engine.h
@@ -104,12 +104,14 @@
                     const std::vector<std::pair<int64_t, int64_t>>* file_windows, Table* out, hs_stats* stats,
                     const CarryOptions* carry = nullptr);
 
-void index_rows(hs_ctx* ctx, Table& table, int nkeys, int num_buckets, IndexedRows* out, hs_stats* stats, bool defer_settle = false);
+void index_rows(hs_ctx* ctx, Table& table, int nkeys, int num_buckets, IndexedRows* out, hs_stats* stats, bool defer_settle = false,
+                const KeyPagesFn* key_pages = nullptr);
 
 struct EncodeRequest {
   const Table* table = nullptr;
   const uint32_t* d_perm = nullptr;
   const uint64_t* d_sorted_keys = nullptr;
+  bool key_sorted = false;
   const SortPlan* plan = nullptr;
   std::vector<uint64_t> seg_offsets;
   std::vector<std::string> seg_names;
@@ -127,13 +129,23 @@
   std::vector<OutFile> files;
 };
 void encode_segments(hs_ctx* ctx, const EncodeRequest& req, EncodedFiles* out, hs_stats* stats);
+struct EncodeLayout {
+  struct Impl;
+  std::shared_ptr<Impl> impl;
+};
+bool layout_needs_sorted_rows(const Table& table);
+void layout_segments(hs_ctx* ctx, const EncodeRequest& req, EncodeLayout* lay, EncodedFiles* out, hs_stats* stats);
+const KeyPageDest* key_page_dest(EncodeLayout& lay, const EncodeRequest& req, EncodedFiles* out);
+void write_segments(hs_ctx* ctx, const EncodeRequest& req, EncodeLayout& lay, bool key_pages_written, EncodedFiles* out,
+                    hs_stats* stats);
 
 void exchange_rows(hs_ctx* ctx, Table& table, int nkeys, int num_buckets, hs_stats* stats);
 void comm_destroy(hs_ctx* ctx);
 void comm_allgather_host(hs_ctx* ctx, const void* in, size_t bytes, void* out);
 bool p2p_exchange_supported(hs_ctx* ctx, int num_buckets);
 void exchange_partition_p2p(hs_ctx* ctx, Table& table, int nkeys, int num_buckets, IndexedRows* out, hs_stats* stats);
-void sort_partitioned_rows(hs_ctx* ctx, int nkeys, int num_buckets, IndexedRows* out, hs_stats* stats, bool defer_settle = false);
+void sort_partitioned_rows(hs_ctx* ctx, int nkeys, int num_buckets, IndexedRows* out, hs_stats* stats, bool defer_settle = false,
+                           const KeyPagesFn* key_pages = nullptr);
 bool settle_sort(hs_ctx* ctx, IndexedRows* out, hs_stats* stats);
 void launch_dictionary_probes(hs_ctx* ctx, const Table& part, bool use_dictionary, std::unique_ptr<DictProbe>* out);
 
diff --git a/hyperspace_b200/csrc/gather_encode.cu b/hyperspace_b200/csrc/gather_encode.cu
--- a/hyperspace_b200/csrc/gather_encode.cu
+++ b/hyperspace_b200/csrc/gather_encode.cu
@@ -6,10 +6,6 @@
 namespace {
 
 constexpr int kThreads = 256;
-
-__device__ __forceinline__ uint64_t sort_decode_int(int type, uint64_t e) {
-  return type == 1 ? (e ^ 0x8000000000000000ull) : (uint64_t)((uint32_t)e ^ 0x80000000u);
-}
 
 template <int W>
 __global__ void __launch_bounds__(kThreads) k_gather_encode(const SortTile* __restrict__ tiles,
@@ -239,13 +235,14 @@
   for (uint32_t i = head + 4 * nwords + threadIdx.x; i < b.len; i += 256) dst[i] = src[i];
 }
 
-__global__ void k_patch_key_stats(const StatPatch* __restrict__ patches, int64_t n, const uint64_t* __restrict__ sorted_keys,
-                                  int key_type, uint8_t* __restrict__ arena) {
+__global__ void k_patch_key_stats(const StatPatch* __restrict__ patches, int64_t n, const uint32_t* __restrict__ perm,
+                                  const void* __restrict__ keys, uint8_t* __restrict__ arena) {
   const int64_t i = (int64_t)blockIdx.x * blockDim.x + threadIdx.x;
   if (i >= n) return;
   const StatPatch p = patches[i];
-  const uint64_t vmin = sort_decode_int(key_type, sorted_keys[p.first_pos]);
-  const uint64_t vmax = sort_decode_int(key_type, sorted_keys[p.last_pos]);
+  const uint32_t rmin = perm[p.first_pos], rmax = perm[p.last_pos];
+  const uint64_t vmin = p.width == 8 ? ((const uint64_t*)keys)[rmin] : ((const uint32_t*)keys)[rmin];
+  const uint64_t vmax = p.width == 8 ? ((const uint64_t*)keys)[rmax] : ((const uint32_t*)keys)[rmax];
   for (int b = 0; b < p.width; b++) {
     const uint8_t lo = (uint8_t)(vmin >> (8 * b)), hi = (uint8_t)(vmax >> (8 * b));
     arena[p.min_off[0] + b] = lo;
@@ -369,10 +366,10 @@
   HS_LAUNCH_CHECK(ctx);
 }
 
-void launch_patch_key_stats(hs_ctx* ctx, const StatPatch* patches, int64_t n, const uint64_t* sorted_keys, int key_type,
+void launch_patch_key_stats(hs_ctx* ctx, const StatPatch* patches, int64_t n, const uint32_t* perm, const void* keys,
                             uint8_t* arena) {
   if (n == 0) return;
-  k_patch_key_stats<<<(unsigned)ceil_div(n, 128), 128, 0, ctx->stream>>>(patches, n, sorted_keys, key_type, arena);
+  k_patch_key_stats<<<(unsigned)ceil_div(n, 128), 128, 0, ctx->stream>>>(patches, n, perm, keys, arena);
   HS_LAUNCH_CHECK(ctx);
 }
 
diff --git a/hyperspace_b200/csrc/kernels.h b/hyperspace_b200/csrc/kernels.h
--- a/hyperspace_b200/csrc/kernels.h
+++ b/hyperspace_b200/csrc/kernels.h
@@ -1,4 +1,6 @@
 #pragma once
+#include <functional>
+
 #include "hs_common.h"
 
 namespace hs {
@@ -180,6 +182,14 @@
   Buf<uint32_t> chunk_sums;
 };
 void build_sort_plan(hs_ctx* ctx, const uint64_t* seg_offsets, int nseg, SortPlan* plan);
+struct KeyPageDest {
+  uint8_t* arena;
+  const uint32_t* seg_page_begin;
+  const uint64_t* page_value_offset;
+  uint32_t rows_per_page;
+  int32_t width;
+  int32_t type;
+};
 struct SortedRows {
   Buf<uint64_t> keys_buf[2];
   Buf<uint32_t> perm_buf[2];
@@ -189,9 +199,11 @@
   bool queued = false;
   uint64_t resort_bits = 0, queued_at = 0;
   uint32_t gave_up = 0;
-};
+  bool key_pages_written = false;
+};
+using KeyPagesFn = std::function<const KeyPageDest*()>;
 void sort_rows(hs_ctx* ctx, SortPlan* plan, const KeyColumn* cols, int ncols, const unsigned long long* last_or_and,
-               bool may_defer, SortedRows* out);
+               bool may_defer, SortedRows* out, const KeyPagesFn* key_pages = nullptr);
 bool settle_sorted_rows(hs_ctx* ctx, SortPlan* plan, SortedRows* s);
 
 struct GatherColumn {
@@ -247,7 +259,7 @@
   uint64_t min_off[2], max_off[2];
   int32_t width, pad;
 };
-void launch_patch_key_stats(hs_ctx* ctx, const StatPatch* patches, int64_t n, const uint64_t* sorted_keys, int key_type,
+void launch_patch_key_stats(hs_ctx* ctx, const StatPatch* patches, int64_t n, const uint32_t* perm, const void* keys,
                             uint8_t* arena);
 struct ByteCopy {
   uint64_t dst;
diff --git a/hyperspace_b200/csrc/radix_sort.cu b/hyperspace_b200/csrc/radix_sort.cu
--- a/hyperspace_b200/csrc/radix_sort.cu
+++ b/hyperspace_b200/csrc/radix_sort.cu
@@ -331,6 +331,7 @@
 constexpr int kLocalSortCap = 12288;
 struct LocalSortItem {
   uint32_t start, count;
+  uint32_t seg, seg_row;
 };
 constexpr int kLocalThreads = 1024;
 constexpr int kLocalWarps = kLocalThreads / 32;
@@ -377,7 +378,7 @@
 template <typename Src>
 __global__ void __launch_bounds__(kLocalThreads, 1) k_local_sort(const LocalSortItem* __restrict__ items, Src src,
                                                                  uint64_t* __restrict__ out_keys,
-                                                                 uint32_t* __restrict__ out_vals) {
+                                                                 uint32_t* __restrict__ out_vals, KeyPageDest pages) {
   extern __shared__ __align__(16) uint8_t smem_raw[];
   LocalShared& sm = *reinterpret_cast<LocalShared*>(smem_raw);
   const LocalSortItem it = items[blockIdx.x];
@@ -466,21 +467,51 @@
     }
   }
   __syncthreads();
+  if (out_keys) {
+#pragma unroll
+    for (int j = 0; j < kLocalItems; j++) {
+      const uint32_t i = j * kLocalThreads + threadIdx.x;
+      if (i < count) {
+        const uint32_t s = sm.slot[i];
+        out_keys[(uint64_t)it.start + i] = sm.keys[s];
+        out_vals[(uint64_t)it.start + i] = sm.vals[s];
+      }
+    }
+    return;
+  }
+  const uint64_t* pvo = pages.page_value_offset + pages.seg_page_begin[it.seg];
+  const uint32_t P = pages.rows_per_page;
 #pragma unroll
   for (int j = 0; j < kLocalItems; j++) {
     const uint32_t i = j * kLocalThreads + threadIdx.x;
     if (i < count) {
       const uint32_t s = sm.slot[i];
-      out_keys[(uint64_t)it.start + i] = sm.keys[s];
       out_vals[(uint64_t)it.start + i] = sm.vals[s];
+      const uint32_t lr = it.seg_row + i, page = lr / P;
+      uint8_t* dst = pages.arena + pvo[page] + (uint64_t)(lr - page * P) * pages.width;
+      const uint64_t v = sort_decode_int(pages.type, sm.keys[s]);
+      if (((uintptr_t)dst & (pages.width - 1)) != 0) {
+        for (int b = 0; b < pages.width; b++) dst[b] = (uint8_t)(v >> (8 * b));
+      } else if (pages.width == 8) {
+        *reinterpret_cast<uint64_t*>(dst) = v;
+      } else {
+        *reinterpret_cast<uint32_t*>(dst) = (uint32_t)v;
+      }
     }
   }
 }
 
 template <typename Src>
 void launch_local_sort(hs_ctx* ctx, const std::vector<LocalSortItem>& items, Src src, uint64_t* out_keys,
-                       uint32_t* out_vals) {
+                       uint32_t* out_vals, const KeyPageDest* pages) {
   if (items.empty()) return;
+  KeyPageDest dest{};
+  if (pages) {
+    dest = *pages;
+    out_keys = nullptr;
+  } else if (!out_keys) {
+    fail(HS_EINVAL, "internal: local sort without a key destination");
+  }
   Buf<LocalSortItem> d_items(ctx, items.size());
   copy_h2d(ctx, d_items.get(), items.data(), items.size() * sizeof(LocalSortItem));
   static DeviceOnce attr_once;
@@ -491,7 +522,7 @@
   }
   KernelScope _ks(ctx, "k_local_sort");
   k_local_sort<Src><<<(unsigned)items.size(), kLocalThreads, sizeof(LocalShared), ctx->stream>>>(d_items.get(), src,
-                                                                                                 out_keys, out_vals);
+                                                                                                 out_keys, out_vals, dest);
   HS_LAUNCH_CHECK(ctx);
 }
 
@@ -566,16 +597,32 @@
   if (first) fail(HS_EINVAL, "sort: raw first-pass source given but no pass ran");
 }
 
-void local_sort_segments(hs_ctx* ctx, const SortPlan& plan, const KeyColumn& raw, SortedRows* s) {
+uint64_t* final_keys(hs_ctx* ctx, SortedRows* s, int64_t n) {
+  Buf<uint64_t>& b = s->keys_buf[s->cur];
+  if (!b) b.alloc(ctx, std::max<int64_t>(1, n));
+  return b.get();
+}
+
+const KeyPageDest* key_destination(hs_ctx* ctx, const KeyPagesFn* key_pages, SortedRows* s, int64_t n) {
+  const KeyPageDest* pages = key_pages ? (*key_pages)() : nullptr;
+  if (!pages) final_keys(ctx, s, n);
+  s->key_pages_written = pages != nullptr;
+  return pages;
+}
+
+void local_sort_segments(hs_ctx* ctx, const SortPlan& plan, const KeyColumn& raw, SortedRows* s,
+                         const KeyPagesFn* key_pages) {
   std::vector<LocalSortItem> items;
   for (int g = 0; g < plan.nseg; g++) {
     const uint64_t n = plan.h_seg_start[g + 1] - plan.h_seg_start[g];
-    if (n) items.push_back(LocalSortItem{(uint32_t)plan.h_seg_start[g], (uint32_t)n});
-  }
-  with_raw_source(raw, [&](auto src) { launch_local_sort(ctx, items, src, s->keys(), s->perm()); });
-}
-
-bool msd_local_sort(hs_ctx* ctx, SortPlan* plan, const KeyColumn& raw, int shift, SortedRows* s) {
+    if (n) items.push_back(LocalSortItem{(uint32_t)plan.h_seg_start[g], (uint32_t)n, (uint32_t)g, 0});
+  }
+  const KeyPageDest* pages = key_destination(ctx, key_pages, s, plan.n);
+  with_raw_source(raw, [&](auto src) { launch_local_sort(ctx, items, src, s->keys(), s->perm(), pages); });
+}
+
+bool msd_local_sort(hs_ctx* ctx, SortPlan* plan, const KeyColumn& raw, int shift, SortedRows* s,
+                    const KeyPagesFn* key_pages) {
   if (plan->ntiles == 0) return false;
   const size_t nsub = (size_t)plan->nseg * 256;
   Buf<uint32_t> d_base(ctx, nsub);
@@ -587,13 +634,14 @@
   base[nsub] = (uint32_t)plan->n;
   std::vector<LocalSortItem> items;
   for (int g = 0; g < plan->nseg; g++) {
-    LocalSortItem cur{base[(size_t)g * 256], 0};
+    const uint32_t seg_begin = base[(size_t)g * 256];
+    LocalSortItem cur{seg_begin, 0, (uint32_t)g, 0};
     for (size_t d = (size_t)g * 256; d < (size_t)(g + 1) * 256; d++) {
       const uint32_t sz = base[d + 1] - base[d];
       if (sz > (uint32_t)kLocalSortCap) return false;
       if (cur.count + sz > (uint32_t)kLocalSortCap) {
         items.push_back(cur);
-        cur = LocalSortItem{base[d], 0};
+        cur = LocalSortItem{base[d], 0, (uint32_t)g, base[d] - seg_begin};
       }
       cur.count += sz;
     }
@@ -602,7 +650,8 @@
   uint64_t* keys_alt = s->keys_buf[s->cur ^ 1].get();
   uint32_t* perm_alt = s->perm_buf[s->cur ^ 1].get();
   with_raw_source(raw, [&](auto src) { run_scatter(ctx, plan, src, digit, keys_alt, perm_alt); });
-  launch_local_sort(ctx, items, SrcPairs{keys_alt, perm_alt}, s->keys(), s->perm());
+  const KeyPageDest* pages = key_destination(ctx, key_pages, s, plan->n);
+  launch_local_sort(ctx, items, SrcPairs{keys_alt, perm_alt}, s->keys(), s->perm(), pages);
   return true;
 }
 
@@ -661,13 +710,20 @@
 }
 
 void sort_rows(hs_ctx* ctx, SortPlan* plan, const KeyColumn* cols, int ncols, const unsigned long long* last_or_and,
-               bool may_defer, SortedRows* out) {
+               bool may_defer, SortedRows* out, const KeyPagesFn* key_pages) {
   const int64_t nrows = plan->n;
-  for (auto& b : out->keys_buf) b.alloc(ctx, std::max<int64_t>(1, nrows));
+  const bool lsd_only = getenv("HS_LSD_SORT") != nullptr;
+  if (ncols != 1 || cols[0].valid || (cols[0].type != HS_TYPE_INT32 && cols[0].type != HS_TYPE_INT64) || lsd_only)
+    key_pages = nullptr;
+  out->cur = 0;
+  out->keys_buf[1].alloc(ctx, std::max<int64_t>(1, nrows));
+  out->keys_buf[0].release();
+  auto need_keys = [&] { final_keys(ctx, out, nrows); };
+  if (!key_pages) need_keys();
   for (auto& b : out->perm_buf) b.alloc(ctx, std::max<int64_t>(1, nrows));
-  out->cur = 0;
   out->queued = false;
   out->resort_bits = 0;
+  out->key_pages_written = false;
   Buf<unsigned long long> d_or_and(ctx, 2);
   unsigned long long or_and[2] = {0, 0};
   auto reduce = [&](auto launch) {
@@ -681,7 +737,6 @@
   for (int g = 0; g < plan->nseg; g++) max_seg = std::max<uint64_t>(max_seg, plan->h_seg_start[g + 1] - plan->h_seg_start[g]);
   int want_bytes = 2;
   while (want_bytes < 8 && (double)max_seg / std::pow(256.0, want_bytes) > 0.5) want_bytes++;
-  const bool lsd_only = getenv("HS_LSD_SORT") != nullptr;
   for (int k = ncols - 1; k >= 0; k--) {
     const KeyColumn& kc = cols[k];
     const bool from_raw = k == ncols - 1 && kc.type >= HS_TYPE_INT32 && kc.type <= HS_TYPE_DOUBLE;
@@ -714,6 +769,7 @@
         }
       const KeyColumn* raw = from_raw ? &kc : nullptr;
       if (from_raw && varying == 0) {
+        need_keys();
         launch_iota_u32(ctx, out->perm(), nrows);
         launch_encode_keys(ctx, kc.data, kc.type, nullptr, nrows, out->keys(), d_or_and.get());
         raw = nullptr;
@@ -722,12 +778,13 @@
       bool local = false;
       if (raw && !kc.valid && !lsd_only) {
         if (max_seg <= (uint64_t)kLocalSortCap) {
-          local_sort_segments(ctx, *plan, kc, out);
+          local_sort_segments(ctx, *plan, kc, out, key_pages);
           local = true;
         } else if (nbytes > 2 && max_seg <= (uint64_t)(0.85 * 256 * kLocalSortCap)) {
-          local = msd_local_sort(ctx, plan, kc, std::max(0, 63 - __builtin_clzll(varying) - 7), out);
+          local = msd_local_sort(ctx, plan, kc, std::max(0, 63 - __builtin_clzll(varying) - 7), out, key_pages);
         }
       }
+      if (!out->key_pages_written) need_keys();
       if (local) {
         out->queued = defer;
       } else if (nbytes > want_bytes) {
```

Measured after the change: 8.334 billion, median of 6. 3.9% higher.
